# maybeLx/MVSFormerPlusPlus

Hardware: AMD Instinct MI355X
Metric: ref-views/sec at 1152x1536 N=5 D=192 4-stage; achieved HBM GB/s vs peak (higher is better)
Workload: dtype fp16 operands/storage, fp32 accumulate (every stage; 1-2 fp16 MFMA terms)

## Files before the change

### include/mvs_hip.h

```cpp
#ifndef MVS_HIP_H
#define MVS_HIP_H

#include <stddef.h>
#include <stdint.h>

#ifdef __cplusplus
extern "C" {
#endif

#define MVS_ABI_VERSION 11

enum { MVS_OK = 0, MVS_ERR_ARG = 1, MVS_ERR_UNSUPPORTED = 2, MVS_ERR_LAUNCH = 3, MVS_ERR_WORKSPACE = 4 };
enum { MVS_DTYPE_F32 = 0, MVS_DTYPE_BF16 = 1, MVS_DTYPE_F16 = 2 };
enum { MVS_LAYOUT_PLANAR = 0, MVS_LAYOUT_OCTET_TILED = 1 };
enum { MVS_HEAD_CE_EVAL = 0, MVS_HEAD_CE_TRAIN = 1, MVS_HEAD_REG = 2 };
enum { MVS_REG_COSTREGNET = 0, MVS_REG_COSTREGNET3D = 1 };
enum { MVS_PREC_FP32 = 0, MVS_PREC_BF16X3 = 1, MVS_PREC_BF16P = 2, MVS_PREC_BF16X3_SPLIT = 3, MVS_PREC_F16X2 = 4, MVS_PREC_ATTN16 = 5, MVS_PREC_F16 = 6, MVS_PREC_F16MIX = 7 };
enum { MVS_VOLUME_F32 = 0, MVS_VOLUME_SPLIT = 1, MVS_VOLUME_F16 = 2 };
enum { MVS_GATHER_F32 = 0, MVS_GATHER_F16 = 1 };
enum { MVS_CORR_F16 = 0, MVS_CORR_F32 = 1 };
enum { MVS_TR_EPI_BIAS = 0, MVS_TR_EPI_GELU = 1, MVS_TR_EPI_RES_LN = 2 };

int mvs_abi_version(void);

unsigned long long mvs_f16_saturation_count(int reset);
const char* mvs_last_error(void);

int mvs_compose_homography(const float* proj, int B, int V, float* homography , void* stream);
int mvs_cascade_prologue_fwd(const float* const* proj_host_ptrs, int n_stages, int B, int V, float* homography,
                             const float* depth_values, int N, int inverse, float* hyp, int D, int H, int W, void* stream);
int mvs_homography_from_proj(const float* src_proj , const float* ref_proj , int B,
                             float* homography , void* stream);

int mvs_homo_warp_fwd(const void* src_fea, int dtype, const float* homography , const float* depth,
                      int depth_is_volume, float* warped, uint8_t* proj_mask, int B, int C, int D, int H, int W,
                      void* stream);

int mvs_warp_corr_entropy_fwd(const void* features, int dtype, int layout, const float* homography ,
                              const float* hyp, float* entropy, int B, int V, int C, int G, int D, int H, int W,
                              int view_begin, int view_end, int gather_format, void* stream);

int mvs_gather_keeps_correlations(int layout, int C, int G, int D, int H, int W);
int mvs_warp_corr_entropy_keep_fwd(const void* features, int dtype, int layout, const float* homography ,
                                   const float* hyp, float* entropy, void* corr, int corr_format, int B, int V, int C, int G, int D,
                                   int H, int W, void* stream);
int mvs_corr_aggregate_fwd(const void* corr, int corr_format, const float* vis , void* volume_cl, int volume_format,
                           int B, int V, int D, int H, int W, void* stream);

int mvs_feature_conv_is_built(int Cin, int Cout);
int mvs_conv2d3x3_tiles_fwd(const void* x, int in_dtype, const void* w_packed, const float* bias, int act, void* tiled, int out_dtype,
                            int N, int Cin, int Cout, int H, int W, long long in_batch_stride, long long out_batch_stride,
                            void* stream);

int mvs_pack_features(const void* features, int dtype, void* tiled, int out_dtype, int N, int C, int H, int W, void* stream);

size_t mvs_vis_workspace_bytes(int N, int H, int W, int precision);
int mvs_vis_weight_fwd(const float* entropy, const float* w1, const float* b1, const void* w2, const float* b2,
                       const void* w3, const float* b3, const float* w4, const float* b4, float* vis,
                       void* workspace, size_t workspace_bytes, int N, int H, int W, int precision, void* stream);

int mvs_vis_conv1_fwd(const float* entropy, const float* w1, const float* b1, float* out_cl16, int N, int H, int W, void* stream);
int mvs_vis_out_fwd(const float* x_cl8, const float* w4, const float* b4, float* vis, int N, int H, int W, void* stream);

int mvs_warp_corr_aggregate_fwd(const void* features, int dtype, int layout, const float* homography, const float* hyp,
                                const float* vis, float* volume_cl, float* vis_sum, int normalise, int volume_format, int B,
                                int V, int C, int G, int D, int H, int W, int view_begin, int view_end, void* stream);
int mvs_slab_pack(const float* volume_cl, const float* vis_sum, float* const* send_host_ptrs, const int* row_begin, const int* row_end,
                  int n_ranks, int B, int D, int H, int W, int G, void* stream);
int mvs_slab_reduce(const float* volume_cl, const float* vis_sum, float* const* recv_host_ptrs, int n_ranks, int my_rank, float* slab_out,
                    int row_begin, int row_end, int B, int D, int H, int W, int G, void* stream);
int mvs_volume_normalise(float* volume_cl, const float* vis_sum, int B, int D, int H, int W, int G, int volume_format, void* stream);
int mvs_gather_is_lds_staged(int layout, int C, int G, int D, int H, int W);
int mvs_volume_to_f16(const float* volume_cl, const float* vis_sum, void* out_f16, int B, int D, int H, int W, int G, void* stream);

int mvs_warp_corr_aggregate_bwd(const void* features, int dtype, const float* homography, const float* hyp, const float* vis,
                                const float* vis_sum, const float* volume_cl, const float* grad_volume_cl,
                                float* grad_features, float* grad_vis, int B, int V, int C, int G, int D, int H, int W,
                                void* stream);

int mvs_conv3d_bn_relu_fwd(const float* x_cl, const void* w_packed, const float* bias, float* y_cl, int B, int Cin,
                           int Cout, int D, int H, int W, int kd, int sd, int sh, int sw, int relu, int precision,
                           void* stream);

int mvs_conv3d_logits_fwd(const float* x_cl, const void* w_packed, const float* bias, float* logits, int B, int D, int H,
                          int W, int precision, void* stream);

int mvs_deconv3d_linear_fwd(const float* x_cl, const void* w_packed, const float* bias, float* y_cl, int B, int Cin, int Cout,
                            int D, int H, int W, int sd, int precision, void* stream);
int mvs_bn_stats(const float* x_cl, double* sums, long long N, int C, int groups, void* stream);
int mvs_bn_finalize(const double* sums, double count, float eps, float* mean, float* var, float* invstd, float* running_mean,
                    float* running_var, float momentum, int C, int groups, void* stream);
int mvs_bn_running_update(const float* mean, const float* var, double count, float momentum, float* running_mean,
                          float* running_var, int C, int groups, void* stream);
int mvs_bn_relu_apply(const float* z_cl, const float* mean, const float* invstd, const float* gamma, const float* beta,
                      const float* skip_cl, float* y_cl, long long N, int C, int relu, int groups, void* stream);
int mvs_bn_relu_bwd(const float* dy_cl, const float* z_cl, const float* mean, const float* invstd, const float* gamma,
                    const float* beta, double* sums, double count, float* dz_cl, long long N, int C, int relu,
                    int use_batch_stats, int phase, int groups, void* stream);
int mvs_train_block_fwd(const float* a_in_cl, const float* w, int transposed, int Cin, int Cout, int kd, int sd, int sh, int sw,
                        int B, int D, int H, int W, const float* gamma, const float* beta, float eps, float* running_mean,
                        float* running_var, float momentum, const float* skip_cl, const float* zero_bias, void* wpack_ws,
                        double* sums_ws, float* z_cl, float* mean, float* var, float* invstd, float* y_cl, int groups,
                        void* stream);
int mvs_train_block_bwd(const float* dy_cl, const float* a_in_cl, const float* z_cl, const float* mean, const float* var,
                        const float* invstd, const float* w, int transposed, int Cin, int Cout, int kd, int sd, int sh, int sw,
                        int B, int D, int H, int W, const float* gamma, const float* beta, float* running_mean,
                        float* running_var, float momentum, const float* zero_bias, void* wpack_ws, double* sums_ws,
                        float* dz_cl, float* dw, float* dgamma, float* dbeta, float* da_cl, int groups, void* stream);

long long mvs_pack_conv_weights_elems(int cout, int cin, int ntap, int ch);
int mvs_pack_conv_weights(const float* w, void* packed_bf16, int cout, int cin, int ntap, int ch, int tflip, void* stream);
long long mvs_pack_deconv_weights_elems(int cin, int cout, int sd);
int mvs_pack_deconv_weights(const float* w, void* packed_bf16, int cin, int cout, int sd, void* stream);
int mvs_conv3d_wgrad(const float* a_cl, const float* g_cl, float* dw, int B, int CA, int CB, int D, int H, int W, int kd,
                     int sd, int sh, int sw, void* stream);

int mvs_deconv3d_bn_relu_add_fwd(const float* x_cl, const void* w_packed, const float* bias, const float* skip_cl,
                                 float* y_cl, int B, int Cin, int Cout, int D, int H, int W, int sd, int precision,
                                 void* stream);

int mvs_conv3d_generic_fwd(const float* x_cl, const float* w_tck, const float* bias, const float* skip_cl, float* y_cl, int B,
                           int Cin, int Cout, int D, int H, int W, int OD, int OH, int OW, int kd, int kh, int kw, int sd, int sh,
                           int sw, int pd, int ph, int pw, int transposed, int relu, void* stream);
int mvs_conv3d_is_tuned(int Cin, int Cout, int kd, int sd, int sh, int sw);
int mvs_deconv3d_is_tuned(int Cin, int Cout, int sd);

int mvs_deconv3d_prob_fwd(const float* x_cl, const void* w_packed, const float* bias, const float* skip_cl, const float* prob_w,
                          const float* prob_b, float* logits, int B, int Cin, int D, int H, int W, int sd, int precision,
                          void* stream);

size_t mvs_regnet_workspace_bytes(int kind, int B, int D, int H, int W);
int mvs_regnet_fwd(int kind, const float* volume_cl, const void* const* w_packed, const float* const* bias,
                   float* feat_cl, void* workspace, size_t workspace_bytes, int B, int D, int H, int W, int precision,
                   void* stream);
int mvs_regnet_logits_fwd(int kind, const float* volume_cl, const void* const* w_packed, const float* const* bias,
                          const float* prob_w, const float* prob_b, float* logits, void* workspace, size_t workspace_bytes,
                          int B, int D, int H, int W, int precision, void* stream);

int mvs_prob_regress_fwd(const float* feat_cl, const float* prob_w, const float* prob_b, int prob_ksize,
                         const float* hyp, float tmp, int mode, int conf_n, float* depth, float* conf,
                         float* prob_volume, float* prob_volume_pre, int B, int D, int H, int W, void* stream);
int mvs_softmax_regress_fwd(const float* logits, const float* hyp, float tmp, int mode, int conf_n, float* depth,
                            float* conf, float* prob_volume, int B, int D, int H, int W, void* stream);
int mvs_softmax_regress_schedule_fwd(const float* logits, const float* hyp, float tmp, int mode, int conf_n, float* depth, float* conf,
                                     float* prob_volume, float ratio, float* next_hyp, int next_D, int B, int D, int H, int W,
                                     void* stream);
int mvs_softmax_regress_confavg_fwd(const float* logits, const float* hyp, float tmp, int mode, int conf_n, float* depth,
                                    float* conf, float* prob_volume, const float* const* prev_conf_host_ptrs,
                                    const int* prev_shifts_host, int n_prev, float* conf_avg, int B, int D, int H, int W,
                                    void* stream);

int mvs_depth_regression_fwd(const float* p, const float* depth_values, float* out, int B, int D, int H, int W, void* stream);
int mvs_conf_regression_fwd(const float* p, int n, float* out, int B, int D, int H, int W, void* stream);

int mvs_init_range_fwd(const float* depth_values , int N, int inverse, float* hyp , int B,
// ... 103 lines not shown
```

### mvsformerplusplus_amd/_lib.py

```python
from __future__ import annotations

import ctypes as C
import os
import threading
from typing import Optional

import torch

_HERE = os.path.dirname(os.path.abspath(__file__))
LIB_PATH = os.environ.get("MVS_HIP_LIB") or os.path.join(_HERE, "csrc", "libmvs_hip.so")

OK = 0
ABI_VERSION = 11
TR_EPI_BIAS, TR_EPI_GELU, TR_EPI_RES_LN = 0, 1, 2
DTYPE_CODE = {torch.float32: 0, torch.bfloat16: 1, torch.float16: 2}
HEAD_CE_EVAL, HEAD_CE_TRAIN, HEAD_REG = 0, 1, 2
LAYOUT_PLANAR, LAYOUT_OCTET_TILED = 0, 1
REG_COSTREGNET, REG_COSTREGNET3D = 0, 1
PREC_FP32, PREC_BF16X3, PREC_BF16P, PREC_BF16X3_SPLIT, PREC_F16X2, PREC_ATTN16, PREC_F16, PREC_F16MIX = 0, 1, 2, 3, 4, 5, 6, 7
PRECISIONS = {"fp32": PREC_FP32, "bf16x3": PREC_BF16X3, "f16x2": PREC_F16X2, "f16": PREC_F16, "f16mix": PREC_F16MIX}
F16_FORMATS = ("f16x2", "f16", "f16mix")
F16_CODES = (PREC_F16X2, PREC_F16, PREC_F16MIX)
VOLUME_F32, VOLUME_SPLIT, VOLUME_F16 = 0, 1, 2
CORR_F16, CORR_F32 = 0, 1

_vp, _i, _f, _sz = C.c_void_p, C.c_int, C.c_float, C.c_size_t

SIGNATURES = {
    "mvs_abi_version": (_i, []),
    "mvs_f16_saturation_count": (C.c_ulonglong, [_i]),
    "mvs_last_error": (C.c_char_p, []),
    "mvs_compose_homography": (_i, [_vp, _i, _i, _vp, _vp]),
    "mvs_cascade_prologue_fwd": (_i, [_vp, _i, _i, _i, _vp, _vp, _i, _i, _vp, _i, _i, _i, _vp]),
    "mvs_homography_from_proj": (_i, [_vp, _vp, _i, _vp, _vp]),
    "mvs_homo_warp_fwd": (_i, [_vp, _i, _vp, _vp, _i, _vp, _vp, _i, _i, _i, _i, _i, _vp]),
    "mvs_warp_corr_entropy_fwd": (_i, [_vp, _i, _i, _vp, _vp, _vp] + [_i] * 10 + [_vp]),
    "mvs_pack_features": (_i, [_vp, _i, _vp, _i, _i, _i, _i, _i, _vp]),
    "mvs_feature_conv_is_built": (_i, [_i, _i]),
    "mvs_conv2d3x3_tiles_fwd": (_i, [_vp, _i, _vp, _vp, _i, _vp, _i, _i, _i, _i, _i, _i, C.c_longlong, C.c_longlong, _vp]),
    "mvs_vis_workspace_bytes": (_sz, [_i, _i, _i, _i]),
    "mvs_vis_weight_fwd": (_i, [_vp] * 10 + [_vp, _sz, _i, _i, _i, _i, _vp]),
    "mvs_vis_conv1_fwd": (_i, [_vp, _vp, _vp, _vp, _i, _i, _i, _vp]),
    "mvs_vis_out_fwd": (_i, [_vp, _vp, _vp, _vp, _i, _i, _i, _vp]),
    "mvs_warp_corr_aggregate_fwd": (_i, [_vp, _i, _i, _vp, _vp, _vp, _vp, _vp, _i, _i] + [_i] * 9 + [_vp]),
    "mvs_volume_normalise": (_i, [_vp, _vp, _i, _i, _i, _i, _i, _i, _vp]),
    "mvs_volume_to_f16": (_i, [_vp, _vp, _vp, _i, _i, _i, _i, _i, _vp]),
    "mvs_gather_is_lds_staged": (_i, [_i, _i, _i, _i, _i, _i]),
    "mvs_gather_keeps_correlations": (_i, [_i, _i, _i, _i, _i, _i]),
    "mvs_warp_corr_entropy_keep_fwd": (_i, [_vp, _i, _i, _vp, _vp, _vp, _vp] + [_i] * 8 + [_vp]),
    "mvs_corr_aggregate_fwd": (_i, [_vp, _i, _vp, _vp] + [_i] * 6 + [_vp]),
    "mvs_slab_pack": (_i, [_vp, _vp, _vp, _vp, _vp, _i, _i, _i, _i, _i, _i, _vp]),
    "mvs_slab_reduce": (_i, [_vp, _vp, _vp, _i, _i, _vp, _i, _i, _i, _i, _i, _i, _i, _vp]),
    "mvs_conv3d_bn_relu_fwd": (_i, [_vp, _vp, _vp, _vp] + [_i] * 12 + [_vp]),
    "mvs_deconv3d_bn_relu_add_fwd": (_i, [_vp, _vp, _vp, _vp, _vp] + [_i] * 8 + [_vp]),
    "mvs_conv3d_generic_fwd": (_i, [_vp] * 5 + [_i] * 20 + [_vp]),
    "mvs_conv3d_is_tuned": (_i, [_i] * 6),
    "mvs_deconv3d_is_tuned": (_i, [_i] * 3),
    "mvs_deconv3d_prob_fwd": (_i, [_vp] * 7 + [_i] * 7 + [_vp]),
    "mvs_conv3d_logits_fwd": (_i, [_vp] * 4 + [_i] * 5 + [_vp]),
    "mvs_deconv3d_linear_fwd": (_i, [_vp] * 4 + [_i] * 8 + [_vp]),
    "mvs_bn_stats": (_i, [_vp, _vp, C.c_longlong, _i, _i, _vp]),
    "mvs_bn_finalize": (_i, [_vp, C.c_double, C.c_float, _vp, _vp, _vp, _vp, _vp, C.c_float, _i, _i, _vp]),
    "mvs_bn_running_update": (_i, [_vp, _vp, C.c_double, C.c_float, _vp, _vp, _i, _i, _vp]),
    "mvs_bn_relu_apply": (_i, [_vp] * 7 + [C.c_longlong, _i, _i, _i, _vp]),
    "mvs_bn_relu_bwd": (_i, [_vp] * 7 + [C.c_double, _vp, C.c_longlong, _i, _i, _i, _i, _i, _vp]),
    "mvs_train_block_fwd": (_i, [_vp, _vp] + [_i] * 11 + [_vp, _vp, C.c_float, _vp, _vp, C.c_float] + [_vp] * 9 + [_i, _vp]),
    "mvs_train_block_bwd": (_i, [_vp] * 7 + [_i] * 11 + [_vp, _vp, _vp, _vp, C.c_float] + [_vp] * 8 + [_i, _vp]),
    "mvs_pack_conv_weights_elems": (C.c_longlong, [_i] * 4),
    "mvs_pack_conv_weights": (_i, [_vp, _vp] + [_i] * 5 + [_vp]),
    "mvs_pack_deconv_weights_elems": (C.c_longlong, [_i] * 3),
    "mvs_pack_deconv_weights": (_i, [_vp, _vp] + [_i] * 3 + [_vp]),
    "mvs_conv3d_wgrad": (_i, [_vp] * 3 + [_i] * 10 + [_vp]),
    "mvs_warp_corr_aggregate_bwd": (_i, [_vp, _i] + [_vp] * 8 + [_i] * 7 + [_vp]),
    "mvs_regnet_workspace_bytes": (_sz, [_i, _i, _i, _i, _i]),
    "mvs_regnet_fwd": (_i, [_i, _vp, _vp, _vp, _vp, _vp, _sz, _i, _i, _i, _i, _i, _vp]),
    "mvs_regnet_logits_fwd": (_i, [_i, _vp, _vp, _vp, _vp, _vp, _vp, _vp, _sz, _i, _i, _i, _i, _i, _vp]),
    "mvs_prob_regress_fwd": (_i, [_vp, _vp, _vp, _i, _vp, _f, _i, _i, _vp, _vp, _vp, _vp, _i, _i, _i, _i, _vp]),
    "mvs_softmax_regress_fwd": (_i, [_vp, _vp, _f, _i, _i, _vp, _vp, _vp, _i, _i, _i, _i, _vp]),
    "mvs_softmax_regress_schedule_fwd": (_i, [_vp, _vp, _f, _i, _i, _vp, _vp, _vp, _f, _vp, _i, _i, _i, _i, _i, _vp]),
    "mvs_softmax_regress_confavg_fwd": (_i, [_vp, _vp, _f, _i, _i, _vp, _vp, _vp, _vp, _vp, _i, _vp, _i, _i, _i, _i, _vp]),
    "mvs_depth_regression_fwd": (_i, [_vp, _vp, _vp, _i, _i, _i, _i, _vp]),
    "mvs_conf_regression_fwd": (_i, [_vp, _i, _vp, _i, _i, _i, _i, _vp]),
    "mvs_init_range_fwd": (_i, [_vp, _i, _i, _vp, _i, _i, _i, _i, _vp]),
    "mvs_init_range_pixel_fwd": (_i, [_vp, _i, _i, _vp, _i, _i, _i, _i, _vp]),
    "mvs_schedule_inverse_range_fwd": (_i, [_vp, _vp, _i, _f, _i, _vp, _i, _i, _i, _i, _vp]),
    "mvs_schedule_range_fwd": (_i, [_vp, _vp, _i, _vp, _i, _i, _i, _i, _vp]),
    "mvs_confidence_average": (_i, [_vp, _vp, _i, _vp, _i, _i, _i, _vp]),
    "mvs_position3d_workspace_bytes": (_sz, []),
    "mvs_position3d_fwd": (_i, [_vp, _vp, _vp, _i, _vp, _i, _vp, _sz, _vp, _i, _i, _i, _i, _vp]),
    "mvs_position3d_raw_fwd": (_i, [_vp, _vp, _vp, _i, _i, _i, _i, _vp]),
    "mvs_position_encoding3d_fwd": (_i, [_vp, _vp, _vp, _i, _i, _f, C.c_longlong, _vp]),
    "mvs_tr_embed_fwd": (_i, [_vp] * 9 + [_i] * 8 + [_vp]),
    "mvs_tr_linear_fwd": (_i, [_vp, _vp, _vp, _i, _vp, _vp, _vp, _vp, _f, _vp, _i, _i, _i, _i, _i, _vp]),
    "mvs_tr_attention_operand_bytes": (_sz, [_i, _i, _i]),
    "mvs_tr_qkv_fwd": (_i, [_vp, _vp, _vp, _vp, _vp, _f, _i, _i, _i, _i, _i, _vp]),
    "mvs_tr_attention_fwd": (_i, [_vp, _vp, _vp, _vp, _i, _i, _i, _i, _vp]),
    "mvs_tr_attention_bwd": (_i, [_vp, _vp, _vp, _vp, _vp, _vp, _i, _i, _i, _f, _vp]),
    "mvs_tr_up_prob_fwd": (_i, [_vp] * 8 + [_i] * 8 + [_vp]),
    "mvs_fusion_campack_floats": (_sz, []),
    "mvs_fusion_prepare_cams": (_i, [_vp, _i, _vp, _vp]),
    "mvs_fusion_filter_fwd": (_i, [_i] + [_vp] * 8 + [_f] * 4 + [_vp] * 7 + [_i] * 4 + [_vp]),
    "mvs_fusion_ave_fwd": (_i, [_vp, _vp, _vp, _vp, _i, _i, _i, _i, _vp]),
    "mvs_pointcloud_workspace_bytes": (_sz, [_i, _i]),
    "mvs_pointcloud_append": (_i, [_vp, _vp, _vp, _i, _i, _vp, _sz, _vp, _vp, _i, _vp, C.c_longlong, _vp]),
    "mvs_gipuma_view_floats": (_sz, []),
    "mvs_gipuma_pair_floats": (_sz, []),
    "mvs_gipuma_prepare_cams": (_i, [_vp, _i, _vp, _vp]),
    "mvs_gipuma_prepare_view": (_i, [_vp, _vp, _vp, _i, _i, _vp, _vp, _vp]),
    "mvs_gipuma_fuse_view": (_i, [_vp] * 5 + [_i] * 4 + [C.c_double, C.c_double, _f, C.c_double] + [_vp] * 5),
    "mvs_colmap_workspace_bytes": (_sz, [_i]),
    "mvs_colmap_depths": (_i, [_vp, _vp, C.c_longlong, _vp, _vp, _vp, _vp]),
    "mvs_colmap_scores": (_i, [_vp, _vp, _vp, _i, _vp, _vp, _i, _vp, _vp, C.c_double, C.c_double, C.c_double, C.c_longlong]
                          + [_vp] * 3 + [_sz, _vp, _vp]),
    "mvs_fpn_conv_is_built": (_i, [_i] * 4),
    "mvs_fpn_merge_is_built": (_i, [_i, _i]),
    "mvs_fpn_conv_fwd": (_i, [_vp, _vp, _vp, _i, _vp] + [_i] * 7 + [_vp]),
    "mvs_fpn_merge_fwd": (_i, [_vp] * 5 + [_i] * 4 + [_vp]),
    "mvs_fpn_merge_conv_fwd": (_i, [_vp] * 6 + [_i, _vp] + [_i] * 5 + [_vp]),
    "mvs_fmt_weights_bytes": (_sz, []),
    "mvs_fmt_vectors_bytes": (_sz, []),
    "mvs_fmt_kv_operand_bytes": (_sz, []),
    "mvs_fmt_kv_workspace_bytes": (_sz, [_i, _i]),
    "mvs_fmt_kv_fwd": (_i, [_vp] * 5 + [_sz, _vp, _i, _i, _vp]),
    "mvs_fmt_block_fwd": (_i, [_vp] * 6 + [_i, _i, _i, _vp]),
    "mvs_fmt_path_fwd": (_i, [_vp] * 5 + [_i] * 6 + [_vp]),
    "mvs_fmt_merge_fwd": (_i, [_vp] * 4 + [_i] * 6 + [_vp]),
    "mvs_fmt_smooth_fwd": (_i, [_vp] * 3 + [_i] * 4 + [_vp]),
    "mvs_ncdhw_to_cl": (_i, [_vp, _vp, _i, _i, _i, _i, _i, _vp]),
    "mvs_cl_to_ncdhw": (_i, [_vp, _vp, _i, _i, _i, _i, _i, _vp]),
}

# ... 88 lines not shown
```

### mvsformerplusplus_amd/cost_volume.py

```python
from __future__ import annotations

from typing import Dict, Optional

import torch
import torch.nn as nn

from . import _lib, ops, packing
from .module import (DEFAULT_PRECISION, DEFAULT_STAGE_POLICY, resolve_stage_precision, F16_FORMATS, MFMA_FORMATS, ConvBnReLU, CostRegNet, CostRegNet3D, PureTransformerCostReg, _bn_dict, _no_grad_path,
                     _PackedCache, precision_code)


def shard_views(n_src: int, world: int, rank: int):
    base, extra = divmod(n_src, world)
    begin = 1 + rank * base + min(rank, extra)
    return begin, begin + base + (1 if rank < extra else 0)


STAGE_DEFAULT_PRECISION = DEFAULT_STAGE_POLICY


_F16_CALLS = {}
_F16_CHECK_DUE = set()
KEEP_CORRELATIONS_MAX_BYTES = 1 << 30
KEEP_MIN_DEPTH = 5
# ... 83 lines not shown

        def build(dev):
            out = []
            for i, ch in ((0, None), (1, 16), (2, 16)):
                layer = self.vis[i]
                w, b = packing.fold_bn(layer.conv.weight.detach().cpu().float(), _bn_dict(layer.bn), 0)
                if i == 0:
                    out += [w[:, 0].permute(1, 2, 0).reshape(9, 16).contiguous().to(dev), b.contiguous().to(dev)]
                else:
                    out += [pack(w.unsqueeze(2), 16).to(dev), packing.pad_bias(b).to(dev)]
            last = self.vis[3]
            out += [last.weight.detach().float().reshape(8).contiguous().to(dev), last.bias.detach().float().reshape(1).contiguous().to(dev)]
            return out
        return self._vis_cache.get(self.vis, build, prec)

    def _vis_precision(self) -> str:
        return self.conv_precision

    def _keeps_correlations(self, feats, G, hyp) -> bool:
        if not self.keep_correlations:
            return False
        exact = self.gather_precision != "f16"
        B, V, _, H, W = feats.shape
        D = hyp.shape[1]
        dmin = self.keep_min_depth if self.keep_min_depth is not None else (KEEP_EXACT_MIN_DEPTH if exact else KEEP_MIN_DEPTH)
        if D < dmin or (exact and D <= 4):
            return False
        if (V - 1) * B * D * H * W * (32 if exact else 16) > KEEP_CORRELATIONS_MAX_BYTES:
            return False
        return ops.gather_keeps_correlations(feats, G, hyp)

    def _f16_activations(self) -> bool:
        return self.conv_precision in F16_FORMATS and not isinstance(self.cost_reg, PureTransformerCostReg) and not self._generic_regulariser()

    def _generic_regulariser(self) -> bool:
        return bool(getattr(self.cost_reg, "is_generic", False))

    def _wants_autograd(self, features) -> bool:
        return self.training or (torch.is_grad_enabled() and torch.is_tensor(features) and features.requires_grad)

    def forward(self, features, proj_matrices, depth_values, tmp, position3d=None, _fused: Optional[dict] = None) -> Dict[str, torch.Tensor]:
        if self._wants_autograd(features):
            from .training import stage_forward_train
            assert features.shape[1] == proj_matrices.shape[1], "Different number of images and projection matrices"
            return stage_forward_train(self, features, proj_matrices, depth_values, tmp, position3d)
        B, V, C, H, W = features.shape
        assert V == proj_matrices.shape[1], "Different number of images and projection matrices"
        G = self.in_channels
        if G > C:
            raise AssertionError("G must <= C!")
        if C % G != 0:
            raise AssertionError("base_ch=%d must divide the %d feature channels (the reference's .view(B, G, C // G, ...), cost_volume.py:80)" % (G, C))
        feats, code = ops._feat(features)
        hyp = ops._f32c(depth_values)
        if hyp.dim() == 2:
            hyp = hyp[:, :, None, None].expand(B, hyp.shape[1], H, W).contiguous()
        elif hyp.dim() != 4:
            raise ValueError("depth_values must be [B,D] or [B,D,H,W], got shape %s" % (tuple(depth_values.shape),))
        hom = _fused.get("homography") if _fused else None
        if hom is None:
            hom = ops.compose_homography(proj_matrices)
        conf_prev = _fused.get("conf_prev") if _fused and self.view_group is None else None
        nxt = _fused.get("next") if _fused and self.view_group is None and conf_prev is None and hyp.shape[1] >= 3 else None
        vis_params = self._vis_params(feats.device)
        prec = precision_code(self._vis_precision())
        if self.view_group is not None:
            import torch.distributed as dist
            world = dist.get_world_size(self.view_group)
            slab = self._slab_plan(H, world) if self.shard_mode in ("auto", "slab") else None
            if slab is not None and not isinstance(self.cost_reg, PureTransformerCostReg):
                return self._forward_slab(feats, code, hom, hyp, depth_values, G, vis_params, float(tmp), slab)
            volume = self._sharded_volume(feats, code, hom, hyp, G, vis_params)
            split = self._split_activations()
        else:
            split = self._split_activations()
            f16 = self._f16_activations()
            w16 = self.gather_precision == "f16"
            if self._keeps_correlations(feats, G, hyp):
                entropy, corr = ops.warp_corr_entropy_keep(feats, code, hom, hyp, G, exact=not w16)
                vis = ops.vis_weight(entropy, vis_params, prec)
                volume = ops.corr_aggregate(corr, vis, split=split, f16=f16)
                del corr
            else:
                entropy = ops.warp_corr_entropy(feats, code, hom, hyp, G, f16_window=w16)
                vis = ops.vis_weight(entropy, vis_params, prec)
                if f16 and not ops.gather_is_lds_staged(feats, G, hyp):
                    volume = ops.volume_to_f16(ops.warp_corr_aggregate(feats, code, hom, hyp, vis, G, normalise=True)[0])
                else:
                    volume, _ = ops.warp_corr_aggregate(feats, code, hom, hyp, vis, G, normalise=True, split=split, f16=f16)
        out = self._regularise_and_regress(volume, hyp, depth_values, float(tmp), position3d, split=split, conf_prev=conf_prev, nxt=nxt)
        if conf_prev is not None:
            _fused["conf_avg"] = out.pop("_conf_avg")
        if "_next_hyp" in out:
            _fused["next_hyp"] = out.pop("_next_hyp")
        if self._f16_activations():
            self._count_f16_call(feats.device, hyp)
        return out

    @staticmethod
    def _count_f16_call(device, hyp=None):
        key = device.index if device.type == "cuda" else -1
        n = _F16_CALLS[key] = _F16_CALLS.get(key, 0) + 1
        due = bool(F16_SATURATION_CHECK_EVERY) and (n == 8 or n % F16_SATURATION_CHECK_EVERY == 0 or key in _F16_CHECK_DUE)
        if not due:
            return
        if device.type == "cuda" and torch.cuda.is_current_stream_capturing():
            _F16_CHECK_DUE.add(key)
            return
        _F16_CHECK_DUE.discard(key)
        check_f16_saturation(device)
        if hyp is not None:
            check_hypothesis_conditioning(hyp)

    def _split_activations(self) -> bool:
        return self.conv_precision == "bf16x3" and not isinstance(self.cost_reg, PureTransformerCostReg) and not self._generic_regulariser()

    def _head_mode(self, D):
        conf_n = 0
        if self.depth_type == "ce":
            mode = _lib.HEAD_CE_TRAIN if self.training else _lib.HEAD_CE_EVAL
        else:
            mode = _lib.HEAD_REG
            conf_n = 4 if D >= 32 else (3 if D == 16 else (2 if D == 8 else 0))
        return mode, conf_n

    def _regularise_and_regress(self, volume, hyp, depth_values, tmp, position3d=None, split=False, conf_prev=None, nxt=None) -> Dict[str, torch.Tensor]:
        D = hyp.shape[1]
        pcode = _lib.PREC_BF16X3_SPLIT if split else precision_code(self.conv_precision)
        mfma = self.conv_precision in MFMA_FORMATS
        mode, conf_n = self._head_mode(D)
        conf_avg = None

        def head(logits):
            if nxt is not None:
                return ops.softmax_regress_schedule(logits, hyp, tmp, mode, conf_n, self.return_prob_volumes, int(nxt[0]), float(nxt[1]))
            return ops.softmax_regress(logits, hyp, tmp, mode, conf_n, self.return_prob_volumes, conf_prev=conf_prev)

        if isinstance(self.cost_reg, PureTransformerCostReg):
            prob_volume_pre = self.cost_reg.logits_cl(volume, position3d)
            depth, conf, prob_volume, *rest = head(prob_volume_pre)
        elif self._generic_regulariser():
            prob_volume_pre = self.cost_reg.logits_cl_generic(volume)
            depth, conf, prob_volume, *rest = head(prob_volume_pre)
        else:
            ws, bs, prob_w, prob_b = self.cost_reg.packed_all(volume.device, self.conv_precision)
            if self.cost_reg.prob_ksize == 1 and mfma and self.fuse_prob_head:
                prob_volume_pre = ops.regnet_logits(self.cost_reg.kind, volume, ws, bs, prob_w, prob_b, pcode)
                depth, conf, prob_volume, *rest = head(prob_volume_pre)
            elif self.cost_reg.prob_ksize == 3 and mfma:
                feat_cl = ops.regnet(self.cost_reg.kind, volume, ws, bs, pcode)
                prob_volume_pre = ops.conv3d_logits(feat_cl, prob_w, prob_b, pcode)
                depth, conf, prob_volume, *rest = head(prob_volume_pre)
            else:
                feat_cl = ops.regnet(self.cost_reg.kind, volume, ws, bs, pcode)
                if split:
                    feat_cl = ops.from_split(feat_cl)
                elif feat_cl.dtype == torch.float16:
                    feat_cl = feat_cl.float()
                depth, conf, prob_volume, prob_volume_pre = ops.prob_regress(
                    feat_cl, prob_w, prob_b, self.cost_reg.prob_ksize, hyp, tmp, mode, conf_n, self.return_prob_volumes)
                rest = []
                if conf_prev is not None:
                    rest = [ops.confidence_average(list(conf_prev) + [conf], conf.shape[-2], conf.shape[-1])]
        out = {"depth": depth, "prob_volume": prob_volume, "photometric_confidence": conf,
               "depth_values": depth_values, "prob_volume_pre": prob_volume_pre}
        if conf_prev is not None:
            out["_conf_avg"] = rest[0]
        elif nxt is not None and rest:
            out["_next_hyp"] = rest[0]
        return out

    MAX_CACHED_SHAPES = 2
# ... 131 lines not shown
```

### mvsformerplusplus_amd/csrc/gather_lds.h

```cpp
#pragma once
#include "gather_common.h"

namespace mvs {

#ifndef MVS_GL_CAP
#define MVS_GL_CAP 1024
#endif
constexpr int GL_CAP = MVS_GL_CAP;
constexpr int GL_XALIGN = 8;
constexpr int GL_DCH = 4;
constexpr int GL_TH = 4;

#ifndef MVS_OPAQUE_SREG
#define MVS_OPAQUE_SREG "s"
#endif
__device__ __forceinline__ float gl_round_f16(float v) { return (float)(_Float16)fminf(fmaxf(v, -65504.0f), 65504.0f); }

#ifndef MVS_GL_DIRECT16
#define MVS_GL_DIRECT16 1
#endif
template <typename T, bool TILED, bool W16, int NOCT, bool KEEPPASS>
constexpr bool gl_direct_v = (MVS_GL_DIRECT16 != 0) && W16 && TILED && std::is_same<T, _Float16>::value && NOCT == 1;

#ifndef MVS_GL_OPT
#define MVS_GL_OPT 1
#endif
#ifndef MVS_GL_SB
#define MVS_GL_SB 2
#endif
#ifndef MVS_GL_ABL
#define MVS_GL_ABL 0
#endif

#define GL_BLEND8(wv, t00, t01, t10, t11, tp)                                                          \
    _Pragma("unroll") for (int j = 0; j < 4; ++j) {                                                    \
        wv[2 * j] = MVS_FMA_MIX_LO(t00[j], tp.w00, 0.0f);                                              \
        wv[2 * j + 1] = MVS_FMA_MIX_HI(t00[j], tp.w00, 0.0f);                                          \
    }                                                                                                  \
    _Pragma("unroll") for (int j = 0; j < 4; ++j) {                                                    \
        wv[2 * j] = MVS_FMA_MIX_LO(t01[j], tp.w01, wv[2 * j]);                                         \
        wv[2 * j + 1] = MVS_FMA_MIX_HI(t01[j], tp.w01, wv[2 * j + 1]);                                 \
    }                                                                                                  \
    _Pragma("unroll") for (int j = 0; j < 4; ++j) {                                                    \
        wv[2 * j] = MVS_FMA_MIX_LO(t10[j], tp.w10, wv[2 * j]);                                         \
        wv[2 * j + 1] = MVS_FMA_MIX_HI(t10[j], tp.w10, wv[2 * j + 1]);                                 \
    }                                                                                                  \
    _Pragma("unroll") for (int j = 0; j < 4; ++j) {                                                    \
        wv[2 * j] = MVS_FMA_MIX_LO(t11[j], tp.w11, wv[2 * j]);                                         \
        wv[2 * j + 1] = MVS_FMA_MIX_HI(t11[j], tp.w11, wv[2 * j + 1]);                                 \
    }

template <typename T, int NOCT, bool KEEP_GROUPS, bool TILED, bool W16, bool DIRECT = false>
__device__ __forceinline__ void gl_unit(const T* __restrict__ src, const T* __restrict__ ref, const Homography& hm, float fx, float fy,
                                        const float* depth, bool active, int H, int W, unsigned HW, unsigned pc, f32x4* win,
                                        unsigned* red, int unit, float wscale, const float* rf_in, float* out) {
    typedef typename PairOf<T>::type P2;
    constexpr int GPO = 8 / NOCT;
    constexpr int CPG = NOCT;
    const int tid = (int)threadIdx.x, lane = tid & 63, wave = tid >> 6;
    const float qx = hm.r[0] * fx + hm.r[1] * fy + hm.r[2];
    const float qy = hm.r[3] * fx + hm.r[4] * fy + hm.r[5];
    const float qz = hm.r[6] * fx + hm.r[7] * fy + hm.r[8];
    GTap tp[GL_DCH];
    u16x2 mn = {0xffff, 0xffff}, mx = {0, 0};
    const float cx = 0.5f * (float)(W - 1), cy = 0.5f * (float)(H - 1);
#if MVS_GL_OPT
#pragma unroll
    for (int dd = 0; dd < GL_DCH; ++dd) {
#if MVS_GL_ABL == 6
        tp[dd].pk = ((unsigned)(int)fy << 16) | (unsigned)(int)fx; tp[dd].w00 = depth[dd]; tp[dd].w01 = qx; tp[dd].w10 = 0.25f; tp[dd].w11 = 0.25f;
        if ((int)fx > W - 2 || (int)fy > H - 2) tp[dd].pk = 0;
#else
        tp[dd] = make_gtap(hm, qx, qy, qz, depth[dd], H, W, cx, cy);
#endif
        const u16x2 pkv = gl_as_vec(tp[dd].pk);
        mn = __builtin_elementwise_min(mn, pkv);
        mx = __builtin_elementwise_max(mx, (u16x2)(pkv + (u16x2){1, 1}));
    }
    if (!active) { mn = (u16x2){0xffff, 0xffff}; mx = (u16x2){0, 0}; }
#else
#pragma unroll
    for (int dd = 0; dd < GL_DCH; ++dd) {
        tp[dd] = make_gtap(hm, qx, qy, qz, depth[dd], H, W, cx, cy);
        if (active && tp[dd].pk != GL_NONE) {
            mn = __builtin_elementwise_min(mn, gl_as_vec(tp[dd].pk));
            mx = __builtin_elementwise_max(mx, gl_as_vec(tp[dd].pk));
        }
    }
#endif
    if constexpr (DIRECT) {
        static_assert(W16 && TILED && std::is_same<T, _Float16>::value, "the direct form reads fp16 octet tiles");
        typedef unsigned u32x4 __attribute__((ext_vector_type(4)));
        unsigned tofs[GL_DCH];
#pragma unroll
        for (int dd = 0; dd < GL_DCH; ++dd) {
            const unsigned pk = tp[dd].pk;
            tofs[dd] = pk == GL_NONE ? 0u : ((pk >> 16) * (unsigned)W + (pk & 0xffffu)) * 16u;
        }
        const int rowb = W * 16;
        if (!active) return;
#pragma unroll
        for (int o = 0; o < NOCT; ++o) {
            unsigned oofs = gl_octet_offset(o, HW);
            asm volatile("" : "+" MVS_OPAQUE_SREG(oofs));
            const __amdgpu_buffer_rsrc_t rs = __builtin_amdgcn_make_buffer_rsrc(const_cast<T*>(src + oofs), 0, (int)(HW * 16u), 0x00020000);
            float rf[8];
            if (NOCT > 1) {
                gl_load8<TILED, T>(ref + oofs, HW, pc, rf);
            } else {
#pragma unroll
                for (int c = 0; c < 8; ++c) rf[c] = rf_in[c];
            }
            u32x4 t[GL_DCH][4];
#pragma unroll
            for (int dd = 0; dd < GL_DCH; ++dd) {
#if MVS_GL_DIRECT16 == 3
                (void)rs; (void)rowb;
#pragma unroll
                for (int k = 0; k < 4; ++k) t[dd][k] = u32x4{tofs[dd], tofs[dd] + (unsigned)k, tofs[dd] ^ 0x3c003c00u, 0x3c003c00u};
#else
                t[dd][0] = __builtin_amdgcn_raw_buffer_load_b128(rs, (int)tofs[dd], 0, 0);
                t[dd][1] = __builtin_amdgcn_raw_buffer_load_b128(rs, (int)(tofs[dd] + 16u), 0, 0);
                t[dd][2] = __builtin_amdgcn_raw_buffer_load_b128(rs, (int)tofs[dd], rowb, 0);
                t[dd][3] = __builtin_amdgcn_raw_buffer_load_b128(rs, (int)(tofs[dd] + 16u), rowb, 0);
#endif
            }
#pragma unroll
            for (int c = 0; c < 8; ++c) rf[c] *= wscale;
#pragma unroll
            for (int dd = 0; dd < GL_DCH; ++dd) {
                float wv[8];
#if MVS_GL_DIRECT16 == 2
#pragma unroll
                for (int j = 0; j < 4; ++j) {
                    const unsigned x = t[dd][0][j] ^ t[dd][1][j] ^ t[dd][2][j] ^ t[dd][3][j];
                    wv[2 * j] = __builtin_bit_cast(float, x & 0x3fffffffu);
                    wv[2 * j + 1] = tp[dd].w00;
                }
#elif MVS_GL_OPT
                GL_BLEND8(wv, t[dd][0], t[dd][1], t[dd][2], t[dd][3], tp[dd])
#else
#pragma unroll
                for (int j = 0; j < 4; ++j) {
                    float a = MVS_FMA_MIX_LO(t[dd][0][j], tp[dd].w00, 0.0f);
                    a = MVS_FMA_MIX_LO(t[dd][1][j], tp[dd].w01, a);
                    a = MVS_FMA_MIX_LO(t[dd][2][j], tp[dd].w10, a);
                    wv[2 * j] = MVS_FMA_MIX_LO(t[dd][3][j], tp[dd].w11, a);
                    float b = MVS_FMA_MIX_HI(t[dd][0][j], tp[dd].w00, 0.0f);
                    b = MVS_FMA_MIX_HI(t[dd][1][j], tp[dd].w01, b);
                    b = MVS_FMA_MIX_HI(t[dd][2][j], tp[dd].w10, b);
                    wv[2 * j + 1] = MVS_FMA_MIX_HI(t[dd][3][j], tp[dd].w11, b);
                }
#endif
                if (KEEP_GROUPS) {
#pragma unroll
                    for (int j = 0; j < GPO; ++j) {
                        float s = out[(o * GPO + j) * GL_DCH + dd];
#pragma unroll
                        for (int c = 0; c < CPG; ++c) s += rf[j * CPG + c] * wv[j * CPG + c];
                        out[(o * GPO + j) * GL_DCH + dd] = s;
                    }
                } else {
                    float s = out[dd];
#pragma unroll
                    for (int c = 0; c < 8; ++c) s += rf[c] * wv[c];
                    out[dd] = s;
                }
            }
        }
        return;
    }
#if MVS_GL_ABL == 5
    {
        __syncthreads();
        const unsigned p0 = (unsigned)__builtin_amdgcn_readfirstlane((int)tp[0].pk);
        const unsigned bx = (p0 & 0xffffu) > 8u ? (p0 & 0xffffu) - 8u : 0u, by = (p0 >> 16) > 2u ? (p0 >> 16) - 2u : 0u;
        mn = gl_as_vec((by << 16) | bx);
        mx = gl_as_vec(((by + 9u) << 16) | (bx + 81u));
#pragma unroll
        for (int dd = 0; dd < GL_DCH; ++dd) tp[dd].pk = ((by + 1u + (unsigned)(lane & 3)) << 16) | (bx + 1u + (unsigned)(lane & 63));
    }
#else
    mn = gl_wave_reduce<false>(mn);
    mx = gl_wave_reduce<true>(mx);
    unsigned* rd = red + (unit & 1) * 8;
    if (lane == 63) { rd[wave] = gl_as_u32(mn); rd[4 + wave] = gl_as_u32(mx); }
    __syncthreads();
    mn = __builtin_elementwise_min(__builtin_elementwise_min(gl_as_vec(rd[0]), gl_as_vec(rd[1])),
                                   __builtin_elementwise_min(gl_as_vec(rd[2]), gl_as_vec(rd[3])));
    mx = __builtin_elementwise_max(__builtin_elementwise_max(gl_as_vec(rd[4]), gl_as_vec(rd[5])),
                                   __builtin_elementwise_max(gl_as_vec(rd[6]), gl_as_vec(rd[7])));
#endif
#if MVS_GL_OPT
    const int xmin = mn[0], ymin = mn[1], xmax = (int)mx[0] - 1, ymax = (int)mx[1] - 1;
#else
    const int xmin = mn[0], ymin = mn[1], xmax = mx[0], ymax = mx[1];
#endif
    if (xmax < xmin) return;
    const int wx0 = xmin & ~(GL_XALIGN - 1);
    const int ww = (xmax + 2 - wx0 + GL_XALIGN - 1) & ~(GL_XALIGN - 1);
    const int wh = ymax + 2 - ymin;
    const int n = ww * wh;
    typedef _Float16 h8 __attribute__((ext_vector_type(8)));
    h8* win16 = reinterpret_cast<h8*>(win);
    if (n <= (W16 ? 2 * GL_CAP : GL_CAP)) {
        unsigned pos[GL_DCH];
#pragma unroll
        for (int dd = 0; dd < GL_DCH; ++dd) {
            const unsigned pk = tp[dd].pk;
#if MVS_GL_OPT
            const unsigned raw = ((pk >> 16) - (unsigned)ymin) * (unsigned)ww + ((pk & 0xffffu) - (unsigned)wx0);
            pos[dd] = raw < (unsigned)(n - ww - 2) ? raw : (unsigned)(n - ww - 2);
#else
            pos[dd] = pk == GL_NONE ? 0u : ((pk >> 16) - (unsigned)ymin) * (unsigned)ww + ((pk & 0xffffu) - (unsigned)wx0);
#endif
        }
        const float inv_ww = __builtin_amdgcn_rcpf((float)ww) * 1.000001f;
        const unsigned gbase = (unsigned)ymin * (unsigned)W + (unsigned)wx0;
#pragma unroll
        for (int o = 0; o < NOCT; ++o) {
            if (o > 0) __syncthreads();
            unsigned oofs = gl_octet_offset(o, HW);
            asm volatile("" : "+" MVS_OPAQUE_SREG(oofs));
            const T* so = src + oofs;
            float rf[8];
            if (NOCT > 1) {
                gl_load8<TILED, T>(ref + oofs, HW, pc, rf);
            } else {
#pragma unroll
                for (int c = 0; c < 8; ++c) rf[c] = rf_in[c];
            }
#if MVS_GL_OPT
            const __amdgpu_buffer_rsrc_t srs = __builtin_amdgcn_make_buffer_rsrc(const_cast<T*>(so), 0, (int)(8u * HW * (unsigned)sizeof(T)), 0x00020000);
            const unsigned planeb = HW * (unsigned)sizeof(T);
#endif
            int istart = tid;
#if MVS_GL_OPT && MVS_GL_ABL == 0
            if constexpr (!TILED) {
                constexpr int SBR = NOCT == 1 ? MVS_GL_SB : 1;
#pragma unroll 1
                for (int i0 = tid; i0 < n; i0 += 256 * SBR) {
                    float v[SBR][8];
#pragma unroll
                    for (int k = 0; k < SBR; ++k) {
                        const int i = i0 + 256 * k;
                        if (i < n) {
                            const int row = (int)(((float)i + 0.5f) * inv_ww);
                            const unsigned g = gbase + (unsigned)row * (unsigned)(W - ww) + (unsigned)i;
#pragma unroll
                            for (int c = 0; c < 8; ++c) {
                                if constexpr (sizeof(T) == 4)
                                    v[k][c] = __builtin_bit_cast(float, __builtin_amdgcn_raw_buffer_load_b32(srs, (int)(g * 4u), (int)((unsigned)c * planeb), 0));
                                else
                                    v[k][c] = to_f32(__builtin_bit_cast(T, (unsigned short)__builtin_amdgcn_raw_buffer_load_b16(srs, (int)(g * 2u), (int)((unsigned)c * planeb), 0)));
                            }
                        }
                    }
#pragma unroll
                    for (int k = 0; k < SBR; ++k) {
                        const int i = i0 + 256 * k;
                        if (i < n) {
                            if (W16) {
                                h8 hv;
#pragma unroll
                                for (int c = 0; c < 8; ++c) hv[c] = (_Float16)__builtin_amdgcn_fmed3f(v[k][c], -65504.0f, 65504.0f);
                                win16[i] = hv;
                            } else {
                                win[i] = f32x4{v[k][0], v[k][1], v[k][2], v[k][3]};
                                win[GL_CAP + i] = f32x4{v[k][4], v[k][5], v[k][6], v[k][7]};
                            }
                        }
                    }
                }
                istart = n;
// ... 30 lines not shown
                }
#endif
                if constexpr (W16 && TILED && std::is_same<T, _Float16>::value) {
                    win16[i] = *(reinterpret_cast<const h8*>(so) + g);
                    continue;
                }
                float v[8];
                gl_load8<TILED, T>(so, HW, g, v);
                if (W16) {
                    h8 hv;
#pragma unroll
                    for (int c = 0; c < 8; ++c) hv[c] = (_Float16)fminf(fmaxf(v[c], -65504.0f), 65504.0f);
                    win16[i] = hv;
                } else {
                    win[i] = f32x4{v[0], v[1], v[2], v[3]};
                    win[GL_CAP + i] = f32x4{v[4], v[5], v[6], v[7]};
                }
            }
            __syncthreads();
            if (active) {
#pragma unroll
                for (int c = 0; c < 8; ++c) rf[c] *= wscale;
#pragma unroll
                for (int dd = 0; dd < GL_DCH; ++dd) {
                    if (dd == 2) __builtin_amdgcn_sched_barrier(0);
                    float wv[8];
                    if (W16) {
                        typedef unsigned u32x4 __attribute__((ext_vector_type(4)));
                        const u32x4* w0 = reinterpret_cast<const u32x4*>(win16) + pos[dd];
#if MVS_GL_ABL == 3
                        const u32x4 t00 = {pos[dd], 0x3c003c00u, 0x3c003c00u, pos[dd]}, t01 = t00, t10 = {0x3c003c00u, pos[dd], pos[dd], 0x3c003c00u}, t11 = t10;
#else
                        const u32x4 t00 = w0[0], t01 = w0[1], t10 = w0[ww], t11 = w0[ww + 1];
#endif
#if MVS_GL_ABL == 4
#pragma unroll
                        for (int j = 0; j < 4; ++j) { wv[2 * j] = __builtin_bit_cast(float, (t00[j] ^ t01[j] ^ t10[j] ^ t11[j]) & 0x3fffffffu); wv[2 * j + 1] = tp[dd].w00; }
#elif MVS_GL_OPT
                        GL_BLEND8(wv, t00, t01, t10, t11, tp[dd])
#else
#pragma unroll
                        for (int j = 0; j < 4; ++j) {
                            float a = MVS_FMA_MIX_LO(t00[j], tp[dd].w00, 0.0f);
                            a = MVS_FMA_MIX_LO(t01[j], tp[dd].w01, a);
                            a = MVS_FMA_MIX_LO(t10[j], tp[dd].w10, a);
                            wv[2 * j] = MVS_FMA_MIX_LO(t11[j], tp[dd].w11, a);
                            float b = MVS_FMA_MIX_HI(t00[j], tp[dd].w00, 0.0f);
                            b = MVS_FMA_MIX_HI(t01[j], tp[dd].w01, b);
                            b = MVS_FMA_MIX_HI(t10[j], tp[dd].w10, b);
                            wv[2 * j + 1] = MVS_FMA_MIX_HI(t11[j], tp[dd].w11, b);
                        }
#endif
                    } else {
                        const f32x4* w0 = win + pos[dd];
                        const f32x4 a0 = w0[0], a1 = w0[1], b0 = w0[ww], b1 = w0[ww + 1];
                        const f32x4 c0 = w0[GL_CAP], c1 = w0[GL_CAP + 1], d0 = w0[GL_CAP + ww], d1 = w0[GL_CAP + ww + 1];
                        f32x4 lo = a0 * tp[dd].w00;
                        lo += a1 * tp[dd].w01;
                        lo += b0 * tp[dd].w10;
                        lo += b1 * tp[dd].w11;
                        f32x4 hi = c0 * tp[dd].w00;
                        hi += c1 * tp[dd].w01;
                        hi += d0 * tp[dd].w10;
                        hi += d1 * tp[dd].w11;
                        wv[0] = lo[0]; wv[1] = lo[1]; wv[2] = lo[2]; wv[3] = lo[3]; wv[4] = hi[0]; wv[5] = hi[1]; wv[6] = hi[2]; wv[7] = hi[3];
                    }
                    if (KEEP_GROUPS) {
#pragma unroll
                        for (int j = 0; j < GPO; ++j) {
                            float s = out[(o * GPO + j) * GL_DCH + dd];
#pragma unroll
                            for (int c = 0; c < CPG; ++c) s += rf[j * CPG + c] * wv[j * CPG + c];
                            out[(o * GPO + j) * GL_DCH + dd] = s;
                        }
                    } else {
                        float s = out[dd];
#pragma unroll
                        for (int c = 0; c < 8; ++c) s += rf[c] * wv[c];
                        out[dd] = s;
                    }
                }
            }
        }
    } else if (active) {
        unsigned top[GL_DCH];
#pragma unroll
        for (int dd = 0; dd < GL_DCH; ++dd) top[dd] = tp[dd].pk == GL_NONE ? 0u : (tp[dd].pk >> 16) * (unsigned)W + (tp[dd].pk & 0xffffu);
#pragma unroll 1
        for (int c = 0; c < 8 * NOCT; ++c) {
            const unsigned cbase = TILED ? (unsigned)(c >> 3) * 8u * HW + (unsigned)(c & 7) : (unsigned)c * HW;
            const unsigned pstep = TILED ? 8u : 1u;
            const float rfc = to_f32(ref[cbase + pc * pstep]) * wscale;
            const T* sp = src + cbase;
            const int g = c / CPG;
#pragma unroll
            for (int dd = 0; dd < GL_DCH; ++dd) {
                float t0, t1, b0, b1;
                if (TILED) {
                    __builtin_amdgcn_sched_barrier(0);
                    t0 = to_f32(sp[top[dd] * 8u]); t1 = to_f32(sp[(top[dd] + 1u) * 8u]);
                    b0 = to_f32(sp[(top[dd] + (unsigned)W) * 8u]); b1 = to_f32(sp[(top[dd] + (unsigned)W + 1u) * 8u]);
                } else {
                    const P2 t = *reinterpret_cast<const P2*>(sp + top[dd]);
                    const P2 b = *reinterpret_cast<const P2*>(sp + top[dd] + (unsigned)W);
                    t0 = to_f32(t.x); t1 = to_f32(t.y); b0 = to_f32(b.x); b1 = to_f32(b.y);
                }
                if (W16) {
                    t0 = gl_round_f16(t0); t1 = gl_round_f16(t1); b0 = gl_round_f16(b0); b1 = gl_round_f16(b1);
                }
                float wv = tp[dd].w00 * t0;
                wv += tp[dd].w01 * t1;
                wv += tp[dd].w10 * b0;
                wv += tp[dd].w11 * b1;
                if (KEEP_GROUPS) {
#pragma unroll
                    for (int gg = 0; gg < 8; ++gg) out[gg * GL_DCH + dd] += (g == gg) ? rfc * wv : 0.0f;
                } else {
                    out[dd] += rfc * wv;
                }
            }
        }
    }
}

constexpr size_t GL_WIN_BYTES = (size_t)2 * GL_CAP * 16;
constexpr size_t GL_RED_BYTES = 64;

template <int NS>
struct GlTile {
    static constexpr int TP = 256 / NS, TW = TP / GL_TH;
    int slot, pi, x, y;
    bool valid;
    unsigned pc;
    float fx, fy;
    __device__ __forceinline__ GlTile(int blk, int ntx, int H, int W) {
        const int tid = (int)threadIdx.x;
        const int ty = blk / ntx, tx = blk - ty * ntx;
        slot = tid / TP;
        pi = tid % TP;
        x = tx * TW + pi % TW;
        y = ty * GL_TH + pi / TW;
        valid = x < W && y < H;
        pc = valid ? (unsigned)y * (unsigned)W + (unsigned)x : (unsigned)H * (unsigned)W - 1u;
        fx = (float)(valid ? x : W - 1);
        fy = (float)(valid ? y : H - 1);
    }
};

template <int DT, int NOCT, int NS, bool TILED, bool KEEP, bool W16>
__global__ __launch_bounds__(256) void gl_entropy_kernel(const void* __restrict__ feat_, const float* __restrict__ hom,
                                                         const float* __restrict__ hyp, float* __restrict__ entropy,
                                                         void* __restrict__ corr, int V, int D, int H,
                                                         int W, int view_begin, int view_end, int vpb, int ntx, int nblk) {
    typedef typename FeatT<DT>::type T;
    constexpr bool DIRECT = gl_direct_v<T, TILED, W16, NOCT, KEEP>;
    HIP_DYNAMIC_SHARED(float, smem)
    f32x4* win = reinterpret_cast<f32x4*>(smem);
    unsigned* red = reinterpret_cast<unsigned*>(reinterpret_cast<char*>(smem) + GL_WIN_BYTES);
    float* sim = reinterpret_cast<float*>(reinterpret_cast<char*>(smem) + GL_WIN_BYTES + GL_RED_BYTES);
    constexpr int C = 8 * NOCT;
    constexpr int TP = GlTile<NS>::TP;
    const unsigned HW = (unsigned)H * (unsigned)W;
    const int b = (int)blockIdx.z;
    const GlTile<NS> t((int)xcd_remap(blockIdx.x, (unsigned)nblk), ntx, H, W);
    const int nch = (D + GL_DCH - 1) / GL_DCH, niter = (nch + NS - 1) / NS;
    const T* feat = reinterpret_cast<const T*>(feat_) + (size_t)(b * V) * C * HW;
    const T* ref = feat;
    const float* hp = hyp + (size_t)b * D * HW;
    const float inv_cpg = 1.0f / (float)NOCT;
    float rf0[8];
    if (NOCT == 1) gl_load8<TILED, T>(ref, HW, t.pc, rf0);
    else {
#pragma unroll
        for (int c = 0; c < 8; ++c) rf0[c] = 0.0f;
    }
    const int v0 = view_begin + (int)blockIdx.y * vpb, v1 = v0 + vpb < view_end ? v0 + vpb : view_end;
    int unit = 0;
    float sat_amax = 0.0f;
    for (int v = v0; v < v1; ++v) {
        const Homography hm = gl_load_homography(hom + (size_t)(b * (V - 1) + (v - 1)) * 12);
        const T* src = feat + (size_t)v * C * HW;
        float s[GL_DCH];
        for (int it = 0; it < niter; ++it, ++unit) {
            const int chunk = it * NS + t.slot;
            const bool active = t.valid && chunk < nch;
            const int d0 = (chunk < nch ? chunk : nch - 1) * GL_DCH;
            float depth[GL_DCH];
#pragma unroll
            for (int dd = 0; dd < GL_DCH; ++dd) depth[dd] = hp[(unsigned)(d0 + dd < D ? d0 + dd : D - 1) * HW + t.pc];
#pragma unroll
            for (int dd = 0; dd < GL_DCH; ++dd) s[dd] = 0.0f;
            if (KEEP) {
                float acc[8 * GL_DCH];
#pragma unroll
                for (int i = 0; i < 8 * GL_DCH; ++i) acc[i] = 0.0f;
                gl_unit<T, NOCT, true, TILED, W16, DIRECT>(src, ref, hm, t.fx, t.fy, depth, active, H, W, HW, t.pc, win, red, unit, inv_cpg, rf0, acc);
                typedef _Float16 h8 __attribute__((ext_vector_type(8)));
                const size_t cbase = (size_t)(b * (V - 1) + (v - 1)) * D * HW + t.pc;
#pragma unroll
                for (int dd = 0; dd < GL_DCH; ++dd) {
                    float r[8];
#pragma unroll
                    for (int g = 0; g < 8; ++g) { r[g] = acc[g * GL_DCH + dd]; s[dd] += r[g]; }
                    if (active && d0 + dd < D) {
                        const size_t vox = cbase + (size_t)(unsigned)(d0 + dd) * HW;
                        if constexpr (W16) {
                            h8 hv;
#pragma unroll
                            for (int g = 0; g < 8; ++g) hv[g] = (_Float16)fminf(fmaxf(r[g], -65504.0f), 65504.0f);
                            sat::track(sat_amax, r[0], r[1], r[2], r[3]);
                            sat::track(sat_amax, r[4], r[5], r[6], r[7]);
                            reinterpret_cast<h8*>(corr)[vox] = hv;
                        } else {
                            f32x4* cv = reinterpret_cast<f32x4*>(corr) + vox * 2;
                            cv[0] = f32x4{r[0], r[1], r[2], r[3]};
                            cv[1] = f32x4{r[4], r[5], r[6], r[7]};
                        }
                    }
                }
            } else {
                gl_unit<T, NOCT, false, TILED, W16, DIRECT>(src, ref, hm, t.fx, t.fy, depth, active, H, W, HW, t.pc, win, red, unit, inv_cpg, rf0, s);
            }
            if (NS > 1 || niter > 1) {
                if (chunk < nch) {
#pragma unroll
                    for (int dd = 0; dd < GL_DCH; ++dd)
                        if (d0 + dd < D) sim[(d0 + dd) * TP + t.pi] = s[dd];
                }
            }
        }
        float* dst = entropy + (size_t)(b * (V - 1) + (v - 1)) * HW + t.pc;
        if (NS == 1 && niter == 1) {
            const float LOG2E = 1.4426950408889634f, LN2 = 0.6931471805599453f;
            float m = s[0];
#pragma unroll
            for (int dd = 1; dd < GL_DCH; ++dd) m = dd < D ? fmaxf(m, s[dd]) : m;
            float e[GL_DCH], den = 0.0f;
#pragma unroll
            for (int dd = 0; dd < GL_DCH; ++dd) { e[dd] = dd < D ? __builtin_amdgcn_exp2f((s[dd] - m) * LOG2E) : 0.0f; den += e[dd]; }
            const float rden = 1.0f / den;
            float ent = 0.0f;
#pragma unroll
            for (int dd = 0; dd < GL_DCH; ++dd) {
                const float pr = e[dd] * rden;
                if (dd < D) ent -= pr * (__builtin_amdgcn_logf(pr + 1e-7f) * LN2);
            }
            if (t.valid) *dst = ent;
        } else {
            __syncthreads();
            if (t.slot == 0 && t.valid) gl_softmax_entropy_store(sim + t.pi, TP, D, dst);
            if constexpr (DIRECT) __syncthreads();
        }
    }
    if (KEEP && W16) sat::commit(sat_amax);
}

template <int DT, int NOCT, int NS, bool TILED, bool W16>
__global__ __launch_bounds__(256) void gl_aggregate_kernel(const void* __restrict__ feat_, const float* __restrict__ hom,
                                                           const float* __restrict__ hyp, const float* __restrict__ vis,
                                                           float* __restrict__ vol, float* __restrict__ vis_sum, int normalise, int V,
                                                           int D, int H, int W, int view_begin, int view_end, int ntx, int nblk) {
    typedef typename FeatT<DT>::type T;
    HIP_DYNAMIC_SHARED(float, smem)
    f32x4* win = reinterpret_cast<f32x4*>(smem);
    unsigned* red = reinterpret_cast<unsigned*>(reinterpret_cast<char*>(smem) + GL_WIN_BYTES);
    constexpr int C = 8 * NOCT;
    const unsigned HW = (unsigned)H * (unsigned)W;
    const int b = (int)blockIdx.z, it = (int)blockIdx.y;
    const GlTile<NS> t((int)xcd_remap(blockIdx.x, (unsigned)nblk), ntx, H, W);
    const int nch = (D + GL_DCH - 1) / GL_DCH;
    const T* feat = reinterpret_cast<const T*>(feat_) + (size_t)(b * V) * C * HW;
    const T* ref = feat;
    const float* hp = hyp + (size_t)b * D * HW;
    const float* vp = vis + (size_t)(b * (V - 1)) * HW + t.pc;
    float vsum = 0.0f;
    for (int v = view_begin; v < view_end; ++v) vsum += vp[(unsigned)(v - 1) * HW];
    if (vis_sum != nullptr && it == 0 && t.slot == 0 && t.valid) vis_sum[(size_t)b * HW + t.pc] = vsum;
    const float rdenom = (normalise & 1) ? 1.0f / (vsum + 1e-6f) : 1.0f;
    const bool split_out = (normalise & 2) != 0;
    const bool f16_out = (normalise & 4) != 0;
    float sat_amax = 0.0f;
    const float inv_cpg = 1.0f / (float)NOCT;
    float rf0[8];
    if (NOCT == 1) gl_load8<TILED, T>(ref, HW, t.pc, rf0);
    else {
#pragma unroll
        for (int c = 0; c < 8; ++c) rf0[c] = 0.0f;
    }
    const int chunk = it * NS + t.slot;
    const bool active = t.valid && chunk < nch;
    const int d0 = (chunk < nch ? chunk : nch - 1) * GL_DCH;
    float depth[GL_DCH];
#pragma unroll
    for (int dd = 0; dd < GL_DCH; ++dd) depth[dd] = hp[(unsigned)(d0 + dd < D ? d0 + dd : D - 1) * HW + t.pc];
    float acc[8 * GL_DCH];
#pragma unroll
    for (int i = 0; i < 8 * GL_DCH; ++i) acc[i] = 0.0f;
    int unit = 0;
    for (int v = view_begin; v < view_end; ++v, ++unit) {
        const Homography hm = gl_load_homography(hom + (size_t)(b * (V - 1) + (v - 1)) * 12);
        const float w = vp[(unsigned)(v - 1) * HW];
        gl_unit<T, NOCT, true, TILED, W16, gl_direct_v<T, TILED, W16, NOCT, false>>(feat + (size_t)v * C * HW, ref, hm, t.fx, t.fy, depth, active, H, W, HW, t.pc, win, red, unit, inv_cpg * w, rf0, acc);
    }
    if (active) {
        float* vb = vol + (size_t)b * D * HW * 8;
#pragma unroll
        for (int dd = 0; dd < GL_DCH; ++dd) {
            if (d0 + dd >= D) continue;
            float r[8];
#pragma unroll
            for (int g = 0; g < 8; ++g) r[g] = acc[g * GL_DCH + dd] * rdenom;
            if (f16_out) {
                typedef _Float16 h8 __attribute__((ext_vector_type(8)));
                h8 hv;
#pragma unroll
                for (int g = 0; g < 8; ++g) hv[g] = (_Float16)fminf(fmaxf(r[g], -65504.0f), 65504.0f);
                sat::track(sat_amax, r[0], r[1], r[2], r[3]);
                sat::track(sat_amax, r[4], r[5], r[6], r[7]);
                *reinterpret_cast<h8*>(reinterpret_cast<_Float16*>(vol) + ((size_t)b * D * HW + (size_t)(unsigned)(d0 + dd) * HW + t.pc) * 8) = hv;
                continue;
            }
            f32x4* o = reinterpret_cast<f32x4*>(vb + ((size_t)(unsigned)(d0 + dd) * HW + t.pc) * 8);
            if (split_out) {
                unsigned hw[4], lw[4];
#pragma unroll
                for (int j = 0; j < 4; ++j) {
                    const uint16_t h0 = from_f32<uint16_t>(r[2 * j]), h1 = from_f32<uint16_t>(r[2 * j + 1]);
                    const uint16_t l0 = from_f32<uint16_t>(r[2 * j] - to_f32(h0)), l1 = from_f32<uint16_t>(r[2 * j + 1] - to_f32(h1));
                    hw[j] = (unsigned)h0 | ((unsigned)h1 << 16);
                    lw[j] = (unsigned)l0 | ((unsigned)l1 << 16);
                }
                o[0] = f32x4{__builtin_bit_cast(float, hw[0]), __builtin_bit_cast(float, hw[1]), __builtin_bit_cast(float, hw[2]), __builtin_bit_cast(float, hw[3])};
                o[1] = f32x4{__builtin_bit_cast(float, lw[0]), __builtin_bit_cast(float, lw[1]), __builtin_bit_cast(float, lw[2]), __builtin_bit_cast(float, lw[3])};
                continue;
            }
            o[0] = f32x4{r[0], r[1], r[2], r[3]};
            o[1] = f32x4{r[4], r[5], r[6], r[7]};
        }
    }
    if (f16_out) sat::commit(sat_amax);
}

static int gl_slots(int D) {
    const int nch = (D + GL_DCH - 1) / GL_DCH;
    return nch >= 8 ? 8 : (nch >= 4 ? 4 : (nch >= 2 ? 2 : 1));
}

bool gl_window_f16_enabled();
bool gl_supported(int C, int G, int D, int H, int W);

template <int DT, int NOCT, int NS, bool TILED, bool KEEP = false, bool W16 = false>
static int gl_launch_entropy_t(const void* feat, const float* hom, const float* hyp, float* ent, int B, int V, int D, int H, int W, int vb,
                               int ve, hipStream_t st, void* corr = nullptr) {
    constexpr int TP = 256 / NS, TW = TP / GL_TH;
    const int ntx = (int)ceil_div(W, TW), nty = (int)ceil_div(H, GL_TH);
    const int nblk = ntx * nty;
    const int vpb = (long long)nblk * B >= 4096 ? ve - vb : 1;
    const size_t lds = GL_WIN_BYTES + GL_RED_BYTES + (size_t)D * TP * sizeof(float);
    if (lds > 48 * 1024)
        hipFuncSetAttribute(reinterpret_cast<const void*>(&gl_entropy_kernel<DT, NOCT, NS, TILED, KEEP, W16>), hipFuncAttributeMaxDynamicSharedMemorySize, (int)lds);
    hipLaunchKernelGGL((gl_entropy_kernel<DT, NOCT, NS, TILED, KEEP, W16>), dim3(nblk, ceil_div(ve - vb, vpb), B), dim3(256), lds, st, feat, hom, hyp, ent,
                       corr, V, D, H, W, vb, ve, vpb, ntx, nblk);
    return check_launch("gl_entropy_kernel");
}

template <int DT, int NOCT, int NS, bool TILED, bool W16 = false>
static int gl_launch_aggregate_t(const void* feat, const float* hom, const float* hyp, const float* vis, float* vol, float* vis_sum,
                                 int normalise, int B, int V, int D, int H, int W, int vb, int ve, hipStream_t st) {
    constexpr int TP = 256 / NS, TW = TP / GL_TH;
    const int ntx = (int)ceil_div(W, TW), nty = (int)ceil_div(H, GL_TH);
    const int nblk = ntx * nty;
    const int nch = (D + GL_DCH - 1) / GL_DCH, niter = (nch + NS - 1) / NS;
    const size_t lds = GL_WIN_BYTES + GL_RED_BYTES;
    hipLaunchKernelGGL((gl_aggregate_kernel<DT, NOCT, NS, TILED, W16>), dim3(nblk, niter, B), dim3(256), lds, st, feat, hom, hyp, vis, vol, vis_sum,
                       normalise, V, D, H, W, vb, ve, ntx, nblk);
    return check_launch("gl_aggregate_kernel");
}

#define GL_DISPATCH_NS(FN, DTV, NOCTV, ...)                                                    \
    switch (gl_slots(D) * 2 + (layout == MVS_LAYOUT_OCTET_TILED ? 1 : 0)) {                    \
        case 2: return FN<DTV, NOCTV, 1, false>(__VA_ARGS__);                                  \
        case 3: return FN<DTV, NOCTV, 1, true>(__VA_ARGS__);                                   \
        case 4: return FN<DTV, NOCTV, 2, false>(__VA_ARGS__);                                  \
        case 5: return FN<DTV, NOCTV, 2, true>(__VA_ARGS__);                                   \
        case 8: return FN<DTV, NOCTV, 4, false>(__VA_ARGS__);                                  \
        case 9: return FN<DTV, NOCTV, 4, true>(__VA_ARGS__);                                   \
        case 16: return FN<DTV, NOCTV, 8, false>(__VA_ARGS__);                                 \
        default: return FN<DTV, NOCTV, 8, true>(__VA_ARGS__);                                  \
    }
#define GL_DISPATCH_C(FN, DTV, ...)                                                            \
    switch (C) {                                                                               \
        case 8: GL_DISPATCH_NS(FN, DTV, 1, __VA_ARGS__)                                        \
        case 16: GL_DISPATCH_NS(FN, DTV, 2, __VA_ARGS__)                                       \
        case 32: GL_DISPATCH_NS(FN, DTV, 4, __VA_ARGS__)                                       \
        default: GL_DISPATCH_NS(FN, DTV, 8, __VA_ARGS__)                                       \
    }
#define GL_DISPATCH(FN, ...)                                                                   \
    do {                                                                                       \
        switch (dtype) {                                                                       \
            case MVS_DTYPE_F32: GL_DISPATCH_C(FN, MVS_DTYPE_F32, __VA_ARGS__)                  \
            case MVS_DTYPE_BF16: GL_DISPATCH_C(FN, MVS_DTYPE_BF16, __VA_ARGS__)                \
            default: GL_DISPATCH_C(FN, MVS_DTYPE_F16, __VA_ARGS__)                             \
        }                                                                                      \
    } while (0)


}
```

### mvsformerplusplus_amd/csrc/gather_lds_aggregate_kernels.hip

```cpp
#include "gather_lds.h"

namespace mvs {

int gl_launch_aggregate_w16(const void* feat, int dtype, int layout, const float* hom, const float* hyp, const float* vis, float* vol, float* vis_sum,
                            int normalise, int B, int V, int C, int D, int H, int W, int vb, int ve, hipStream_t st);

int gl_launch_aggregate(const void* feat, int dtype, int layout, const float* hom, const float* hyp, const float* vis, float* vol, float* vis_sum,
                        int normalise, int B, int V, int C, int D, int H, int W, int vb, int ve, hipStream_t st) {
    if ((normalise & 4) && gl_window_f16_enabled())
        return gl_launch_aggregate_w16(feat, dtype, layout, hom, hyp, vis, vol, vis_sum, normalise, B, V, C, D, H, W, vb, ve, st);
    GL_DISPATCH(gl_launch_aggregate_t, feat, hom, hyp, vis, vol, vis_sum, normalise, B, V, D, H, W, vb, ve, st);
}

}

namespace mvs { MVS_DEFINE_SAT_READER(sat_read_gather_agg) }
```

### mvsformerplusplus_amd/csrc/gather_lds_aggregate_w16_kernels.hip

```cpp
#include "gather_lds.h"

namespace mvs {

template <int DT, int NOCT, int NS, bool TILED>
static int gl_launch_aggregate_w16_t(const void* feat, const float* hom, const float* hyp, const float* vis, float* vol, float* vis_sum,
                                     int normalise, int B, int V, int D, int H, int W, int vb, int ve, hipStream_t st) {
    return gl_launch_aggregate_t<DT, NOCT, NS, TILED, true>(feat, hom, hyp, vis, vol, vis_sum, normalise, B, V, D, H, W, vb, ve, st);
}

int gl_launch_aggregate_w16(const void* feat, int dtype, int layout, const float* hom, const float* hyp, const float* vis, float* vol, float* vis_sum,
                            int normalise, int B, int V, int C, int D, int H, int W, int vb, int ve, hipStream_t st) {
    GL_DISPATCH(gl_launch_aggregate_w16_t, feat, hom, hyp, vis, vol, vis_sum, normalise, B, V, D, H, W, vb, ve, st);
}

}

namespace mvs { MVS_DEFINE_SAT_READER(sat_read_gather_agg16) }
```

### mvsformerplusplus_amd/csrc/gather_lds_entropy_w16_kernels.hip

```cpp
#include "gather_lds.h"

namespace mvs {

template <int DT, int NOCT, int NS, bool TILED>
static int gl_launch_entropy_w16_t(const void* feat, const float* hom, const float* hyp, float* ent, int B, int V, int D, int H, int W, int vb,
                                   int ve, hipStream_t st) {
    return gl_launch_entropy_t<DT, NOCT, NS, TILED, false, true>(feat, hom, hyp, ent, B, V, D, H, W, vb, ve, st);
}

int gl_launch_entropy_w16(const void* feat, int dtype, int layout, const float* hom, const float* hyp, float* ent, int B, int V, int C, int D, int H, int W,
                          int vb, int ve, hipStream_t st) {
    GL_DISPATCH(gl_launch_entropy_w16_t, feat, hom, hyp, ent, B, V, D, H, W, vb, ve, st);
}

}
```

### mvsformerplusplus_amd/csrc/gather_lds_kernels.hip

```cpp
#include "gather_lds.h"

namespace mvs {

bool gl_window_f16_enabled() {
    static const int on = [] { const char* e = getenv("MVS_GATHER_WINDOW"); return (e && e[0] == 'f' && e[1] == '3') ? 0 : 1; }();
    return on != 0;
}

bool gl_supported(int C, int G, int D, int H, int W) {
    if (G != 8 || !(C == 8 || C == 16 || C == 32 || C == 64)) return false;
    if (W % GL_XALIGN != 0 || W < GL_XALIGN || H < 2 || W > 65535 || H > 65535) return false;
    if ((long long)D * H * W > 0x7fffffffLL) return false;
    if ((long long)H * W >= (1LL << 28)) return false;
    return (size_t)D * (256 / gl_slots(D)) * sizeof(float) <= 64 * 1024;
}

bool gl_keep_supported(int C, int G, int D, int H, int W) { return gl_supported(C, G, D, H, W); }
bool gl_keep32_supported(int C, int G, int D, int H, int W) { return gl_supported(C, G, D, H, W) && D > GL_DCH; }


int gl_launch_entropy_w16(const void* feat, int dtype, int layout, const float* hom, const float* hyp, float* ent, int B, int V, int C, int D, int H, int W,
                          int vb, int ve, hipStream_t st);

int gl_launch_entropy(const void* feat, int dtype, int layout, const float* hom, const float* hyp, float* ent, int B, int V, int C, int D, int H, int W,
                      int vb, int ve, int w16, hipStream_t st) {
    if (w16 && gl_window_f16_enabled()) return gl_launch_entropy_w16(feat, dtype, layout, hom, hyp, ent, B, V, C, D, H, W, vb, ve, st);
    GL_DISPATCH(gl_launch_entropy_t, feat, hom, hyp, ent, B, V, D, H, W, vb, ve, st);
}

template <typename TI, typename TO>
__global__ __launch_bounds__(256) void pack_features_kernel(const TI* __restrict__ in, TO* __restrict__ out, int C, unsigned HW) {
    const unsigned p = blockIdx.x * 256u + threadIdx.x;
    if (p >= HW) return;
    const size_t n = blockIdx.z, o = blockIdx.y;
    const TI* src = in + (n * C + o * 8) * HW + p;
    TO* dst = out + ((n * (C / 8) + o) * HW + p) * 8;
    typedef TO to8 __attribute__((ext_vector_type(8)));
    to8 v;
#pragma unroll
    for (int c = 0; c < 8; ++c) {
        float f = to_f32(src[(size_t)c * HW]);
        if (std::is_same<TO, _Float16>::value && !std::is_same<TI, _Float16>::value) f = fminf(fmaxf(f, -65504.0f), 65504.0f);
        if (sizeof(TI) == 2 && sizeof(TO) == 2) v[c] = *reinterpret_cast<const TO*>(&src[(size_t)c * HW]);
        else v[c] = from_f32<TO>(f);
    }
    *reinterpret_cast<to8*>(dst) = v;
}

template <typename TI, typename TO>
static int pack_features_t(const void* in, void* out, int N, int C, int H, int W, hipStream_t st) {
    const unsigned HW = (unsigned)H * (unsigned)W;
    hipLaunchKernelGGL((pack_features_kernel<TI, TO>), dim3(ceil_div(HW, 256), C / 8, N), dim3(256), 0, st, static_cast<const TI*>(in),
                       static_cast<TO*>(out), C, HW);
    return check_launch("pack_features_kernel");
}

int pack_features_dispatch(const void* in, int in_dtype, void* out, int out_dtype, int N, int C, int H, int W, hipStream_t st) {
    if (out_dtype == MVS_DTYPE_F32) {
        switch (in_dtype) {
            case MVS_DTYPE_F32: return pack_features_t<float, float>(in, out, N, C, H, W, st);
            case MVS_DTYPE_BF16: return pack_features_t<uint16_t, float>(in, out, N, C, H, W, st);
            default: return pack_features_t<_Float16, float>(in, out, N, C, H, W, st);
        }
    }
    if (out_dtype == MVS_DTYPE_BF16) {
        switch (in_dtype) {
            case MVS_DTYPE_F32: return pack_features_t<float, uint16_t>(in, out, N, C, H, W, st);
            case MVS_DTYPE_BF16: return pack_features_t<uint16_t, uint16_t>(in, out, N, C, H, W, st);
            default: set_error("mvs_pack_features: fp16 -> bf16 is not a hand-off the reference produces"); return MVS_ERR_UNSUPPORTED;
        }
    }
    switch (in_dtype) {
        case MVS_DTYPE_F32: return pack_features_t<float, _Float16>(in, out, N, C, H, W, st);
        case MVS_DTYPE_F16: return pack_features_t<_Float16, _Float16>(in, out, N, C, H, W, st);
        default: set_error("mvs_pack_features: bf16 -> fp16 is not a hand-off the reference produces"); return MVS_ERR_UNSUPPORTED;
    }
}

}

namespace mvs { MVS_DEFINE_SAT_READER(sat_read_gather) }
```

### mvsformerplusplus_amd/csrc/warp_kernels.hip

```cpp
#include "mvs_common.h"

#include <stdlib.h>

namespace mvs {

__device__ void compose_p(const float* pm , double* P ) {
    const float* E = pm;
    const float* K = pm + 16;
    for (int i = 0; i < 3; ++i)
        for (int j = 0; j < 4; ++j) {
            float s = 0.0f;
            for (int k = 0; k < 3; ++k) s += K[i * 4 + k] * E[k * 4 + j];
            P[i * 4 + j] = (double)s;
        }
    for (int j = 0; j < 4; ++j) P[12 + j] = (double)E[12 + j];
}

__device__ void invert4(const double* A, double* Ai) {
    double m[4][8];
    for (int i = 0; i < 4; ++i)
        for (int j = 0; j < 4; ++j) { m[i][j] = A[i * 4 + j]; m[i][4 + j] = (i == j) ? 1.0 : 0.0; }
    for (int c = 0; c < 4; ++c) {
        int piv = c;
        double best = fabs(m[c][c]);
// ... 423 lines not shown
}

template <int DT>
__global__ __launch_bounds__(256) void homo_warp_kernel(const void* __restrict__ src_, const float* __restrict__ hom,
                                                        const float* __restrict__ depth_, int depth_is_volume,
                                                        float* __restrict__ warped, uint8_t* __restrict__ mask, int C, int D, int H,
                                                        int W) {
    typedef typename FeatT<DT>::type T;
    const int HW = H * W;
    const int lane = threadIdx.x & 63, slot = threadIdx.x >> 6;
    const int p = (int)blockIdx.x * 64 + lane;
    const int b = (int)blockIdx.z;
    if (p >= HW) return;
    const int y = p / W, x = p - y * W;
    const Homography hm = load_homography(hom + (size_t)b * 12);
    const float fx = (float)x, fy = (float)y;
    const float qx = hm.r[0] * fx + hm.r[1] * fy + hm.r[2];
    const float qy = hm.r[3] * fx + hm.r[4] * fy + hm.r[5];
    const float qz = hm.r[6] * fx + hm.r[7] * fy + hm.r[8];
    const float half_w = (float)((double)(W - 1) / 2.0), half_h = (float)((double)(H - 1) / 2.0);
    const T* src = reinterpret_cast<const T*>(src_) + (size_t)b * C * HW;
    for (int d = (int)blockIdx.y * 4 + slot; d < D; d += (int)gridDim.y * 4) {
        const float depth = depth_is_volume ? depth_[((size_t)b * D + d) * HW + p] : depth_[(size_t)b * D + d];
        bool oof;
        const Taps tp = make_taps(hm, qx, qy, qz, depth, H, W, half_w, half_h, &oof);
        if (mask != nullptr) mask[((size_t)b * D + d) * HW + p] = oof ? 1 : 0;
        if (warped != nullptr) {
            for (int c = 0; c < C; ++c) {
                const T* sp = src + (size_t)c * HW;
                float wv = tp.w[0] * to_f32(sp[tp.off[0]]);
                wv += tp.w[1] * to_f32(sp[tp.off[1]]);
                wv += tp.w[2] * to_f32(sp[tp.off[2]]);
                wv += tp.w[3] * to_f32(sp[tp.off[3]]);
                warped[(((size_t)b * C + c) * D + d) * HW + p] = wv;
            }
        }
    }
}

template <int DT, int CT, int GT>
static int launch_entropy(const void* feat, const float* hom, const float* hyp, float* ent, int B, int V, int C, int G,
                          int D, int H, int W, int vb, int ve, hipStream_t st) {
    const int HW = H * W;
    const int ppb = CT > 0 ? chunk_map(D).ppb : 64;
    const int nblk = (int)ceil_div(HW, ppb);
    const size_t lds = (size_t)D * ppb * sizeof(float);
    if (lds > 160 * 1024) { set_error("warp_corr_entropy: D=%d needs %zu B of LDS (> 160 KiB)", D, lds); return MVS_ERR_UNSUPPORTED; }
    if (lds > 48 * 1024)
        hipFuncSetAttribute(reinterpret_cast<const void*>(&warp_corr_entropy_kernel<DT, CT, GT>), hipFuncAttributeMaxDynamicSharedMemorySize, (int)lds);
    hipLaunchKernelGGL((warp_corr_entropy_kernel<DT, CT, GT>), dim3(nblk, ve - vb, B), dim3(256), lds, st, feat, hom, hyp, ent, V, C, G, D,
                       H, W, vb, nblk);
    return check_launch("warp_corr_entropy_kernel");
}

template <int DT, int CT, int GT>
static int launch_aggregate(const void* feat, const float* hom, const float* hyp, const float* vis, float* vol, float* vis_sum,
                            int normalise, int B, int V, int C, int G, int D, int H, int W, int vb, int ve, hipStream_t st) {
    const int nblk = (int)ceil_div((long long)H * W, CT > 0 ? chunk_map(D).ppb : 64);
    hipLaunchKernelGGL((warp_corr_aggregate_kernel<DT, CT, GT>), dim3(nblk, 1, B), dim3(256), 0, st, feat, hom, hyp, vis, vol, vis_sum,
                       normalise, V, C, G, D, H, W, vb, ve, nblk);
    return check_launch("warp_corr_aggregate_kernel");
}

#define MVS_DISPATCH_CG(FN, DT, ...)                                              \
    do {                                                                          \
        if (G == 8 && W >= 2) return FN<DT, 1, 8>(__VA_ARGS__);                   \
        return FN<DT, 0, 0>(__VA_ARGS__);                                         \
    } while (0)

static int check_corr_args(const char* who, const void* feat, const float* hom, const float* hyp, int dtype, int B, int V, int C, int G,
                           int D, int H, int W, int vb, int ve) {
    if (!feat || !hom || !hyp) { set_error("%s: null pointer", who); return MVS_ERR_ARG; }
    if (B < 1 || V < 2 || C < 1 || G < 1 || D < 1 || H < 1 || W < 1) { set_error("%s: bad shape", who); return MVS_ERR_ARG; }
    if (G > C || C % G != 0) { set_error("%s: G must divide C and G <= C (got C=%d G=%d)", who, C, G); return MVS_ERR_ARG; }
    if (G > 64) { set_error("%s: G=%d > 64 unsupported", who, G); return MVS_ERR_UNSUPPORTED; }
    if (vb < 1 || ve > V || vb >= ve) { set_error("%s: bad source-view range [%d,%d) for V=%d", who, vb, ve, V); return MVS_ERR_ARG; }
    if (dtype < 0 || dtype > 2) { set_error("%s: bad dtype %d", who, dtype); return MVS_ERR_ARG; }
    if ((long long)B * V * C * H * W > 0x7fffffffLL * 2 || (long long)C * H * W > 0x7fffffffLL) { set_error("%s: feature tensor too large for 32-bit plane offsets", who); return MVS_ERR_UNSUPPORTED; }
    return MVS_OK;
}

bool gl_supported(int C, int G, int D, int H, int W);
int gl_launch_entropy(const void* feat, int dtype, int layout, const float* hom, const float* hyp, float* ent, int B, int V, int C, int D, int H,
                      int W, int vb, int ve, int w16, hipStream_t st);
int gl_launch_aggregate(const void* feat, int dtype, int layout, const float* hom, const float* hyp, const float* vis, float* vol,
                        float* vis_sum, int normalise, int B, int V, int C, int D, int H, int W, int vb, int ve, hipStream_t st);
bool gl_keep_supported(int C, int G, int D, int H, int W);
bool gl_keep32_supported(int C, int G, int D, int H, int W);
int gl_launch_entropy_keep(const void* feat, int dtype, int layout, const float* hom, const float* hyp, float* ent, void* corr, int corr_format, int B,
                           int V, int C, int D, int H, int W, hipStream_t st);
int launch_corr_aggregate(const void* corr, int corr_format, const float* vis, void* vol, int volume_format, int B, int V, int D, int H, int W,
                          hipStream_t st);
int pack_features_dispatch(const void* in, int in_dtype, void* out, int out_dtype, int N, int C, int H, int W, hipStream_t st);

static int gather_impl(int C, int G, int D, int H, int W) {
    const char* e = getenv("MVS_GATHER_IMPL");
    if (e && e[0] == 'd') return 0;
    return gl_supported(C, G, D, H, W) ? 1 : 0;
}

}

using namespace mvs;

static int volume_to_split(float* volume_cl, const float* vis_sum, int B, int D, int H, int W, int G, hipStream_t st, const char* who);

extern "C" int mvs_compose_homography(const float* proj, int B, int V, float* homography, void* stream) {
    if (!proj || !homography || B < 1 || V < 2) { set_error("mvs_compose_homography: bad arguments"); return MVS_ERR_ARG; }
    const int n = B * (V - 1);
    hipLaunchKernelGGL(compose_homography_kernel, dim3(ceil_div(n, 64)), dim3(64), 0, (hipStream_t)stream, proj, B, V, homography);
    return check_launch("compose_homography_kernel");
}

extern "C" int mvs_cascade_prologue_fwd(const float* const* proj_host_ptrs, int n_stages, int B, int V, float* homography, const float* depth_values,
                                       int N, int inverse, float* hyp, int D, int H, int W, void* stream) {
    if (!proj_host_ptrs || !homography || n_stages < 1 || n_stages > 8 || B < 1 || V < 2) { set_error("mvs_cascade_prologue_fwd: bad arguments (1..8 stages)"); return MVS_ERR_ARG; }
    if (hyp && (!depth_values || N < 1 || D < 2 || H < 1 || W < 1)) { set_error("mvs_cascade_prologue_fwd: bad hypothesis arguments"); return MVS_ERR_ARG; }
    ProloguePtrs pp;
    pp.n = n_stages;
    for (int i = 0; i < 8; ++i) {
        pp.proj[i] = i < n_stages ? proj_host_ptrs[i] : nullptr;
        if (i < n_stages && !pp.proj[i]) { set_error("mvs_cascade_prologue_fwd: null projection tensor of stage %d", i); return MVS_ERR_ARG; }
    }
    int init_blocks = 0;
    dim3 grid(1, 1, 1);
    if (hyp) {
        const int HW = H * W;
        init_blocks = (int)(ceil_div(HW, 1024) > 64 ? 64 : ceil_div(HW, 1024));
        grid = dim3(init_blocks + 1, D, B);
    }
    hipLaunchKernelGGL(cascade_prologue_kernel, grid, dim3(256), 0, (hipStream_t)stream, pp, B, V, homography, depth_values, N, inverse,
                       hyp, D, H * W, init_blocks);
    return check_launch("cascade_prologue_kernel");
}

extern "C" int mvs_homography_from_proj(const float* src_proj, const float* ref_proj, int B, float* homography, void* stream) {
    if (!src_proj || !ref_proj || !homography || B < 1) { set_error("mvs_homography_from_proj: bad arguments"); return MVS_ERR_ARG; }
    hipLaunchKernelGGL(homography_from_proj_kernel, dim3(ceil_div(B, 64)), dim3(64), 0, (hipStream_t)stream, src_proj, ref_proj, B, homography);
    return check_launch("homography_from_proj_kernel");
}

extern "C" int mvs_homo_warp_fwd(const void* src_fea, int dtype, const float* homography, const float* depth, int depth_is_volume,
                                 float* warped, uint8_t* proj_mask, int B, int C, int D, int H, int W, void* stream) {
    if (!src_fea || !homography || !depth || B < 1 || C < 1 || D < 1 || H < 1 || W < 1) { set_error("mvs_homo_warp_fwd: bad arguments"); return MVS_ERR_ARG; }
    const dim3 grid(ceil_div((long long)H * W, 64), ceil_div(D, 4) > 64 ? 64 : ceil_div(D, 4), B);
    hipStream_t st = (hipStream_t)stream;
    switch (dtype) {
        case MVS_DTYPE_F32: hipLaunchKernelGGL((homo_warp_kernel<MVS_DTYPE_F32>), grid, dim3(256), 0, st, src_fea, homography, depth, depth_is_volume, warped, proj_mask, C, D, H, W); break;
        case MVS_DTYPE_BF16: hipLaunchKernelGGL((homo_warp_kernel<MVS_DTYPE_BF16>), grid, dim3(256), 0, st, src_fea, homography, depth, depth_is_volume, warped, proj_mask, C, D, H, W); break;
        case MVS_DTYPE_F16: hipLaunchKernelGGL((homo_warp_kernel<MVS_DTYPE_F16>), grid, dim3(256), 0, st, src_fea, homography, depth, depth_is_volume, warped, proj_mask, C, D, H, W); break;
        default: set_error("mvs_homo_warp_fwd: bad dtype %d", dtype); return MVS_ERR_ARG;
    }
    return check_launch("homo_warp_kernel");
}

extern "C" int mvs_pack_features(const void* features, int dtype, void* tiled, int out_dtype, int N, int C, int H, int W, void* stream) {
    if (!features || !tiled || N < 1 || C < 8 || (C % 8) || H < 1 || W < 1 || dtype < 0 || dtype > 2 || out_dtype < 0 || out_dtype > 2) {
        set_error("mvs_pack_features: bad arguments (C must be a multiple of 8)");
        return MVS_ERR_ARG;
    }
    return pack_features_dispatch(features, dtype, tiled, out_dtype, N, C, H, W, (hipStream_t)stream);
}

static int check_layout(const char* who, int layout, int C, int G, int D, int H, int W) {
    if (layout == MVS_LAYOUT_PLANAR) return MVS_OK;
    if (layout != MVS_LAYOUT_OCTET_TILED) { set_error("%s: unknown feature layout %d", who, layout); return MVS_ERR_ARG; }
    if (!gl_supported(C, G, D, H, W)) {
        set_error("%s: the octet-tiled feature layout needs G == 8, C in {8,16,32,64} and W %% 8 == 0", who);
        return MVS_ERR_UNSUPPORTED;
    }
    return MVS_OK;
}

extern "C" int mvs_warp_corr_entropy_fwd(const void* features, int dtype, int layout, const float* homography, const float* hyp, float* entropy,
                                         int B, int V, int C, int G, int D, int H, int W, int view_begin, int view_end, int gather_format,
                                         void* stream) {
    int rc = check_corr_args("mvs_warp_corr_entropy_fwd", features, homography, hyp, dtype, B, V, C, G, D, H, W, view_begin, view_end);
    if (rc != MVS_OK) return rc;
    if (!entropy) { set_error("mvs_warp_corr_entropy_fwd: null output"); return MVS_ERR_ARG; }
    if (gather_format != MVS_GATHER_F32 && gather_format != MVS_GATHER_F16) { set_error("mvs_warp_corr_entropy_fwd: unknown gather format %d", gather_format); return MVS_ERR_ARG; }
    hipStream_t st = (hipStream_t)stream;
    rc = check_layout("mvs_warp_corr_entropy_fwd", layout, C, G, D, H, W);
    if (rc != MVS_OK) return rc;
    const int impl = gather_impl(C, G, D, H, W);
    if (layout == MVS_LAYOUT_OCTET_TILED || impl == 1)
        return gl_launch_entropy(features, dtype, layout, homography, hyp, entropy, B, V, C, D, H, W, view_begin, view_end, gather_format == MVS_GATHER_F16, st);
    switch (dtype) {
        case MVS_DTYPE_F32: MVS_DISPATCH_CG(launch_entropy, MVS_DTYPE_F32, features, homography, hyp, entropy, B, V, C, G, D, H, W, view_begin, view_end, st);
        case MVS_DTYPE_BF16: MVS_DISPATCH_CG(launch_entropy, MVS_DTYPE_BF16, features, homography, hyp, entropy, B, V, C, G, D, H, W, view_begin, view_end, st);
        default: MVS_DISPATCH_CG(launch_entropy, MVS_DTYPE_F16, features, homography, hyp, entropy, B, V, C, G, D, H, W, view_begin, view_end, st);
    }
}

extern "C" int mvs_gather_keeps_correlations(int layout, int C, int G, int D, int H, int W) {
    if (layout != MVS_LAYOUT_OCTET_TILED && gather_impl(C, G, D, H, W) != 1) return 0;
    return gl_keep_supported(C, G, D, H, W) ? 1 : 0;
}

extern "C" int mvs_warp_corr_entropy_keep_fwd(const void* features, int dtype, int layout, const float* homography, const float* hyp, float* entropy,
                                              void* corr, int corr_format, int B, int V, int C, int G, int D, int H, int W, void* stream) {
    int rc = check_corr_args("mvs_warp_corr_entropy_keep_fwd", features, homography, hyp, dtype, B, V, C, G, D, H, W, 1, V);
    if (rc != MVS_OK) return rc;
    if (!entropy || !corr) { set_error("mvs_warp_corr_entropy_keep_fwd: null output"); return MVS_ERR_ARG; }
    if (corr_format != MVS_CORR_F16 && corr_format != MVS_CORR_F32) { set_error("mvs_warp_corr_entropy_keep_fwd: unknown correlation format %d", corr_format); return MVS_ERR_ARG; }
    rc = check_layout("mvs_warp_corr_entropy_keep_fwd", layout, C, G, D, H, W);
    if (rc != MVS_OK) return rc;
    if (!gl_keep_supported(C, G, D, H, W) || (corr_format == MVS_CORR_F32 && !gl_keep32_supported(C, G, D, H, W))) {
        set_error("mvs_warp_corr_entropy_keep_fwd: built for the LDS-staged gather (G == 8, C in {8,16,32,64}, W %% 8 == 0; MVS_CORR_F32: D > 4 as well); "
                  "mvs_gather_keeps_correlations() says which shapes qualify");
        return MVS_ERR_UNSUPPORTED;
    }
    return gl_launch_entropy_keep(features, dtype, layout, homography, hyp, entropy, corr, corr_format, B, V, C, D, H, W, (hipStream_t)stream);
}

extern "C" int mvs_corr_aggregate_fwd(const void* corr, int corr_format, const float* vis, void* volume_cl, int volume_format, int B, int V, int D,
                                      int H, int W, void* stream) {
    if (!corr || !vis || !volume_cl) { set_error("mvs_corr_aggregate_fwd: null pointer"); return MVS_ERR_ARG; }
    if (corr_format != MVS_CORR_F16 && corr_format != MVS_CORR_F32) { set_error("mvs_corr_aggregate_fwd: unknown correlation format %d", corr_format); return MVS_ERR_ARG; }
    if (B < 1 || V < 2 || D < 1 || H < 1 || W < 1 || (long long)D * H * W > 0x7fffffffLL) { set_error("mvs_corr_aggregate_fwd: bad shape"); return MVS_ERR_ARG; }
    if (volume_format != MVS_VOLUME_F32 && volume_format != MVS_VOLUME_SPLIT && volume_format != MVS_VOLUME_F16) { set_error("mvs_corr_aggregate_fwd: unknown volume format %d", volume_format); return MVS_ERR_ARG; }
    return launch_corr_aggregate(corr, corr_format, vis, volume_cl, volume_format, B, V, D, H, W, (hipStream_t)stream);
}

extern "C" int mvs_warp_corr_aggregate_fwd(const void* features, int dtype, int layout, const float* homography, const float* hyp, const float* vis,
                                           float* volume_cl, float* vis_sum, int normalise, int volume_format, int B, int V, int C, int G,
                                           int D, int H, int W, int view_begin, int view_end, void* stream) {
    int rc = check_corr_args("mvs_warp_corr_aggregate_fwd", features, homography, hyp, dtype, B, V, C, G, D, H, W, view_begin, view_end);
    if (rc != MVS_OK) return rc;
    if (!vis || !volume_cl) { set_error("mvs_warp_corr_aggregate_fwd: null pointer"); return MVS_ERR_ARG; }
    if (!normalise && !vis_sum) { set_error("mvs_warp_corr_aggregate_fwd: partial mode needs vis_sum"); return MVS_ERR_ARG; }
    if (volume_format != MVS_VOLUME_F32 && volume_format != MVS_VOLUME_SPLIT && volume_format != MVS_VOLUME_F16) { set_error("mvs_warp_corr_aggregate_fwd: unknown volume format %d", volume_format); return MVS_ERR_ARG; }
    if (volume_format != MVS_VOLUME_F32 && (!normalise || G != 8)) {
        set_error("mvs_warp_corr_aggregate_fwd: the split / fp16 volume formats hold the NORMALISED volume of 8 groups (partial sums stay fp32)");
        return MVS_ERR_UNSUPPORTED;
    }
    hipStream_t st = (hipStream_t)stream;
    rc = check_layout("mvs_warp_corr_aggregate_fwd", layout, C, G, D, H, W);
    if (rc != MVS_OK) return rc;
    const int impl = gather_impl(C, G, D, H, W);
    if (layout == MVS_LAYOUT_OCTET_TILED || impl == 1)
        return gl_launch_aggregate(features, dtype, layout, homography, hyp, vis, volume_cl, vis_sum, normalise | (volume_format << 1), B, V, C, D, H, W, view_begin, view_end, st);
    if (volume_format == MVS_VOLUME_F16) {
        set_error("mvs_warp_corr_aggregate_fwd: the fp16 volume is written by the LDS-staged gather only (C in {8,16,32,64}, W %% 8 == 0); "
                  "for other shapes aggregate in MVS_VOLUME_F32 and convert with mvs_volume_to_f16");
        return MVS_ERR_UNSUPPORTED;
    }
    if (volume_format == MVS_VOLUME_SPLIT) {
        rc = mvs_warp_corr_aggregate_fwd(features, dtype, layout, homography, hyp, vis, volume_cl, vis_sum, normalise, MVS_VOLUME_F32, B, V, C, G, D, H, W,
                                         view_begin, view_end, stream);
        return rc != MVS_OK ? rc : volume_to_split(volume_cl, nullptr, B, D, H, W, G, st, "mvs_warp_corr_aggregate_fwd");
    }
    switch (dtype) {
        case MVS_DTYPE_F32: MVS_DISPATCH_CG(launch_aggregate, MVS_DTYPE_F32, features, homography, hyp, vis, volume_cl, vis_sum, normalise, B, V, C, G, D, H, W, view_begin, view_end, st);
        case MVS_DTYPE_BF16: MVS_DISPATCH_CG(launch_aggregate, MVS_DTYPE_BF16, features, homography, hyp, vis, volume_cl, vis_sum, normalise, B, V, C, G, D, H, W, view_begin, view_end, st);
        default: MVS_DISPATCH_CG(launch_aggregate, MVS_DTYPE_F16, features, homography, hyp, vis, volume_cl, vis_sum, normalise, B, V, C, G, D, H, W, view_begin, view_end, st);
    }
}

static int volume_to_split(float* volume_cl, const float* vis_sum, int B, int D, int H, int W, int G, hipStream_t st, const char* who) {
    if (G != 8) { set_error("%s: the split volume format needs 8 groups", who); return MVS_ERR_UNSUPPORTED; }
    const size_t nvox = (size_t)B * D * H * W;
    const unsigned grid = (unsigned)((nvox + 255) / 256 > 16384 ? 16384 : (nvox + 255) / 256);
    hipLaunchKernelGGL(volume_to_split_kernel, dim3(grid), dim3(256), 0, st, volume_cl, vis_sum, D, H * W, nvox);
    return check_launch("volume_to_split_kernel");
}

static bool slab_args(const char* who, const float* volume_cl, const float* vis_sum, float* const* bufs, const int* r0, const int* r1, int n, int B, int D,
                      int H, int W, int G, SlabMsgs* m) {
    if (!volume_cl || !vis_sum || !bufs || !r0 || !r1 || n < 1 || n > kMaxShardRanks || B < 1 || D < 1 || H < 1 || W < 1 || G < 1) {
        set_error("%s: bad arguments (1..%d ranks)", who, kMaxShardRanks);
        return false;
    }
    m->n = n;
    for (int j = 0; j < kMaxShardRanks; ++j) {
        m->ptr[j] = j < n ? bufs[j] : nullptr;
        m->r0[j] = j < n ? r0[j] : 0;
        m->r1[j] = j < n ? r1[j] : 0;
        if (j < n && bufs[j] != nullptr && (r0[j] < 0 || r1[j] > H || r1[j] < r0[j])) { set_error("%s: rows [%d, %d) outside the volume", who, r0[j], r1[j]); return false; }
    }
    return true;
}

extern "C" int mvs_slab_pack(const float* volume_cl, const float* vis_sum, float* const* send_host_ptrs, const int* row_begin, const int* row_end,
                             int n_ranks, int B, int D, int H, int W, int G, void* stream) {
    SlabMsgs m;
    if (!slab_args("mvs_slab_pack", volume_cl, vis_sum, send_host_ptrs, row_begin, row_end, n_ranks, B, D, H, W, G, &m)) return MVS_ERR_ARG;
    hipLaunchKernelGGL(slab_pack_kernel, dim3(1024, n_ranks), dim3(256), 0, (hipStream_t)stream, volume_cl, vis_sum, m, B, D, H, W, G);
    return check_launch("slab_pack_kernel");
}

extern "C" int mvs_slab_reduce(const float* volume_cl, const float* vis_sum, float* const* recv_host_ptrs, int n_ranks, int my_rank, float* slab_out,
                               int row_begin, int row_end, int B, int D, int H, int W, int G, void* stream) {
    int r0[kMaxShardRanks], r1[kMaxShardRanks];
    for (int j = 0; j < kMaxShardRanks; ++j) { r0[j] = row_begin; r1[j] = row_end; }
    SlabMsgs m;
    if (!slab_out || my_rank < 0 || my_rank >= n_ranks || row_begin < 0 || row_end > H || row_end <= row_begin ||
        !slab_args("mvs_slab_reduce", volume_cl, vis_sum, recv_host_ptrs, r0, r1, n_ranks, B, D, H, W, G, &m)) {
        if (!slab_out || my_rank < 0 || my_rank >= n_ranks || row_begin < 0 || row_end > H || row_end <= row_begin) set_error("mvs_slab_reduce: bad arguments");
        return MVS_ERR_ARG;
    }
    hipLaunchKernelGGL(slab_reduce_kernel, dim3(2048), dim3(256), 0, (hipStream_t)stream, volume_cl, vis_sum, m, my_rank, slab_out, row_begin, row_end, B, D, H,
                       W, G);
    return check_launch("slab_reduce_kernel");
}

extern "C" int mvs_gather_is_lds_staged(int layout, int C, int G, int D, int H, int W) {
    return (layout == MVS_LAYOUT_OCTET_TILED || gather_impl(C, G, D, H, W) == 1) ? 1 : 0;
}

extern "C" int mvs_volume_to_f16(const float* volume_cl, const float* vis_sum, void* out_f16, int B, int D, int H, int W, int G, void* stream) {
    if (!volume_cl || !out_f16 || B < 1 || D < 1 || H < 1 || W < 1) { set_error("mvs_volume_to_f16: bad arguments"); return MVS_ERR_ARG; }
    if (G != 8) { set_error("mvs_volume_to_f16: the fp16 volume format needs 8 groups"); return MVS_ERR_UNSUPPORTED; }
    const size_t nvox = (size_t)B * D * H * W;
    const unsigned grid = (unsigned)((nvox + 255) / 256 > 16384 ? 16384 : (nvox + 255) / 256);
    hipLaunchKernelGGL(volume_to_f16_kernel, dim3(grid), dim3(256), 0, (hipStream_t)stream, volume_cl, vis_sum, static_cast<_Float16*>(out_f16), D, H * W, nvox);
    return check_launch("volume_to_f16_kernel");
}

extern "C" int mvs_volume_normalise(float* volume_cl, const float* vis_sum, int B, int D, int H, int W, int G, int volume_format, void* stream) {
    if (!volume_cl || !vis_sum || B < 1 || D < 1 || H < 1 || W < 1 || G < 1) { set_error("mvs_volume_normalise: bad arguments"); return MVS_ERR_ARG; }
    if (volume_format == MVS_VOLUME_SPLIT) return volume_to_split(volume_cl, vis_sum, B, D, H, W, G, (hipStream_t)stream, "mvs_volume_normalise");
    if (volume_format != MVS_VOLUME_F32) { set_error("mvs_volume_normalise: unknown volume format %d", volume_format); return MVS_ERR_ARG; }
    const size_t total = (size_t)B * D * H * W * G;
    const unsigned grid = (unsigned)((total + 255) / 256 > 8192 ? 8192 : (total + 255) / 256);
// ... 6 lines not shown
```

### mvsformerplusplus_amd/ops.py

```python
from __future__ import annotations

import ctypes as C
import os
from typing import List, Optional, Sequence, Tuple

import torch

from . import _lib
from ._lib import check, lib, ptr, stream_of


def _f32c(t: torch.Tensor) -> torch.Tensor:
    return t.contiguous() if t.dtype == torch.float32 else t.float().contiguous()


class PackedFeatures:

    def __init__(self, data: torch.Tensor):
        assert data.dim() == 6 and data.shape[-1] == 8 and data.is_contiguous(), "PackedFeatures wants a dense [B,V,C/8,H,W,8] tensor"
        self.data = data

    @property
    def shape(self):
        B, V, O, H, W, _ = self.data.shape
# ... 169 lines not shown


def fmt_merge(prev: torch.Tensor, lateral: torch.Tensor, w_reduce: torch.Tensor) -> torch.Tensor:
    prev, lateral, w_reduce, N, C, h, w, H, W = _fmt_level(prev, lateral, w_reduce)
    out = torch.empty_like(lateral)
    check(lib().mvs_fmt_merge_fwd(ptr(prev), ptr(lateral), ptr(w_reduce), ptr(out), N, C, h, w, H, W, stream_of(lateral)), "mvs_fmt_merge_fwd")
    return out


def fmt_smooth(x: torch.Tensor, w_packed: torch.Tensor) -> torch.Tensor:
    x = _planar32(x)
    N, C, H, W = x.shape
    _fmt_smooth_weights(w_packed, C)
    out = torch.empty_like(x)
    check(lib().mvs_fmt_smooth_fwd(ptr(x), ptr(w_packed), ptr(out), N, C, H, W, stream_of(x)), "mvs_fmt_smooth_fwd")
    return out


def _feat(t) -> Tuple[torch.Tensor, int]:
    if isinstance(t, PackedFeatures):
        return t, _lib.DTYPE_CODE[t.dtype]
    if t.dtype not in _lib.DTYPE_CODE:
        t = t.float()
    return t.contiguous(), _lib.DTYPE_CODE[t.dtype]


def _feat_ptr(features):
    if isinstance(features, PackedFeatures):
        return features.data, _lib.LAYOUT_OCTET_TILED
    return features, _lib.LAYOUT_PLANAR


def compose_homography(proj_matrices: torch.Tensor) -> torch.Tensor:
    p = _f32c(proj_matrices)
    B, V = p.shape[:2]
    assert p.shape[2:] == (2, 4, 4), "proj_matrices must be [B,V,2,4,4]"
    out = torch.empty(B, V - 1, 12, dtype=torch.float32, device=p.device)
    check(lib().mvs_compose_homography(ptr(p), B, V, ptr(out), stream_of(p)), "mvs_compose_homography")
    return out


def cascade_prologue(proj_matrices: Sequence[torch.Tensor], depth_values: Optional[torch.Tensor] = None, ndepths: int = 0, H: int = 0, W: int = 0,
                     inverse: bool = True):
    ps = [_f32c(p) for p in proj_matrices]
    B, V = ps[0].shape[:2]
    for p in ps:
        assert p.shape == (B, V, 2, 4, 4), "proj_matrices must be [B,V,2,4,4] with the same B, V on every stage"
    hom = torch.empty(len(ps), B, V - 1, 12, dtype=torch.float32, device=ps[0].device)
    hyp, dv, N = None, None, 0
    if depth_values is not None:
        dv = _f32c(depth_values)
        assert dv.dim() == 2 and dv.shape[0] == B, "depth_values must be [B,N] (per-pixel ranges go through init_range)"
        N = dv.shape[1]
        hyp = torch.empty(B, ndepths, H, W, dtype=torch.float32, device=dv.device)
    pa = _ptr_array(ps)
    check(lib().mvs_cascade_prologue_fwd(C.cast(pa, C.c_void_p), len(ps), B, V, ptr(hom), ptr(dv), N, 1 if inverse else 0, ptr(hyp), ndepths, H, W,
                                         stream_of(ps[0])), "mvs_cascade_prologue_fwd")
    return list(hom.unbind(0)), hyp


def homography_from_proj(src_proj: torch.Tensor, ref_proj: torch.Tensor) -> torch.Tensor:
    s, r = _f32c(src_proj), _f32c(ref_proj)
    B = s.shape[0]
    out = torch.empty(B, 12, dtype=torch.float32, device=s.device)
    check(lib().mvs_homography_from_proj(ptr(s), ptr(r), B, ptr(out), stream_of(s)), "mvs_homography_from_proj")
    return out


def homo_warp(src_fea: torch.Tensor, homography: torch.Tensor, depth_values: torch.Tensor,
              want_warped: bool = True, want_mask: bool = True):
    f, code = _feat(src_fea)
    B, Cc, H, W = f.shape
    dv = _f32c(depth_values)
    D = dv.shape[1]
    is_vol = 1 if dv.dim() == 4 else 0
    warped = torch.empty(B, Cc, D, H, W, dtype=torch.float32, device=f.device) if want_warped else None
    mask = torch.empty(B, D, H, W, dtype=torch.uint8, device=f.device) if want_mask else None
    check(lib().mvs_homo_warp_fwd(ptr(f), code, ptr(homography.contiguous()), ptr(dv), is_vol, ptr(warped), ptr(mask),
                                  B, Cc, D, H, W, stream_of(f)), "mvs_homo_warp_fwd")
    return warped, (mask.bool() if mask is not None else None)


def warp_corr_entropy(features: torch.Tensor, code: int, homography: torch.Tensor, hyp: torch.Tensor, G: int,
                      view_begin: int = 1, view_end: Optional[int] = None, out: Optional[torch.Tensor] = None, f16_window: bool = False) -> torch.Tensor:
    B, V, Cc, H, W = features.shape
    D = hyp.shape[1]
    view_end = V if view_end is None else view_end
    if out is not None:
        ent = out
    elif view_begin == 1 and view_end == V:
        ent = torch.empty(B, V - 1, H, W, dtype=torch.float32, device=features.device)
    else:
        ent = torch.zeros(B, V - 1, H, W, dtype=torch.float32, device=features.device)
    ft, layout = _feat_ptr(features)
    check(lib().mvs_warp_corr_entropy_fwd(ptr(ft), code, layout, ptr(homography), ptr(hyp), ptr(ent), B, V, Cc, G, D, H, W,
                                          view_begin, view_end, 1 if f16_window else 0, stream_of(ft)), "mvs_warp_corr_entropy_fwd")
    return ent


def vis_weight(entropy: torch.Tensor, params: Sequence[torch.Tensor], precision: int = 0) -> torch.Tensor:
    e = _f32c(entropy)
    H, W = e.shape[-2:]
    N = e.numel() // (H * W)
    vis = torch.empty_like(e)
    nbytes = lib().mvs_vis_workspace_bytes(N, H, W, precision)
    ws = torch.empty(max(nbytes // 4, 4), dtype=torch.float32, device=e.device)
    check(lib().mvs_vis_weight_fwd(ptr(e), *[ptr(p) for p in params], ptr(vis), ptr(ws), nbytes, N, H, W, precision, stream_of(e)),
          "mvs_vis_weight_fwd")
    return vis


def vis_conv1(entropy: torch.Tensor, w1: torch.Tensor, b1: torch.Tensor) -> torch.Tensor:
    e = _f32c(entropy)
    H, W = e.shape[-2:]
    N = e.numel() // (H * W)
    out = torch.empty(N, H, W, 16, dtype=torch.float32, device=e.device)
    check(lib().mvs_vis_conv1_fwd(ptr(e), ptr(w1), ptr(b1), ptr(out), N, H, W, stream_of(e)), "mvs_vis_conv1_fwd")
    return out


def vis_out(x_cl8: torch.Tensor, w4: torch.Tensor, b4: torch.Tensor, shape) -> torch.Tensor:
    N, H, W, _ = x_cl8.shape
    vis = torch.empty(shape, dtype=torch.float32, device=x_cl8.device)
    check(lib().mvs_vis_out_fwd(ptr(x_cl8), ptr(w4), ptr(b4), ptr(vis), N, H, W, stream_of(x_cl8)), "mvs_vis_out_fwd")
    return vis


def warp_corr_aggregate(features: torch.Tensor, code: int, homography: torch.Tensor, hyp: torch.Tensor, vis: torch.Tensor,
                        G: int, normalise: bool = True, view_begin: int = 1, view_end: Optional[int] = None, out=None, split: bool = False,
                        f16: bool = False):
    B, V, Cc, H, W = features.shape
    D = hyp.shape[1]
    view_end = V if view_end is None else view_end
    if out is not None:
        vol, vsum = out
    else:
        vol = torch.empty(B, D, H, W, G, dtype=torch.float16 if f16 else torch.float32, device=features.device)
        vsum = None if normalise else torch.empty(B, H, W, dtype=torch.float32, device=features.device)
    ft, layout = _feat_ptr(features)
    check(lib().mvs_warp_corr_aggregate_fwd(ptr(ft), code, layout, ptr(homography), ptr(hyp), ptr(vis), ptr(vol), ptr(vsum),
                                            1 if normalise else 0, _lib.VOLUME_F16 if f16 else (_lib.VOLUME_SPLIT if split else _lib.VOLUME_F32), B, V, Cc, G, D, H, W,
                                            view_begin, view_end, stream_of(ft)), "mvs_warp_corr_aggregate_fwd")
    return vol, vsum


def warp_corr_aggregate_bwd(features: torch.Tensor, code: int, homography: torch.Tensor, hyp: torch.Tensor, vis: torch.Tensor,
                            vis_sum: torch.Tensor, volume_cl: torch.Tensor, grad_volume_cl: torch.Tensor, G: int):
    B, V, Cc, H, W = features.shape
    D = hyp.shape[1]
    gfeat = torch.empty(B, V, Cc, H, W, dtype=torch.float32, device=features.device)
    gvis = torch.empty(B, V - 1, H, W, dtype=torch.float32, device=features.device)
    check(lib().mvs_warp_corr_aggregate_bwd(ptr(features), code, ptr(homography), ptr(hyp), ptr(vis), ptr(vis_sum), ptr(volume_cl),
                                            ptr(grad_volume_cl), ptr(gfeat), ptr(gvis), B, V, Cc, G, D, H, W, stream_of(features)),
          "mvs_warp_corr_aggregate_bwd")
    return gfeat, gvis


def volume_normalise_(vol_cl: torch.Tensor, vis_sum: torch.Tensor, split: bool = False) -> torch.Tensor:
    B, D, H, W, G = vol_cl.shape
    check(lib().mvs_volume_normalise(ptr(vol_cl), ptr(vis_sum), B, D, H, W, G, _lib.VOLUME_SPLIT if split else _lib.VOLUME_F32,
                                     stream_of(vol_cl)), "mvs_volume_normalise")
    return vol_cl


def gather_is_lds_staged(features, G: int, hyp: torch.Tensor) -> bool:
    B, V, Cc, H, W = features.shape
    _, layout = _feat_ptr(features)
    return bool(lib().mvs_gather_is_lds_staged(layout, Cc, G, hyp.shape[1], H, W))


def gather_keeps_correlations(features, G: int, hyp: torch.Tensor) -> bool:
    B, V, Cc, H, W = features.shape
    _, layout = _feat_ptr(features)
    return bool(lib().mvs_gather_keeps_correlations(layout, Cc, G, hyp.shape[1], H, W))


def warp_corr_entropy_keep(features, code: int, homography: torch.Tensor, hyp: torch.Tensor, G: int, exact: bool = False) -> Tuple[torch.Tensor, torch.Tensor]:
    B, V, Cc, H, W = features.shape
    D = hyp.shape[1]
    ft, layout = _feat_ptr(features)
    ent = torch.empty(B, V - 1, H, W, dtype=torch.float32, device=ft.device)
    corr = torch.empty(B, V - 1, D, H, W, 8, dtype=torch.float32 if exact else torch.float16, device=ft.device)
    check(lib().mvs_warp_corr_entropy_keep_fwd(ptr(ft), code, layout, ptr(homography), ptr(hyp), ptr(ent), ptr(corr),
                                               _lib.CORR_F32 if exact else _lib.CORR_F16, B, V, Cc, G, D, H, W, stream_of(ft)),
          "mvs_warp_corr_entropy_keep_fwd")
    return ent, corr


def corr_aggregate(corr: torch.Tensor, vis: torch.Tensor, split: bool = False, f16: bool = True) -> torch.Tensor:
    assert corr.dtype in (torch.float16, torch.float32) and corr.is_contiguous() and corr.dim() == 6 and corr.shape[-1] == 8
    B, NV, D, H, W, _ = corr.shape
    v = _f32c(vis)
    assert v.shape == (B, NV, H, W)
    f16 = f16 and not split
    vol = torch.empty(B, D, H, W, 8, dtype=torch.float16 if f16 else torch.float32, device=corr.device)
    fmt = _lib.VOLUME_F16 if f16 else (_lib.VOLUME_SPLIT if split else _lib.VOLUME_F32)
    cfmt = _lib.CORR_F32 if corr.dtype == torch.float32 else _lib.CORR_F16
    check(lib().mvs_corr_aggregate_fwd(ptr(corr), cfmt, ptr(v), ptr(vol), fmt, B, NV + 1, D, H, W, stream_of(corr)), "mvs_corr_aggregate_fwd")
    return vol


def f16_saturation_count(reset: bool = False, device=None) -> int:
    if device is not None and torch.device(device).type == "cuda":
        with torch.cuda.device(device):
            return int(lib().mvs_f16_saturation_count(1 if reset else 0))
    return int(lib().mvs_f16_saturation_count(1 if reset else 0))


def volume_to_f16(vol_cl: torch.Tensor, vis_sum: Optional[torch.Tensor] = None) -> torch.Tensor:
    B, D, H, W, G = vol_cl.shape
    out = torch.empty(B, D, H, W, G, dtype=torch.float16, device=vol_cl.device)
    check(lib().mvs_volume_to_f16(ptr(vol_cl), ptr(vis_sum), ptr(out), B, D, H, W, G, stream_of(vol_cl)), "mvs_volume_to_f16")
    return out


def slab_pack(vol_cl: torch.Tensor, vis_sum: torch.Tensor, send_bufs, rows) -> None:
    import ctypes as C
    B, D, H, W, G = vol_cl.shape
    n = len(send_bufs)
    fn = lib().mvs_slab_pack
    ptrs = (C.c_void_p * n)(*[None if b is None else ptr(b) for b in send_bufs])
    r0 = (C.c_int * n)(*[int(r[0]) for r in rows])
# ... 657 lines not shown
```

### mvsformerplusplus_amd/profiling.py

```python
from __future__ import annotations

from collections import OrderedDict
from typing import Dict, List, Sequence, Tuple

import torch

from . import _lib, ops
from .cascade import CascadeDepthHead

PEAK_HBM_GBS = 8000.0
PEAK_F32_MFMA_TFLOPS = 157.3
PEAK_F16_MFMA_TFLOPS = 2500.0


def match_kernel(label: str, table: dict):
    import re
    keys = [k for k in table if not k.startswith("_")]
    if label in table:
        return label
    base = label.split(" ")[0].split("+")[0]
    cands = []
    m = re.match(r"conv3d_mfma<(\d+),(\d+),k(\d),s(\d)(\d)(\d)>", base)
    if m:
        cin, cout, kd, sd, sh, sw = m.groups()
# ... 143 lines not shown
    P = net._cache.get(net, net._build, "bf16x3")
    prec = _lib.PREC_BF16X3
    B, D, H, W, _ = vol.shape
    rate = net.rate
    n = (D // rate[0]) * (H // rate[1]) * (W // rate[2])
    kp = 8 * rate[0] * rate[1] * rate[2]
    T = B * n
    x = _timed(launches, "tr_gemm<embed>", stage, 2.0 * T * kp * 64, 4.0 * (vol.numel() + (3 * B * D * H * W if pos is not None else 0) + T * 64),
               lambda: ops.tr_embed(vol, pos, P["pe_w"], P["pe_div"], P["down_w"], P["down_b"], *P["down_ln"], rate, prec))
    scale = (64 // net.num_heads) ** -0.5
    if net.softmax_scale == "entropy_invariance":
        scale *= math.log(n, net.train_avg_length)
    for L in P["layers"]:
        a = _timed(launches, "[bundle] tr_gemm<qkv>+tr_attention", stage, 2.0 * T * 64 * 192 + 4.0 * B * n * n * 64,
                   4.0 * T * (64 + 64) + 2.0 * T * 192 * 2, lambda: ops.tr_attention(x, L["qkv"], net.num_heads, scale, prec, net.attention_code()))
        x = _timed(launches, "tr_gemm<res_ln,64>", stage, 2.0 * T * 64 * 64, 4.0 * T * 64 * 3,
                   lambda: ops.tr_linear(a, L["proj"], L["proj_b"], _lib.TR_EPI_RES_LN, 64, prec, residual=x, gamma=L["g1"],
                                         ln_w=L["n1"][0], ln_b=L["n1"][1], ln_eps=L["n1"][2]))
        hdn = _timed(launches, "tr_gemm<gelu>", stage, 2.0 * T * 64 * 256, 4.0 * T * (64 + 256),
                     lambda: ops.tr_linear(x, L["l1"], L["l1_b"], _lib.TR_EPI_GELU, 256, prec))
        x = _timed(launches, "tr_gemm<res_ln,256>", stage, 2.0 * T * 256 * 64, 4.0 * T * (256 + 128),
                   lambda: ops.tr_linear(hdn, L["l2"], L["l2_b"], _lib.TR_EPI_RES_LN, 64, prec, residual=x, gamma=L["g2"],
                                         ln_w=L["n2"][0], ln_b=L["n2"][1], ln_eps=L["n2"][2]))
    return _timed(launches, "tr_gemm<up>", stage, 2.0 * T * 64 * kp, 4.0 * (T * 64 + B * D * H * W),
                  lambda: ops.tr_up_prob(x, P["up_w"], P["up_b"], *P["up_ln"], P["prob_w"], P["prob_b"], (D, H, W), rate, prec))


@torch.no_grad()
def profile_cascade(head: CascadeDepthHead, features, proj_matrices, depth_values, tmp=(5.0, 5.0, 5.0, 1.0)) -> Tuple[dict, List[Launch]]:
    launches: List[Launch] = []
    n = len(head.ndepths)
    out = None
    confs = []
    final_conf = None
    pe_range = None
    if depth_values.is_cuda:
        torch.cuda._sleep(int(2.0e7))
    H0, W0 = features["stage1"].shape[-2:]
    B0 = depth_values.shape[0]
    homs, hyp0 = _timed(launches, "cascade_prologue", 0, 0, 4.0 * B0 * head.ndepths[0] * H0 * W0,
                        lambda: ops.cascade_prologue([proj_matrices["stage%d" % (i + 1)] for i in range(n)], depth_values, head.ndepths[0], H0, W0,
                                                     inverse=head.inverse_depth))
    for s in range(n):
        key = "stage%d" % (s + 1)
        net = head.fusions[s]
        _CUR_PREC[0] = net.conv_precision
        feats, code = ops._feat(features[key])
        proj = proj_matrices[key]
        B, V, C, H, W = feats.shape
        D = head.ndepths[s]
        HW = H * W
        esz = feats.element_size()
        if s == 0:
            hyp = hyp0
        elif out.get("next_hyp") is not None:
            hyp = out["next_hyp"]
        else:
            pd, ph = out["depth"], out["depth_values"]
            hyp = _timed(launches, "schedule_range", s, 0, 4.0 * (B * D * HW + 3 * B * HW / 4),
                         lambda: ops.schedule_inverse_range(pd, ph, D, head.depth_interals_ratio[s], H, W))
        hom = homs[s]
        last = s == n - 1
        cprev = list(confs) if last else None
        sched = (not last and head.inverse_depth and D >= 3 and tuple(features["stage%d" % (s + 2)].shape[-2:]) == (2 * H, 2 * W))
        Dn = head.ndepths[s + 1] if not last else 0
        rn = head.depth_interals_ratio[s + 1] if not last else 0.0

        def run_head(lg):
            if sched:
                return ops.softmax_regress_schedule(lg, hyp, tmp[s], _lib.HEAD_CE_EVAL, 0, net.return_prob_volumes, Dn, rn)
            return ops.softmax_regress(lg, hyp, tmp[s], _lib.HEAD_CE_EVAL, 0, net.return_prob_volumes, conf_prev=cprev)
        head_label = "prob_regress_sched_kernel" if sched else "softmax_regress_kernel"
        head_bytes = 4.0 * B * ((2 + int(bool(net.return_prob_volumes))) * D * HW + 2 * HW + (HW if last else 0) + (4 * Dn * HW if sched else 0))
        corr_flops = 2.0 * (V - 1) * B * D * HW * C * 5
        tiled = isinstance(feats, ops.PackedFeatures)
        keep = net._keeps_correlations(feats, 8, hyp)
        w16 = net.gather_precision == "f16"
        corr_bytes = B * (V - 1) * D * HW * (16.0 if w16 else 32.0)
        if keep:
            ent, corr = _timed(launches, gather_kernel_name("entropy", code, C, D, W, tiled, True, w16), s, corr_flops,
                               B * (V * C * HW * esz + D * HW * 4 + (V - 1) * HW * 4) + corr_bytes,
                               lambda: ops.warp_corr_entropy_keep(feats, code, hom, hyp, 8, exact=not w16))
        else:
            ent = _timed(launches, gather_kernel_name("entropy", code, C, D, W, tiled, False, w16), s, corr_flops, B * (V * C * HW * esz + D * HW * 4 + (V - 1) * HW * 4),
                         lambda: ops.warp_corr_entropy(feats, code, hom, hyp, 8, f16_window=w16))
        vp = net._vis_params(feats.device)
        prec = _lib.PRECISIONS[net._vis_precision()]
        N = B * (V - 1)
        vis_flops = 2.0 * N * HW * (9 * 16 + 9 * 16 * 16 + 9 * 16 * 8 + 8)
        if net._vis_precision() in ("bf16x3",) + _lib.F16_FORMATS:
            vis = _timed(launches, "vis_cnn_kernel", s, vis_flops, 4.0 * N * HW * 2, lambda: ops.vis_weight(ent, vp, prec))
        else:
            t1 = _timed(launches, "vis_conv1", s, 2.0 * N * HW * 9 * 16, 4.0 * N * HW * 17, lambda: ops.vis_conv1(ent, vp[0], vp[1]))
            t1 = t1.reshape(1, N, H, W, 16)
            t2 = _timed(launches, _conv_name(16, 16, 1, (1, 1, 1)), s, 2.0 * N * HW * 9 * 16 * 16, 4.0 * N * HW * 32,
                        lambda: ops.conv3d_bn_relu(t1, vp[2], vp[3], 16, 1, (1, 1, 1), True, prec))
            t3 = _timed(launches, _conv_name(16, 8, 1, (1, 1, 1)), s, 2.0 * N * HW * 9 * 16 * 8, 4.0 * N * HW * 24,
                        lambda: ops.conv3d_bn_relu(t2, vp[4], vp[5], 8, 1, (1, 1, 1), True, prec))
            vis = _timed(launches, "vis_out", s, 2.0 * N * HW * 8, 4.0 * N * HW * 9,
                         lambda: ops.vis_out(t3.reshape(N, H, W, 8), vp[6], vp[7], ent.shape))
        split = net._split_activations()
        f16 = net._f16_activations()
        agg_name = gather_kernel_name("aggregate", code, C, D, W, tiled, w16=f16 and ops.gather_is_lds_staged(feats, 8, hyp))
        if keep:
            vol = _timed(launches, "corr_aggregate_kernel", s, 2.0 * B * (V - 1) * D * HW * 8, corr_bytes + B * ((V - 1) * HW * 4 + 8 * D * HW * (2 if f16 else 4)),
                         lambda: ops.corr_aggregate(corr, vis, split=split, f16=f16))
            del corr
        elif f16 and not ops.gather_is_lds_staged(feats, 8, hyp):
            v32 = _timed(launches, agg_name, s, corr_flops, B * (V * C * HW * esz + D * HW * 4 + (V - 1) * HW * 4 + 8 * D * HW * 4),
                         lambda: ops.warp_corr_aggregate(feats, code, hom, hyp, vis, 8, normalise=True)[0])
            vol = _timed(launches, "volume_to_f16", s, 0, B * 8 * D * HW * 6.0, lambda: ops.volume_to_f16(v32))
        else:
            vol = _timed(launches, agg_name, s, corr_flops,
                         B * (V * C * HW * esz + D * HW * 4 + (V - 1) * HW * 4 + 8 * D * HW * (2 if f16 else 4)),
                         lambda: ops.warp_corr_aggregate(feats, code, hom, hyp, vis, 8, split=split, f16=f16)[0])
        if getattr(net.cost_reg, "kind", None) == "transformer":
            pos = None
            if head.use_pe3d:
                pr = pe_range
                pos, pe_range = _timed(launches, "[bundle] pos3d", s, 0, 4.0 * 4 * B * D * HW,
                                       lambda: ops.position3d(proj[:, 0, 1, :3, :3], hyp, depth_values, pr))
            logits = _transformer_layers(net.cost_reg, vol, pos, s, launches)
            r3 = _timed(launches, head_label, s, 0, head_bytes, lambda: run_head(logits))
            out = {"depth": r3[0], "photometric_confidence": r3[1], "depth_values": hyp, "next_hyp": r3[3] if sched else None}
            confs.append(r3[1])
            if last:
                final_conf = r3[3]
            continue
        ks = net.cost_reg.prob_ksize
        if ks == 1 and net.conv_precision in _lib.F16_FORMATS + ("bf16x3",) and net.fuse_prob_head:
            logits = _regnet_layers(net.cost_reg, vol, s, launches, net.conv_precision, fused_head=True, split=split)
            r3 = _timed(launches, head_label, s, 0, head_bytes, lambda: run_head(logits))
            out = {"depth": r3[0], "photometric_confidence": r3[1], "depth_values": hyp, "next_hyp": r3[3] if sched else None}
            confs.append(r3[1])
            if last:
                final_conf = r3[3]
            continue
        feat_cl = _regnet_layers(net.cost_reg, vol, s, launches, net.conv_precision, split=split)
        ws, bs, prob_w, prob_b = net.cost_reg.packed_all(feats.device, net.conv_precision)
        if ks == 3 and net.conv_precision in _lib.F16_FORMATS + ("bf16x3",):
            logits = _timed(launches, "conv3d_mfma<8,1,k3,s111> prob head", s, 2.0 * B * D * HW * 8 * 27, B * (float(feat_cl.element_size()) * 8 * D * HW + 4.0 * D * HW),
                            lambda: ops.conv3d_logits(feat_cl, prob_w, prob_b, _lib.PREC_BF16X3_SPLIT if split else _lib.PRECISIONS[net.conv_precision]))
            r3 = _timed(launches, head_label, s, 0, head_bytes, lambda: run_head(logits))
            out = {"depth": r3[0], "photometric_confidence": r3[1], "depth_values": hyp, "next_hyp": r3[3] if sched else None}
            confs.append(r3[1])
            if last:
                final_conf = r3[3]
            continue
        res = _timed(launches, "prob_regress_kernel<%d,%d>" % (D, ks), s, 2.0 * B * D * HW * 8 * (27 if ks == 3 else 1),
                     4.0 * B * (8 * D * HW + D * HW + 2 * D * HW + 2 * HW),
                     lambda: ops.prob_regress(feat_cl, prob_w, prob_b, ks, hyp, tmp[s], _lib.HEAD_CE_EVAL, 0, net.return_prob_volumes))
        out = {"depth": res[0], "photometric_confidence": res[1], "depth_values": hyp}
        confs.append(res[1])
    Hf, Wf = features["stage%d" % n].shape[-2:]
    if final_conf is None:
        final_conf = _timed(launches, "confidence_average", n - 1, 0, 4.0 * Hf * Wf * 2, lambda: ops.confidence_average(confs, Hf, Wf))
    torch.cuda.synchronize()
    for l in launches:
        l.ms = l.start.elapsed_time(l.end)
    return {"refined_depth": out["depth"], "photometric_confidence": final_conf}, launches


def summarize(launches: Sequence[Launch]) -> "OrderedDict[str, dict]":
    agg: "OrderedDict[str, dict]" = OrderedDict()
    for l in launches:
        a = agg.setdefault(l.kernel, {"calls": 0, "ms": 0.0, "flops": 0.0, "bytes": 0.0, "issued_flops": 0.0})
        a["calls"] += 1
        a["ms"] += l.ms
        a["flops"] += l.flops
        a["bytes"] += l.bytes
        a["issued_flops"] += l.flops * (mfma_terms(l.kernel, l.prec) if l.prec else 1)
    for a in agg.values():
        t = max(a["ms"], 1e-9) * 1e-3
        a["avg_ms"] = a["ms"] / a["calls"]
        a["gbs"] = a["bytes"] / t / 1e9
        a["tflops"] = a["flops"] / t / 1e12
    return agg
```

Measured before the change: 677.0.

## Record gather window boxes in entropy pass and reuse them in aggregate pass

The entropy gather kernel now writes each tile's per-view bounding box of sampled pixels to a small buffer. The aggregate gather reads these boxes back instead of recomputing them with a wave reduction and block barrier. A pipelined aggregate path double-buffers the staged LDS window across views using the known boxes. This trades a small extra global buffer and added code complexity for fewer reductions and syncs, plus overlap of window staging with the blend.

```diff
diff --git a/include/mvs_hip.h b/include/mvs_hip.h
--- a/include/mvs_hip.h
+++ b/include/mvs_hip.h
@@ -71,6 +71,15 @@
                     int row_begin, int row_end, int B, int D, int H, int W, int G, void* stream);
 int mvs_volume_normalise(float* volume_cl, const float* vis_sum, int B, int D, int H, int W, int G, int volume_format, void* stream);
 int mvs_gather_is_lds_staged(int layout, int C, int G, int D, int H, int W);
+
+int mvs_gather_boxes_dims(int D, int H, int W, int* iterations, int* tiles);
+int mvs_warp_corr_entropy_boxes_fwd(const void* features, int dtype, int layout, const float* homography , const float* hyp,
+                                    float* entropy, unsigned* boxes, int B, int V, int C, int G, int D, int H, int W, int view_begin,
+                                    int view_end, int gather_format, void* stream);
+int mvs_warp_corr_aggregate_boxes_fwd(const void* features, int dtype, int layout, const float* homography, const float* hyp,
+                                      const float* vis, float* volume_cl, float* vis_sum, int normalise, int volume_format,
+                                      const unsigned* boxes, int B, int V, int C, int G, int D, int H, int W, int view_begin, int view_end,
+                                      void* stream);
 int mvs_volume_to_f16(const float* volume_cl, const float* vis_sum, void* out_f16, int B, int D, int H, int W, int G, void* stream);
 
 int mvs_warp_corr_aggregate_bwd(const void* features, int dtype, const float* homography, const float* hyp, const float* vis,
diff --git a/mvsformerplusplus_amd/_lib.py b/mvsformerplusplus_amd/_lib.py
--- a/mvsformerplusplus_amd/_lib.py
+++ b/mvsformerplusplus_amd/_lib.py
@@ -47,6 +47,9 @@
     "mvs_volume_to_f16": (_i, [_vp, _vp, _vp, _i, _i, _i, _i, _i, _vp]),
     "mvs_gather_is_lds_staged": (_i, [_i, _i, _i, _i, _i, _i]),
     "mvs_gather_keeps_correlations": (_i, [_i, _i, _i, _i, _i, _i]),
+    "mvs_gather_boxes_dims": (_i, [_i, _i, _i, _vp, _vp]),
+    "mvs_warp_corr_entropy_boxes_fwd": (_i, [_vp, _i, _i, _vp, _vp, _vp, _vp] + [_i] * 10 + [_vp]),
+    "mvs_warp_corr_aggregate_boxes_fwd": (_i, [_vp, _i, _i, _vp, _vp, _vp, _vp, _vp, _i, _i, _vp] + [_i] * 9 + [_vp]),
     "mvs_warp_corr_entropy_keep_fwd": (_i, [_vp, _i, _i, _vp, _vp, _vp, _vp] + [_i] * 8 + [_vp]),
     "mvs_corr_aggregate_fwd": (_i, [_vp, _i, _vp, _vp] + [_i] * 6 + [_vp]),
     "mvs_slab_pack": (_i, [_vp, _vp, _vp, _vp, _vp, _i, _i, _i, _i, _i, _i, _vp]),
diff --git a/mvsformerplusplus_amd/cost_volume.py b/mvsformerplusplus_amd/cost_volume.py
--- a/mvsformerplusplus_amd/cost_volume.py
+++ b/mvsformerplusplus_amd/cost_volume.py
@@ -189,12 +189,14 @@
                 volume = ops.corr_aggregate(corr, vis, split=split, f16=f16)
                 del corr
             else:
-                entropy = ops.warp_corr_entropy(feats, code, hom, hyp, G, f16_window=w16)
+                staged = ops.gather_is_lds_staged(feats, G, hyp)
+                boxes = ops.gather_boxes(feats, hyp) if staged else None
+                entropy = ops.warp_corr_entropy(feats, code, hom, hyp, G, f16_window=w16, boxes=boxes)
                 vis = ops.vis_weight(entropy, vis_params, prec)
-                if f16 and not ops.gather_is_lds_staged(feats, G, hyp):
+                if f16 and not staged:
                     volume = ops.volume_to_f16(ops.warp_corr_aggregate(feats, code, hom, hyp, vis, G, normalise=True)[0])
                 else:
-                    volume, _ = ops.warp_corr_aggregate(feats, code, hom, hyp, vis, G, normalise=True, split=split, f16=f16)
+                    volume, _ = ops.warp_corr_aggregate(feats, code, hom, hyp, vis, G, normalise=True, split=split, f16=f16, boxes=boxes)
         out = self._regularise_and_regress(volume, hyp, depth_values, float(tmp), position3d, split=split, conf_prev=conf_prev, nxt=nxt)
         if conf_prev is not None:
             _fused["conf_avg"] = out.pop("_conf_avg")
diff --git a/mvsformerplusplus_amd/csrc/gather_lds.h b/mvsformerplusplus_amd/csrc/gather_lds.h
--- a/mvsformerplusplus_amd/csrc/gather_lds.h
+++ b/mvsformerplusplus_amd/csrc/gather_lds.h
@@ -50,10 +50,167 @@
         wv[2 * j + 1] = MVS_FMA_MIX_HI(t11[j], tp.w11, wv[2 * j + 1]);                                 \
     }
 
-template <typename T, int NOCT, bool KEEP_GROUPS, bool TILED, bool W16, bool DIRECT = false>
+template <typename T, int R>
+__device__ __forceinline__ void gl_stage_load(__amdgpu_buffer_rsrc_t srs, unsigned planeb, unsigned gbase, int W, int ww, float inv_ww, int n, int i0,
+                                              float (&v)[R][8]) {
+#pragma unroll
+    for (int k = 0; k < R; ++k) {
+        const int i = i0 + 256 * k;
+        if (i < n) {
+#if MVS_GL_ABL == 1
+#pragma unroll
+            for (int c = 0; c < 8; ++c) v[k][c] = (float)(i & 7);
+#else
+            const int row = (int)(((float)i + 0.5f) * inv_ww);
+            const unsigned g = gbase + (unsigned)row * (unsigned)(W - ww) + (unsigned)i;
+#pragma unroll
+            for (int c = 0; c < 8; ++c) {
+                if constexpr (sizeof(T) == 4)
+                    v[k][c] = __builtin_bit_cast(float, __builtin_amdgcn_raw_buffer_load_b32(srs, (int)(g * 4u), (int)((unsigned)c * planeb), 0));
+                else
+                    v[k][c] = to_f32(__builtin_bit_cast(T, (unsigned short)__builtin_amdgcn_raw_buffer_load_b16(srs, (int)(g * 2u), (int)((unsigned)c * planeb), 0)));
+            }
+#endif
+        }
+    }
+}
+template <bool W16, int R>
+__device__ __forceinline__ void gl_stage_store(f32x4* w, int n, int i0, const float (&v)[R][8]) {
+    typedef _Float16 h8 __attribute__((ext_vector_type(8)));
+#pragma unroll
+    for (int k = 0; k < R; ++k) {
+        const int i = i0 + 256 * k;
+        if (i < n) {
+            if (W16) {
+                h8 hv;
+#pragma unroll
+                for (int c = 0; c < 8; ++c) hv[c] = (_Float16)__builtin_amdgcn_fmed3f(v[k][c], -65504.0f, 65504.0f);
+                reinterpret_cast<h8*>(w)[i] = hv;
+            } else {
+                w[i] = f32x4{v[k][0], v[k][1], v[k][2], v[k][3]};
+                w[GL_CAP + i] = f32x4{v[k][4], v[k][5], v[k][6], v[k][7]};
+            }
+        }
+    }
+}
+
+template <int NOCT, bool KEEP_GROUPS, bool W16>
+__device__ __forceinline__ void gl_gather_octet(const f32x4* w, const unsigned* pos, int ww, const GTap* tp, float* rf, float wscale, int o, float* out) {
+    constexpr int GPO = 8 / NOCT;
+    constexpr int CPG = NOCT;
+#pragma unroll
+    for (int c = 0; c < 8; ++c) rf[c] *= wscale;
+#pragma unroll
+    for (int dd = 0; dd < GL_DCH; ++dd) {
+        if (dd == 2) __builtin_amdgcn_sched_barrier(0);
+        float wv[8];
+        if (W16) {
+            typedef unsigned u32x4 __attribute__((ext_vector_type(4)));
+            const u32x4* w0 = reinterpret_cast<const u32x4*>(w) + pos[dd];
+#if MVS_GL_ABL == 3
+            const u32x4 t00 = {pos[dd], 0x3c003c00u, 0x3c003c00u, pos[dd]}, t01 = t00, t10 = {0x3c003c00u, pos[dd], pos[dd], 0x3c003c00u}, t11 = t10;
+#else
+            const u32x4 t00 = w0[0], t01 = w0[1], t10 = w0[ww], t11 = w0[ww + 1];
+#endif
+#if MVS_GL_ABL == 4
+#pragma unroll
+            for (int j = 0; j < 4; ++j) { wv[2 * j] = __builtin_bit_cast(float, (t00[j] ^ t01[j] ^ t10[j] ^ t11[j]) & 0x3fffffffu); wv[2 * j + 1] = tp[dd].w00; }
+#elif MVS_GL_OPT
+            GL_BLEND8(wv, t00, t01, t10, t11, tp[dd])
+#else
+#pragma unroll
+            for (int j = 0; j < 4; ++j) {
+                float a = MVS_FMA_MIX_LO(t00[j], tp[dd].w00, 0.0f);
+                a = MVS_FMA_MIX_LO(t01[j], tp[dd].w01, a);
+                a = MVS_FMA_MIX_LO(t10[j], tp[dd].w10, a);
+                wv[2 * j] = MVS_FMA_MIX_LO(t11[j], tp[dd].w11, a);
+                float b = MVS_FMA_MIX_HI(t00[j], tp[dd].w00, 0.0f);
+                b = MVS_FMA_MIX_HI(t01[j], tp[dd].w01, b);
+                b = MVS_FMA_MIX_HI(t10[j], tp[dd].w10, b);
+                wv[2 * j + 1] = MVS_FMA_MIX_HI(t11[j], tp[dd].w11, b);
+            }
+#endif
+        } else {
+            const f32x4* w0 = w + pos[dd];
+            const f32x4 a0 = w0[0], a1 = w0[1], b0 = w0[ww], b1 = w0[ww + 1];
+            const f32x4 c0 = w0[GL_CAP], c1 = w0[GL_CAP + 1], d0 = w0[GL_CAP + ww], d1 = w0[GL_CAP + ww + 1];
+            f32x4 lo = a0 * tp[dd].w00;
+            lo += a1 * tp[dd].w01;
+            lo += b0 * tp[dd].w10;
+            lo += b1 * tp[dd].w11;
+            f32x4 hi = c0 * tp[dd].w00;
+            hi += c1 * tp[dd].w01;
+            hi += d0 * tp[dd].w10;
+            hi += d1 * tp[dd].w11;
+            wv[0] = lo[0]; wv[1] = lo[1]; wv[2] = lo[2]; wv[3] = lo[3]; wv[4] = hi[0]; wv[5] = hi[1]; wv[6] = hi[2]; wv[7] = hi[3];
+        }
+        if (KEEP_GROUPS) {
+#pragma unroll
+            for (int j = 0; j < GPO; ++j) {
+                float s = out[(o * GPO + j) * GL_DCH + dd];
+#pragma unroll
+                for (int c = 0; c < CPG; ++c) s += rf[j * CPG + c] * wv[j * CPG + c];
+                out[(o * GPO + j) * GL_DCH + dd] = s;
+            }
+        } else {
+            float s = out[dd];
+#pragma unroll
+            for (int c = 0; c < 8; ++c) s += rf[c] * wv[c];
+            out[dd] = s;
+        }
+    }
+}
+
+template <typename T, int NOCT, bool KEEP_GROUPS, bool TILED, bool W16>
+__device__ __forceinline__ void gl_unit_global(const T* __restrict__ src, const T* __restrict__ ref, const GTap* tp, int W, unsigned HW, unsigned pc,
+                                               float wscale, float* out) {
+    typedef typename PairOf<T>::type P2;
+    constexpr int CPG = NOCT;
+    unsigned top[GL_DCH];
+#pragma unroll
+    for (int dd = 0; dd < GL_DCH; ++dd) top[dd] = tp[dd].pk == GL_NONE ? 0u : (tp[dd].pk >> 16) * (unsigned)W + (tp[dd].pk & 0xffffu);
+#pragma unroll 1
+    for (int c = 0; c < 8 * NOCT; ++c) {
+        const unsigned cbase = TILED ? (unsigned)(c >> 3) * 8u * HW + (unsigned)(c & 7) : (unsigned)c * HW;
+        const unsigned pstep = TILED ? 8u : 1u;
+        const float rfc = to_f32(ref[cbase + pc * pstep]) * wscale;
+        const T* sp = src + cbase;
+        const int g = c / CPG;
+#pragma unroll
+        for (int dd = 0; dd < GL_DCH; ++dd) {
+            float t0, t1, b0, b1;
+            if (TILED) {
+                __builtin_amdgcn_sched_barrier(0);
+                t0 = to_f32(sp[top[dd] * 8u]); t1 = to_f32(sp[(top[dd] + 1u) * 8u]);
+                b0 = to_f32(sp[(top[dd] + (unsigned)W) * 8u]); b1 = to_f32(sp[(top[dd] + (unsigned)W + 1u) * 8u]);
+            } else {
+                const P2 t = *reinterpret_cast<const P2*>(sp + top[dd]);
+                const P2 b = *reinterpret_cast<const P2*>(sp + top[dd] + (unsigned)W);
+                t0 = to_f32(t.x); t1 = to_f32(t.y); b0 = to_f32(b.x); b1 = to_f32(b.y);
+            }
+            if (W16) {
+                t0 = gl_round_f16(t0); t1 = gl_round_f16(t1); b0 = gl_round_f16(b0); b1 = gl_round_f16(b1);
+            }
+            float wv = tp[dd].w00 * t0;
+            wv += tp[dd].w01 * t1;
+            wv += tp[dd].w10 * b0;
+            wv += tp[dd].w11 * b1;
+            if (KEEP_GROUPS) {
+#pragma unroll
+                for (int gg = 0; gg < 8; ++gg) out[gg * GL_DCH + dd] += (g == gg) ? rfc * wv : 0.0f;
+            } else {
+                out[dd] += rfc * wv;
+            }
+        }
+    }
+}
+
+template <typename T, int NOCT, bool KEEP_GROUPS, bool TILED, bool W16, bool DIRECT = false, bool BOXES = false>
 __device__ __forceinline__ void gl_unit(const T* __restrict__ src, const T* __restrict__ ref, const Homography& hm, float fx, float fy,
                                         const float* depth, bool active, int H, int W, unsigned HW, unsigned pc, f32x4* win,
-                                        unsigned* red, int unit, float wscale, const float* rf_in, float* out) {
+                                        unsigned* red, int unit, float wscale, const float* rf_in, float* out,
+                                        const unsigned* box_in = nullptr, unsigned* box_out = nullptr) {
+    static_assert(!(BOXES && DIRECT), "the direct form has no window");
     typedef typename PairOf<T>::type P2;
     constexpr int GPO = 8 / NOCT;
     constexpr int CPG = NOCT;
@@ -73,9 +230,11 @@
 #else
         tp[dd] = make_gtap(hm, qx, qy, qz, depth[dd], H, W, cx, cy);
 #endif
-        const u16x2 pkv = gl_as_vec(tp[dd].pk);
-        mn = __builtin_elementwise_min(mn, pkv);
-        mx = __builtin_elementwise_max(mx, (u16x2)(pkv + (u16x2){1, 1}));
+        if constexpr (!BOXES) {
+            const u16x2 pkv = gl_as_vec(tp[dd].pk);
+            mn = __builtin_elementwise_min(mn, pkv);
+            mx = __builtin_elementwise_max(mx, (u16x2)(pkv + (u16x2){1, 1}));
+        }
     }
     if (!active) { mn = (u16x2){0xffff, 0xffff}; mx = (u16x2){0, 0}; }
 #else
@@ -170,6 +329,10 @@
         }
         return;
     }
+    if constexpr (BOXES) {
+        mn = gl_as_vec(box_in[0]);
+        mx = gl_as_vec(box_in[1]);
+    } else
 #if MVS_GL_ABL == 5
     {
         __syncthreads();
@@ -181,15 +344,18 @@
         for (int dd = 0; dd < GL_DCH; ++dd) tp[dd].pk = ((by + 1u + (unsigned)(lane & 3)) << 16) | (bx + 1u + (unsigned)(lane & 63));
     }
 #else
-    mn = gl_wave_reduce<false>(mn);
-    mx = gl_wave_reduce<true>(mx);
-    unsigned* rd = red + (unit & 1) * 8;
-    if (lane == 63) { rd[wave] = gl_as_u32(mn); rd[4 + wave] = gl_as_u32(mx); }
-    __syncthreads();
-    mn = __builtin_elementwise_min(__builtin_elementwise_min(gl_as_vec(rd[0]), gl_as_vec(rd[1])),
-                                   __builtin_elementwise_min(gl_as_vec(rd[2]), gl_as_vec(rd[3])));
-    mx = __builtin_elementwise_max(__builtin_elementwise_max(gl_as_vec(rd[4]), gl_as_vec(rd[5])),
-                                   __builtin_elementwise_max(gl_as_vec(rd[6]), gl_as_vec(rd[7])));
+    {
+        mn = gl_wave_reduce<false>(mn);
+        mx = gl_wave_reduce<true>(mx);
+        unsigned* rd = red + (unit & 1) * 8;
+        if (lane == 63) { rd[wave] = gl_as_u32(mn); rd[4 + wave] = gl_as_u32(mx); }
+        __syncthreads();
+        mn = __builtin_elementwise_min(__builtin_elementwise_min(gl_as_vec(rd[0]), gl_as_vec(rd[1])),
+                                       __builtin_elementwise_min(gl_as_vec(rd[2]), gl_as_vec(rd[3])));
+        mx = __builtin_elementwise_max(__builtin_elementwise_max(gl_as_vec(rd[4]), gl_as_vec(rd[5])),
+                                       __builtin_elementwise_max(gl_as_vec(rd[6]), gl_as_vec(rd[7])));
+        if (box_out != nullptr && tid == 0) { box_out[0] = gl_as_u32(mn); box_out[1] = gl_as_u32(mx); }
+    }
 #endif
 #if MVS_GL_OPT
     const int xmin = mn[0], ymin = mn[1], xmax = (int)mx[0] - 1, ymax = (int)mx[1] - 1;
@@ -386,6 +552,7 @@
                 }
             }
         }
+        if constexpr (BOXES) __syncthreads();
     } else if (active) {
         unsigned top[GL_DCH];
 #pragma unroll
@@ -424,6 +591,115 @@
                 }
             }
         }
+    }
+}
+
+#ifndef MVS_GL_PIPE
+#define MVS_GL_PIPE 1
+#endif
+template <typename T, bool TILED, bool W16, int NOCT>
+constexpr bool gl_pipe_v = (MVS_GL_PIPE != 0) && (MVS_GL_OPT != 0) && (MVS_GL_ABL == 0 || MVS_GL_ABL == 1) && !TILED && NOCT == 1;
+
+struct GlBox {
+    int wx0, ymin, ww, n;
+};
+__device__ __forceinline__ GlBox gl_box_decode(const unsigned* bx) {
+    const u16x2 mn = gl_as_vec(bx[0]), mx = gl_as_vec(bx[1]);
+    const int xmin = mn[0], ymin = mn[1], xmax = (int)mx[0] - 1, ymax = (int)mx[1] - 1;
+    GlBox b;
+    b.wx0 = xmin & ~(GL_XALIGN - 1);
+    b.ymin = ymin;
+    b.ww = (xmax + 2 - b.wx0 + GL_XALIGN - 1) & ~(GL_XALIGN - 1);
+    b.n = xmax < xmin ? 0 : b.ww * (ymax + 2 - ymin);
+    return b;
+}
+
+template <typename T, bool W16>
+__device__ __forceinline__ void gl_stage_window(const T* so, unsigned HW, int W, const GlBox& bx, f32x4* w) {
+    const __amdgpu_buffer_rsrc_t srs = __builtin_amdgcn_make_buffer_rsrc(const_cast<T*>(so), 0, (int)(8u * HW * (unsigned)sizeof(T)), 0x00020000);
+    const unsigned planeb = HW * (unsigned)sizeof(T);
+    const float inv_ww = __builtin_amdgcn_rcpf((float)bx.ww) * 1.000001f;
+    const unsigned gbase = (unsigned)bx.ymin * (unsigned)W + (unsigned)bx.wx0;
+#pragma unroll 1
+    for (int i0 = (int)threadIdx.x; i0 < bx.n; i0 += 256 * MVS_GL_SB) {
+        float v[MVS_GL_SB][8];
+        gl_stage_load<T, MVS_GL_SB>(srs, planeb, gbase, W, bx.ww, inv_ww, bx.n, i0, v);
+        gl_stage_store<W16, MVS_GL_SB>(w, bx.n, i0, v);
+    }
+}
+
+template <typename T, bool W16>
+__device__ __forceinline__ void gl_aggregate_pipe(const T* __restrict__ feat, const float* __restrict__ hom, const float* __restrict__ vp,
+                                                  const unsigned* __restrict__ boxes, size_t bvs, float fx, float fy, const float* depth, bool active,
+                                                  int H, int W, unsigned HW, unsigned pc, f32x4* win, int view_begin, int view_end, int pipe,
+                                                  const float* rf0, float* acc) {
+    constexpr int CAPP = W16 ? 2 * GL_CAP : GL_CAP, HALF = CAPP / 2;
+    constexpr int R = HALF / 256;
+    const int tid = (int)threadIdx.x;
+    const float cx = 0.5f * (float)(W - 1), cy = 0.5f * (float)(H - 1);
+    int half = 0;
+    bool staged = false;
+    GlBox bx = gl_box_decode(boxes + (size_t)(view_begin - 1) * bvs);
+    for (int v = view_begin; v < view_end; ++v) {
+        GlBox nb;
+        nb.wx0 = nb.ymin = nb.ww = nb.n = 0;
+        if (v + 1 < view_end) nb = gl_box_decode(boxes + (size_t)v * bvs);
+        if (bx.n != 0) {
+            const Homography hm = gl_load_homography(hom + (size_t)(v - 1) * 12);
+            const float wscale = vp[(unsigned)(v - 1) * HW];
+            const T* src = feat + (size_t)v * 8 * HW;
+            const float qx = hm.r[0] * fx + hm.r[1] * fy + hm.r[2];
+            const float qy = hm.r[3] * fx + hm.r[4] * fy + hm.r[5];
+            const float qz = hm.r[6] * fx + hm.r[7] * fy + hm.r[8];
+            GTap tp[GL_DCH];
+            if (bx.n > CAPP) {
+#pragma unroll
+                for (int dd = 0; dd < GL_DCH; ++dd) tp[dd] = make_gtap(hm, qx, qy, qz, depth[dd], H, W, cx, cy);
+                if (active) gl_unit_global<T, 1, true, false, W16>(src, feat, tp, W, HW, pc, wscale, acc);
+            } else {
+                const bool fits = bx.n <= HALF;
+                f32x4* wv = win + (fits ? half * HALF : 0);
+                if (!staged) {
+                    gl_stage_window<T, W16>(src, HW, W, bx, wv);
+                    __syncthreads();
+                }
+                const bool pf = pipe != 0 && fits && nb.n != 0 && nb.n <= HALF;
+                f32x4* wn = win + (half ^ 1) * HALF;
+                const __amdgpu_buffer_rsrc_t nrs =
+                    __builtin_amdgcn_make_buffer_rsrc(const_cast<T*>(src + (size_t)8 * HW), 0, (int)(8u * HW * (unsigned)sizeof(T)), 0x00020000);
+                const unsigned planeb = HW * (unsigned)sizeof(T);
+                const float ninv = __builtin_amdgcn_rcpf((float)nb.ww) * 1.000001f;
+                const unsigned ngbase = (unsigned)nb.ymin * (unsigned)W + (unsigned)nb.wx0;
+                float pv[R][8];
+#pragma unroll
+                for (int k = 0; k < R; ++k) {
+#pragma unroll
+                    for (int c = 0; c < 8; ++c) pv[k][c] = 0.0f;
+                }
+                if (pf) gl_stage_load<T, R>(nrs, planeb, ngbase, W, nb.ww, ninv, nb.n, tid, pv);
+                __builtin_amdgcn_sched_barrier(0);
+                unsigned pos[GL_DCH];
+#pragma unroll
+                for (int dd = 0; dd < GL_DCH; ++dd) {
+                    tp[dd] = make_gtap(hm, qx, qy, qz, depth[dd], H, W, cx, cy);
+                    const unsigned pk = tp[dd].pk;
+                    const unsigned raw = ((pk >> 16) - (unsigned)bx.ymin) * (unsigned)bx.ww + ((pk & 0xffffu) - (unsigned)bx.wx0);
+                    pos[dd] = raw < (unsigned)(bx.n - bx.ww - 2) ? raw : (unsigned)(bx.n - bx.ww - 2);
+                }
+                __builtin_amdgcn_sched_barrier(0);
+                if (pf) gl_stage_store<W16, R>(wn, nb.n, tid, pv);
+                if (active) {
+                    float rf[8];
+#pragma unroll
+                    for (int c = 0; c < 8; ++c) rf[c] = rf0[c];
+                    gl_gather_octet<1, true, W16>(wv, pos, bx.ww, tp, rf, wscale, 0, acc);
+                }
+                __syncthreads();
+                staged = pf;
+                if (pf) half ^= 1;
+            }
+        }
+        bx = nb;
     }
 }
 
@@ -455,7 +731,8 @@
 __global__ __launch_bounds__(256) void gl_entropy_kernel(const void* __restrict__ feat_, const float* __restrict__ hom,
                                                          const float* __restrict__ hyp, float* __restrict__ entropy,
                                                          void* __restrict__ corr, int V, int D, int H,
-                                                         int W, int view_begin, int view_end, int vpb, int ntx, int nblk) {
+                                                         int W, int view_begin, int view_end, int vpb, int ntx, int nblk,
+                                                         unsigned* __restrict__ boxes) {
     typedef typename FeatT<DT>::type T;
     constexpr bool DIRECT = gl_direct_v<T, TILED, W16, NOCT, KEEP>;
     HIP_DYNAMIC_SHARED(float, smem)
@@ -466,7 +743,8 @@
     constexpr int TP = GlTile<NS>::TP;
     const unsigned HW = (unsigned)H * (unsigned)W;
     const int b = (int)blockIdx.z;
-    const GlTile<NS> t((int)xcd_remap(blockIdx.x, (unsigned)nblk), ntx, H, W);
+    const unsigned blk = xcd_remap(blockIdx.x, (unsigned)nblk);
+    const GlTile<NS> t((int)blk, ntx, H, W);
     const int nch = (D + GL_DCH - 1) / GL_DCH, niter = (nch + NS - 1) / NS;
     const T* feat = reinterpret_cast<const T*>(feat_) + (size_t)(b * V) * C * HW;
     const T* ref = feat;
@@ -494,11 +772,12 @@
             for (int dd = 0; dd < GL_DCH; ++dd) depth[dd] = hp[(unsigned)(d0 + dd < D ? d0 + dd : D - 1) * HW + t.pc];
 #pragma unroll
             for (int dd = 0; dd < GL_DCH; ++dd) s[dd] = 0.0f;
+            unsigned* bxo = (KEEP || boxes == nullptr) ? nullptr : boxes + ((((size_t)(b * (V - 1) + (v - 1))) * niter + it) * nblk + blk) * 2;
             if (KEEP) {
                 float acc[8 * GL_DCH];
 #pragma unroll
                 for (int i = 0; i < 8 * GL_DCH; ++i) acc[i] = 0.0f;
-                gl_unit<T, NOCT, true, TILED, W16, DIRECT>(src, ref, hm, t.fx, t.fy, depth, active, H, W, HW, t.pc, win, red, unit, inv_cpg, rf0, acc);
+                gl_unit<T, NOCT, true, TILED, W16, DIRECT>(src, ref, hm, t.fx, t.fy, depth, active, H, W, HW, t.pc, win, red, unit, inv_cpg, rf0, acc, nullptr, bxo);
                 typedef _Float16 h8 __attribute__((ext_vector_type(8)));
                 const size_t cbase = (size_t)(b * (V - 1) + (v - 1)) * D * HW + t.pc;
 #pragma unroll
@@ -523,7 +802,7 @@
                     }
                 }
             } else {
-                gl_unit<T, NOCT, false, TILED, W16, DIRECT>(src, ref, hm, t.fx, t.fy, depth, active, H, W, HW, t.pc, win, red, unit, inv_cpg, rf0, s);
+                gl_unit<T, NOCT, false, TILED, W16, DIRECT>(src, ref, hm, t.fx, t.fy, depth, active, H, W, HW, t.pc, win, red, unit, inv_cpg, rf0, s, nullptr, bxo);
             }
             if (NS > 1 || niter > 1) {
                 if (chunk < nch) {
@@ -563,7 +842,8 @@
 __global__ __launch_bounds__(256) void gl_aggregate_kernel(const void* __restrict__ feat_, const float* __restrict__ hom,
                                                            const float* __restrict__ hyp, const float* __restrict__ vis,
                                                            float* __restrict__ vol, float* __restrict__ vis_sum, int normalise, int V,
-                                                           int D, int H, int W, int view_begin, int view_end, int ntx, int nblk) {
+                                                           int D, int H, int W, int view_begin, int view_end, int ntx, int nblk,
+                                                           const unsigned* __restrict__ boxes, int pipe) {
     typedef typename FeatT<DT>::type T;
     HIP_DYNAMIC_SHARED(float, smem)
     f32x4* win = reinterpret_cast<f32x4*>(smem);
@@ -571,7 +851,8 @@
     constexpr int C = 8 * NOCT;
     const unsigned HW = (unsigned)H * (unsigned)W;
     const int b = (int)blockIdx.z, it = (int)blockIdx.y;
-    const GlTile<NS> t((int)xcd_remap(blockIdx.x, (unsigned)nblk), ntx, H, W);
+    const unsigned blk = xcd_remap(blockIdx.x, (unsigned)nblk);
+    const GlTile<NS> t((int)blk, ntx, H, W);
     const int nch = (D + GL_DCH - 1) / GL_DCH;
     const T* feat = reinterpret_cast<const T*>(feat_) + (size_t)(b * V) * C * HW;
     const T* ref = feat;
@@ -600,11 +881,30 @@
     float acc[8 * GL_DCH];
 #pragma unroll
     for (int i = 0; i < 8 * GL_DCH; ++i) acc[i] = 0.0f;
-    int unit = 0;
-    for (int v = view_begin; v < view_end; ++v, ++unit) {
-        const Homography hm = gl_load_homography(hom + (size_t)(b * (V - 1) + (v - 1)) * 12);
-        const float w = vp[(unsigned)(v - 1) * HW];
-        gl_unit<T, NOCT, true, TILED, W16, gl_direct_v<T, TILED, W16, NOCT, false>>(feat + (size_t)v * C * HW, ref, hm, t.fx, t.fy, depth, active, H, W, HW, t.pc, win, red, unit, inv_cpg * w, rf0, acc);
+    constexpr bool DIRECT = gl_direct_v<T, TILED, W16, NOCT, false>;
+    const size_t bvs = (size_t)gridDim.y * (unsigned)nblk * 2;
+    const unsigned* bxp = boxes == nullptr ? nullptr : boxes + ((size_t)(b * (V - 1)) * gridDim.y + (unsigned)it) * (unsigned)nblk * 2 + (size_t)blk * 2;
+    if (!DIRECT && bxp != nullptr) {
+        if constexpr (!DIRECT) {
+            if constexpr (gl_pipe_v<T, TILED, W16, NOCT>) {
+                gl_aggregate_pipe<T, W16>(feat, hom + (size_t)(b * (V - 1)) * 12, vp, bxp, bvs, t.fx, t.fy, depth, active, H, W, HW, t.pc, win, view_begin,
+                                          view_end, pipe, rf0, acc);
+            } else {
+                for (int v = view_begin; v < view_end; ++v) {
+                    const Homography hm = gl_load_homography(hom + (size_t)(b * (V - 1) + (v - 1)) * 12);
+                    const float w = vp[(unsigned)(v - 1) * HW];
+                    gl_unit<T, NOCT, true, TILED, W16, false, true>(feat + (size_t)v * C * HW, ref, hm, t.fx, t.fy, depth, active, H, W, HW, t.pc, win, red, 0,
+                                                                    inv_cpg * w, rf0, acc, bxp + (size_t)(v - 1) * bvs);
+                }
+            }
+        }
+    } else {
+        int unit = 0;
+        for (int v = view_begin; v < view_end; ++v, ++unit) {
+            const Homography hm = gl_load_homography(hom + (size_t)(b * (V - 1) + (v - 1)) * 12);
+            const float w = vp[(unsigned)(v - 1) * HW];
+            gl_unit<T, NOCT, true, TILED, W16, DIRECT>(feat + (size_t)v * C * HW, ref, hm, t.fx, t.fy, depth, active, H, W, HW, t.pc, win, red, unit, inv_cpg * w, rf0, acc);
+        }
     }
     if (active) {
         float* vb = vol + (size_t)b * D * HW * 8;
@@ -655,7 +955,7 @@
 
 template <int DT, int NOCT, int NS, bool TILED, bool KEEP = false, bool W16 = false>
 static int gl_launch_entropy_t(const void* feat, const float* hom, const float* hyp, float* ent, int B, int V, int D, int H, int W, int vb,
-                               int ve, hipStream_t st, void* corr = nullptr) {
+                               int ve, hipStream_t st, void* corr = nullptr, unsigned* boxes = nullptr) {
     constexpr int TP = 256 / NS, TW = TP / GL_TH;
     const int ntx = (int)ceil_div(W, TW), nty = (int)ceil_div(H, GL_TH);
     const int nblk = ntx * nty;
@@ -664,20 +964,21 @@
     if (lds > 48 * 1024)
         hipFuncSetAttribute(reinterpret_cast<const void*>(&gl_entropy_kernel<DT, NOCT, NS, TILED, KEEP, W16>), hipFuncAttributeMaxDynamicSharedMemorySize, (int)lds);
     hipLaunchKernelGGL((gl_entropy_kernel<DT, NOCT, NS, TILED, KEEP, W16>), dim3(nblk, ceil_div(ve - vb, vpb), B), dim3(256), lds, st, feat, hom, hyp, ent,
-                       corr, V, D, H, W, vb, ve, vpb, ntx, nblk);
+                       corr, V, D, H, W, vb, ve, vpb, ntx, nblk, boxes);
     return check_launch("gl_entropy_kernel");
 }
 
 template <int DT, int NOCT, int NS, bool TILED, bool W16 = false>
 static int gl_launch_aggregate_t(const void* feat, const float* hom, const float* hyp, const float* vis, float* vol, float* vis_sum,
-                                 int normalise, int B, int V, int D, int H, int W, int vb, int ve, hipStream_t st) {
+                                 int normalise, int B, int V, int D, int H, int W, int vb, int ve, hipStream_t st, const unsigned* boxes = nullptr,
+                                 int pipe = 0) {
     constexpr int TP = 256 / NS, TW = TP / GL_TH;
     const int ntx = (int)ceil_div(W, TW), nty = (int)ceil_div(H, GL_TH);
     const int nblk = ntx * nty;
     const int nch = (D + GL_DCH - 1) / GL_DCH, niter = (nch + NS - 1) / NS;
     const size_t lds = GL_WIN_BYTES + GL_RED_BYTES;
     hipLaunchKernelGGL((gl_aggregate_kernel<DT, NOCT, NS, TILED, W16>), dim3(nblk, niter, B), dim3(256), lds, st, feat, hom, hyp, vis, vol, vis_sum,
-                       normalise, V, D, H, W, vb, ve, ntx, nblk);
+                       normalise, V, D, H, W, vb, ve, ntx, nblk, boxes, pipe);
     return check_launch("gl_aggregate_kernel");
 }
 
diff --git a/mvsformerplusplus_amd/csrc/gather_lds_aggregate_kernels.hip b/mvsformerplusplus_amd/csrc/gather_lds_aggregate_kernels.hip
--- a/mvsformerplusplus_amd/csrc/gather_lds_aggregate_kernels.hip
+++ b/mvsformerplusplus_amd/csrc/gather_lds_aggregate_kernels.hip
@@ -3,13 +3,28 @@
 namespace mvs {
 
 int gl_launch_aggregate_w16(const void* feat, int dtype, int layout, const float* hom, const float* hyp, const float* vis, float* vol, float* vis_sum,
-                            int normalise, int B, int V, int C, int D, int H, int W, int vb, int ve, hipStream_t st);
+                            int normalise, int B, int V, int C, int D, int H, int W, int vb, int ve, hipStream_t st, const unsigned* boxes,
+                            int pipe);
+
+static int gl_pipe_choice() {
+    const char* sw = getenv("MVS_GATHER_PIPELINE");
+    if (sw && (sw[0] == '0' || sw[0] == '1') && sw[1] == 0) return sw[0] - '0';
+    return 1;
+}
+
+template <int DT, int NOCT, int NS, bool TILED>
+static int gl_launch_aggregate_f32_t(const void* feat, const float* hom, const float* hyp, const float* vis, float* vol, float* vis_sum,
+                                     int normalise, int B, int V, int D, int H, int W, int vb, int ve, hipStream_t st, const unsigned* boxes,
+                                     int pipe) {
+    return gl_launch_aggregate_t<DT, NOCT, NS, TILED, false>(feat, hom, hyp, vis, vol, vis_sum, normalise, B, V, D, H, W, vb, ve, st, boxes, pipe);
+}
 
 int gl_launch_aggregate(const void* feat, int dtype, int layout, const float* hom, const float* hyp, const float* vis, float* vol, float* vis_sum,
-                        int normalise, int B, int V, int C, int D, int H, int W, int vb, int ve, hipStream_t st) {
+                        int normalise, int B, int V, int C, int D, int H, int W, int vb, int ve, hipStream_t st, const unsigned* boxes) {
+    const int pipe = boxes != nullptr ? gl_pipe_choice() : 0;
     if ((normalise & 4) && gl_window_f16_enabled())
-        return gl_launch_aggregate_w16(feat, dtype, layout, hom, hyp, vis, vol, vis_sum, normalise, B, V, C, D, H, W, vb, ve, st);
-    GL_DISPATCH(gl_launch_aggregate_t, feat, hom, hyp, vis, vol, vis_sum, normalise, B, V, D, H, W, vb, ve, st);
+        return gl_launch_aggregate_w16(feat, dtype, layout, hom, hyp, vis, vol, vis_sum, normalise, B, V, C, D, H, W, vb, ve, st, boxes, pipe);
+    GL_DISPATCH(gl_launch_aggregate_f32_t, feat, hom, hyp, vis, vol, vis_sum, normalise, B, V, D, H, W, vb, ve, st, boxes, pipe);
 }
 
 }
diff --git a/mvsformerplusplus_amd/csrc/gather_lds_aggregate_w16_kernels.hip b/mvsformerplusplus_amd/csrc/gather_lds_aggregate_w16_kernels.hip
--- a/mvsformerplusplus_amd/csrc/gather_lds_aggregate_w16_kernels.hip
+++ b/mvsformerplusplus_amd/csrc/gather_lds_aggregate_w16_kernels.hip
@@ -4,13 +4,14 @@
 
 template <int DT, int NOCT, int NS, bool TILED>
 static int gl_launch_aggregate_w16_t(const void* feat, const float* hom, const float* hyp, const float* vis, float* vol, float* vis_sum,
-                                     int normalise, int B, int V, int D, int H, int W, int vb, int ve, hipStream_t st) {
-    return gl_launch_aggregate_t<DT, NOCT, NS, TILED, true>(feat, hom, hyp, vis, vol, vis_sum, normalise, B, V, D, H, W, vb, ve, st);
+                                     int normalise, int B, int V, int D, int H, int W, int vb, int ve, hipStream_t st, const unsigned* boxes,
+                                     int pipe) {
+    return gl_launch_aggregate_t<DT, NOCT, NS, TILED, true>(feat, hom, hyp, vis, vol, vis_sum, normalise, B, V, D, H, W, vb, ve, st, boxes, pipe);
 }
 
 int gl_launch_aggregate_w16(const void* feat, int dtype, int layout, const float* hom, const float* hyp, const float* vis, float* vol, float* vis_sum,
-                            int normalise, int B, int V, int C, int D, int H, int W, int vb, int ve, hipStream_t st) {
-    GL_DISPATCH(gl_launch_aggregate_w16_t, feat, hom, hyp, vis, vol, vis_sum, normalise, B, V, D, H, W, vb, ve, st);
+                            int normalise, int B, int V, int C, int D, int H, int W, int vb, int ve, hipStream_t st, const unsigned* boxes, int pipe) {
+    GL_DISPATCH(gl_launch_aggregate_w16_t, feat, hom, hyp, vis, vol, vis_sum, normalise, B, V, D, H, W, vb, ve, st, boxes, pipe);
 }
 
 }
diff --git a/mvsformerplusplus_amd/csrc/gather_lds_entropy_w16_kernels.hip b/mvsformerplusplus_amd/csrc/gather_lds_entropy_w16_kernels.hip
--- a/mvsformerplusplus_amd/csrc/gather_lds_entropy_w16_kernels.hip
+++ b/mvsformerplusplus_amd/csrc/gather_lds_entropy_w16_kernels.hip
@@ -4,13 +4,13 @@
 
 template <int DT, int NOCT, int NS, bool TILED>
 static int gl_launch_entropy_w16_t(const void* feat, const float* hom, const float* hyp, float* ent, int B, int V, int D, int H, int W, int vb,
-                                   int ve, hipStream_t st) {
-    return gl_launch_entropy_t<DT, NOCT, NS, TILED, false, true>(feat, hom, hyp, ent, B, V, D, H, W, vb, ve, st);
+                                   int ve, hipStream_t st, unsigned* boxes) {
+    return gl_launch_entropy_t<DT, NOCT, NS, TILED, false, true>(feat, hom, hyp, ent, B, V, D, H, W, vb, ve, st, nullptr, boxes);
 }
 
 int gl_launch_entropy_w16(const void* feat, int dtype, int layout, const float* hom, const float* hyp, float* ent, int B, int V, int C, int D, int H, int W,
-                          int vb, int ve, hipStream_t st) {
-    GL_DISPATCH(gl_launch_entropy_w16_t, feat, hom, hyp, ent, B, V, D, H, W, vb, ve, st);
+                          int vb, int ve, hipStream_t st, unsigned* boxes) {
+    GL_DISPATCH(gl_launch_entropy_w16_t, feat, hom, hyp, ent, B, V, D, H, W, vb, ve, st, boxes);
 }
 
 }
diff --git a/mvsformerplusplus_amd/csrc/gather_lds_kernels.hip b/mvsformerplusplus_amd/csrc/gather_lds_kernels.hip
--- a/mvsformerplusplus_amd/csrc/gather_lds_kernels.hip
+++ b/mvsformerplusplus_amd/csrc/gather_lds_kernels.hip
@@ -20,12 +20,24 @@
 
 
 int gl_launch_entropy_w16(const void* feat, int dtype, int layout, const float* hom, const float* hyp, float* ent, int B, int V, int C, int D, int H, int W,
-                          int vb, int ve, hipStream_t st);
+                          int vb, int ve, hipStream_t st, unsigned* boxes);
+
+template <int DT, int NOCT, int NS, bool TILED>
+static int gl_launch_entropy_f32_t(const void* feat, const float* hom, const float* hyp, float* ent, int B, int V, int D, int H, int W, int vb,
+                                   int ve, hipStream_t st, unsigned* boxes) {
+    return gl_launch_entropy_t<DT, NOCT, NS, TILED, false, false>(feat, hom, hyp, ent, B, V, D, H, W, vb, ve, st, nullptr, boxes);
+}
+
+void gl_boxes_dims(int D, int H, int W, int* iters, int* tiles) {
+    const int ns = gl_slots(D), tw = 256 / ns / GL_TH, nch = (D + GL_DCH - 1) / GL_DCH;
+    *iters = (nch + ns - 1) / ns;
+    *tiles = (int)(ceil_div(W, tw) * ceil_div(H, GL_TH));
+}
 
 int gl_launch_entropy(const void* feat, int dtype, int layout, const float* hom, const float* hyp, float* ent, int B, int V, int C, int D, int H, int W,
-                      int vb, int ve, int w16, hipStream_t st) {
-    if (w16 && gl_window_f16_enabled()) return gl_launch_entropy_w16(feat, dtype, layout, hom, hyp, ent, B, V, C, D, H, W, vb, ve, st);
-    GL_DISPATCH(gl_launch_entropy_t, feat, hom, hyp, ent, B, V, D, H, W, vb, ve, st);
+                      int vb, int ve, int w16, hipStream_t st, unsigned* boxes) {
+    if (w16 && gl_window_f16_enabled()) return gl_launch_entropy_w16(feat, dtype, layout, hom, hyp, ent, B, V, C, D, H, W, vb, ve, st, boxes);
+    GL_DISPATCH(gl_launch_entropy_f32_t, feat, hom, hyp, ent, B, V, D, H, W, vb, ve, st, boxes);
 }
 
 template <typename TI, typename TO>
diff --git a/mvsformerplusplus_amd/csrc/warp_kernels.hip b/mvsformerplusplus_amd/csrc/warp_kernels.hip
--- a/mvsformerplusplus_amd/csrc/warp_kernels.hip
+++ b/mvsformerplusplus_amd/csrc/warp_kernels.hip
@@ -529,9 +529,10 @@
 
 bool gl_supported(int C, int G, int D, int H, int W);
 int gl_launch_entropy(const void* feat, int dtype, int layout, const float* hom, const float* hyp, float* ent, int B, int V, int C, int D, int H,
-                      int W, int vb, int ve, int w16, hipStream_t st);
+                      int W, int vb, int ve, int w16, hipStream_t st, unsigned* boxes);
 int gl_launch_aggregate(const void* feat, int dtype, int layout, const float* hom, const float* hyp, const float* vis, float* vol,
-                        float* vis_sum, int normalise, int B, int V, int C, int D, int H, int W, int vb, int ve, hipStream_t st);
+                        float* vis_sum, int normalise, int B, int V, int C, int D, int H, int W, int vb, int ve, hipStream_t st, const unsigned* boxes);
+void gl_boxes_dims(int D, int H, int W, int* iters, int* tiles);
 bool gl_keep_supported(int C, int G, int D, int H, int W);
 bool gl_keep32_supported(int C, int G, int D, int H, int W);
 int gl_launch_entropy_keep(const void* feat, int dtype, int layout, const float* hom, const float* hyp, float* ent, void* corr, int corr_format, int B,
@@ -619,19 +620,54 @@
     return MVS_OK;
 }
 
+static int boxes_supported(const char* who, int layout, int C, int G, int D, int H, int W) {
+    if (layout != MVS_LAYOUT_OCTET_TILED && gather_impl(C, G, D, H, W) != 1) {
+        set_error("%s: window boxes belong to the LDS-staged gather (G == 8, C in {8,16,32,64}, W %% 8 == 0); mvs_gather_is_lds_staged() says which shapes qualify", who);
+        return MVS_ERR_UNSUPPORTED;
+    }
+    return MVS_OK;
+}
+
+extern "C" int mvs_gather_boxes_dims(int D, int H, int W, int* iterations, int* tiles) {
+    if (!iterations || !tiles || D < 1 || H < 1 || W < 1) { set_error("mvs_gather_boxes_dims: bad arguments"); return MVS_ERR_ARG; }
+    gl_boxes_dims(D, H, W, iterations, tiles);
+    return MVS_OK;
+}
+
+static int warp_corr_entropy(const char* who, const void* features, int dtype, int layout, const float* homography, const float* hyp, float* entropy,
+                             unsigned* boxes, int B, int V, int C, int G, int D, int H, int W, int view_begin, int view_end, int gather_format,
+                             void* stream);
+
 extern "C" int mvs_warp_corr_entropy_fwd(const void* features, int dtype, int layout, const float* homography, const float* hyp, float* entropy,
                                          int B, int V, int C, int G, int D, int H, int W, int view_begin, int view_end, int gather_format,
                                          void* stream) {
-    int rc = check_corr_args("mvs_warp_corr_entropy_fwd", features, homography, hyp, dtype, B, V, C, G, D, H, W, view_begin, view_end);
+    return warp_corr_entropy("mvs_warp_corr_entropy_fwd", features, dtype, layout, homography, hyp, entropy, nullptr, B, V, C, G, D, H, W, view_begin,
+                             view_end, gather_format, stream);
+}
+
+extern "C" int mvs_warp_corr_entropy_boxes_fwd(const void* features, int dtype, int layout, const float* homography, const float* hyp, float* entropy,
+                                               unsigned* boxes, int B, int V, int C, int G, int D, int H, int W, int view_begin, int view_end,
+                                               int gather_format, void* stream) {
+    if (!boxes) { set_error("mvs_warp_corr_entropy_boxes_fwd: null boxes"); return MVS_ERR_ARG; }
+    const int rc = boxes_supported("mvs_warp_corr_entropy_boxes_fwd", layout, C, G, D, H, W);
     if (rc != MVS_OK) return rc;
-    if (!entropy) { set_error("mvs_warp_corr_entropy_fwd: null output"); return MVS_ERR_ARG; }
-    if (gather_format != MVS_GATHER_F32 && gather_format != MVS_GATHER_F16) { set_error("mvs_warp_corr_entropy_fwd: unknown gather format %d", gather_format); return MVS_ERR_ARG; }
+    return warp_corr_entropy("mvs_warp_corr_entropy_boxes_fwd", features, dtype, layout, homography, hyp, entropy, boxes, B, V, C, G, D, H, W, view_begin,
+                             view_end, gather_format, stream);
+}
+
+static int warp_corr_entropy(const char* who, const void* features, int dtype, int layout, const float* homography, const float* hyp, float* entropy,
+                             unsigned* boxes, int B, int V, int C, int G, int D, int H, int W, int view_begin, int view_end, int gather_format,
+                             void* stream) {
+    int rc = check_corr_args(who, features, homography, hyp, dtype, B, V, C, G, D, H, W, view_begin, view_end);
+    if (rc != MVS_OK) return rc;
+    if (!entropy) { set_error("%s: null output", who); return MVS_ERR_ARG; }
+    if (gather_format != MVS_GATHER_F32 && gather_format != MVS_GATHER_F16) { set_error("%s: unknown gather format %d", who, gather_format); return MVS_ERR_ARG; }
     hipStream_t st = (hipStream_t)stream;
-    rc = check_layout("mvs_warp_corr_entropy_fwd", layout, C, G, D, H, W);
+    rc = check_layout(who, layout, C, G, D, H, W);
     if (rc != MVS_OK) return rc;
     const int impl = gather_impl(C, G, D, H, W);
     if (layout == MVS_LAYOUT_OCTET_TILED || impl == 1)
-        return gl_launch_entropy(features, dtype, layout, homography, hyp, entropy, B, V, C, D, H, W, view_begin, view_end, gather_format == MVS_GATHER_F16, st);
+        return gl_launch_entropy(features, dtype, layout, homography, hyp, entropy, B, V, C, D, H, W, view_begin, view_end, gather_format == MVS_GATHER_F16, st, boxes);
     switch (dtype) {
         case MVS_DTYPE_F32: MVS_DISPATCH_CG(launch_entropy, MVS_DTYPE_F32, features, homography, hyp, entropy, B, V, C, G, D, H, W, view_begin, view_end, st);
         case MVS_DTYPE_BF16: MVS_DISPATCH_CG(launch_entropy, MVS_DTYPE_BF16, features, homography, hyp, entropy, B, V, C, G, D, H, W, view_begin, view_end, st);
@@ -669,9 +705,30 @@
     return launch_corr_aggregate(corr, corr_format, vis, volume_cl, volume_format, B, V, D, H, W, (hipStream_t)stream);
 }
 
+static int warp_corr_aggregate(const void* features, int dtype, int layout, const float* homography, const float* hyp, const float* vis,
+                               float* volume_cl, float* vis_sum, int normalise, int volume_format, const unsigned* boxes, int B, int V, int C, int G,
+                               int D, int H, int W, int view_begin, int view_end, void* stream);
+
 extern "C" int mvs_warp_corr_aggregate_fwd(const void* features, int dtype, int layout, const float* homography, const float* hyp, const float* vis,
                                            float* volume_cl, float* vis_sum, int normalise, int volume_format, int B, int V, int C, int G,
                                            int D, int H, int W, int view_begin, int view_end, void* stream) {
+    return warp_corr_aggregate(features, dtype, layout, homography, hyp, vis, volume_cl, vis_sum, normalise, volume_format, nullptr, B, V, C, G, D, H, W,
+                               view_begin, view_end, stream);
+}
+
+extern "C" int mvs_warp_corr_aggregate_boxes_fwd(const void* features, int dtype, int layout, const float* homography, const float* hyp, const float* vis,
+                                                 float* volume_cl, float* vis_sum, int normalise, int volume_format, const unsigned* boxes, int B, int V,
+                                                 int C, int G, int D, int H, int W, int view_begin, int view_end, void* stream) {
+    if (!boxes) { set_error("mvs_warp_corr_aggregate_boxes_fwd: null boxes"); return MVS_ERR_ARG; }
+    const int rc = boxes_supported("mvs_warp_corr_aggregate_boxes_fwd", layout, C, G, D, H, W);
+    if (rc != MVS_OK) return rc;
+    return warp_corr_aggregate(features, dtype, layout, homography, hyp, vis, volume_cl, vis_sum, normalise, volume_format, boxes, B, V, C, G, D, H, W,
+                               view_begin, view_end, stream);
+}
+
+static int warp_corr_aggregate(const void* features, int dtype, int layout, const float* homography, const float* hyp, const float* vis,
+                               float* volume_cl, float* vis_sum, int normalise, int volume_format, const unsigned* boxes, int B, int V, int C, int G,
+                               int D, int H, int W, int view_begin, int view_end, void* stream) {
     int rc = check_corr_args("mvs_warp_corr_aggregate_fwd", features, homography, hyp, dtype, B, V, C, G, D, H, W, view_begin, view_end);
     if (rc != MVS_OK) return rc;
     if (!vis || !volume_cl) { set_error("mvs_warp_corr_aggregate_fwd: null pointer"); return MVS_ERR_ARG; }
@@ -686,7 +743,7 @@
     if (rc != MVS_OK) return rc;
     const int impl = gather_impl(C, G, D, H, W);
     if (layout == MVS_LAYOUT_OCTET_TILED || impl == 1)
-        return gl_launch_aggregate(features, dtype, layout, homography, hyp, vis, volume_cl, vis_sum, normalise | (volume_format << 1), B, V, C, D, H, W, view_begin, view_end, st);
+        return gl_launch_aggregate(features, dtype, layout, homography, hyp, vis, volume_cl, vis_sum, normalise | (volume_format << 1), B, V, C, D, H, W, view_begin, view_end, st, boxes);
     if (volume_format == MVS_VOLUME_F16) {
         set_error("mvs_warp_corr_aggregate_fwd: the fp16 volume is written by the LDS-staged gather only (C in {8,16,32,64}, W %% 8 == 0); "
                   "for other shapes aggregate in MVS_VOLUME_F32 and convert with mvs_volume_to_f16");
diff --git a/mvsformerplusplus_amd/ops.py b/mvsformerplusplus_amd/ops.py
--- a/mvsformerplusplus_amd/ops.py
+++ b/mvsformerplusplus_amd/ops.py
@@ -275,7 +275,8 @@
 
 
 def warp_corr_entropy(features: torch.Tensor, code: int, homography: torch.Tensor, hyp: torch.Tensor, G: int,
-                      view_begin: int = 1, view_end: Optional[int] = None, out: Optional[torch.Tensor] = None, f16_window: bool = False) -> torch.Tensor:
+                      view_begin: int = 1, view_end: Optional[int] = None, out: Optional[torch.Tensor] = None, f16_window: bool = False,
+                      boxes: Optional[torch.Tensor] = None) -> torch.Tensor:
     B, V, Cc, H, W = features.shape
     D = hyp.shape[1]
     view_end = V if view_end is None else view_end
@@ -286,9 +287,25 @@
     else:
         ent = torch.zeros(B, V - 1, H, W, dtype=torch.float32, device=features.device)
     ft, layout = _feat_ptr(features)
+    if boxes is not None:
+        assert boxes.dtype == torch.int32 and tuple(boxes.shape) == gather_boxes_shape(B, V, D, H, W), "boxes: gather_boxes(...) of this call's shapes"
+        check(lib().mvs_warp_corr_entropy_boxes_fwd(ptr(ft), code, layout, ptr(homography), ptr(hyp), ptr(ent), ptr(boxes), B, V, Cc, G, D, H, W,
+                                                    view_begin, view_end, 1 if f16_window else 0, stream_of(ft)), "mvs_warp_corr_entropy_boxes_fwd")
+        return ent
     check(lib().mvs_warp_corr_entropy_fwd(ptr(ft), code, layout, ptr(homography), ptr(hyp), ptr(ent), B, V, Cc, G, D, H, W,
                                           view_begin, view_end, 1 if f16_window else 0, stream_of(ft)), "mvs_warp_corr_entropy_fwd")
     return ent
+
+
+def gather_boxes_shape(B: int, V: int, D: int, H: int, W: int) -> Tuple[int, int, int, int, int]:
+    it, tiles = C.c_int(0), C.c_int(0)
+    check(lib().mvs_gather_boxes_dims(D, H, W, C.addressof(it), C.addressof(tiles)), "mvs_gather_boxes_dims")
+    return (B, V - 1, it.value, tiles.value, 2)
+
+
+def gather_boxes(features: torch.Tensor, hyp: torch.Tensor) -> torch.Tensor:
+    B, V, _, H, W = features.shape
+    return torch.empty(gather_boxes_shape(B, V, hyp.shape[1], H, W), dtype=torch.int32, device=features.device)
 
 
 def vis_weight(entropy: torch.Tensor, params: Sequence[torch.Tensor], precision: int = 0) -> torch.Tensor:
@@ -321,7 +338,7 @@
 
 def warp_corr_aggregate(features: torch.Tensor, code: int, homography: torch.Tensor, hyp: torch.Tensor, vis: torch.Tensor,
                         G: int, normalise: bool = True, view_begin: int = 1, view_end: Optional[int] = None, out=None, split: bool = False,
-                        f16: bool = False):
+                        f16: bool = False, boxes: Optional[torch.Tensor] = None):
     B, V, Cc, H, W = features.shape
     D = hyp.shape[1]
     view_end = V if view_end is None else view_end
@@ -331,6 +348,12 @@
         vol = torch.empty(B, D, H, W, G, dtype=torch.float16 if f16 else torch.float32, device=features.device)
         vsum = None if normalise else torch.empty(B, H, W, dtype=torch.float32, device=features.device)
     ft, layout = _feat_ptr(features)
+    if boxes is not None:
+        assert boxes.dtype == torch.int32 and tuple(boxes.shape) == gather_boxes_shape(B, V, D, H, W), "boxes: gather_boxes(...) of this call's shapes"
+        check(lib().mvs_warp_corr_aggregate_boxes_fwd(ptr(ft), code, layout, ptr(homography), ptr(hyp), ptr(vis), ptr(vol), ptr(vsum),
+                                                      1 if normalise else 0, _lib.VOLUME_F16 if f16 else (_lib.VOLUME_SPLIT if split else _lib.VOLUME_F32),
+                                                      ptr(boxes), B, V, Cc, G, D, H, W, view_begin, view_end, stream_of(ft)), "mvs_warp_corr_aggregate_boxes_fwd")
+        return vol, vsum
     check(lib().mvs_warp_corr_aggregate_fwd(ptr(ft), code, layout, ptr(homography), ptr(hyp), ptr(vis), ptr(vol), ptr(vsum),
                                             1 if normalise else 0, _lib.VOLUME_F16 if f16 else (_lib.VOLUME_SPLIT if split else _lib.VOLUME_F32), B, V, Cc, G, D, H, W,
                                             view_begin, view_end, stream_of(ft)), "mvs_warp_corr_aggregate_fwd")
diff --git a/mvsformerplusplus_amd/profiling.py b/mvsformerplusplus_amd/profiling.py
--- a/mvsformerplusplus_amd/profiling.py
+++ b/mvsformerplusplus_amd/profiling.py
@@ -249,8 +249,9 @@
                                B * (V * C * HW * esz + D * HW * 4 + (V - 1) * HW * 4) + corr_bytes,
                                lambda: ops.warp_corr_entropy_keep(feats, code, hom, hyp, 8, exact=not w16))
         else:
+            boxes = ops.gather_boxes(feats, hyp) if ops.gather_is_lds_staged(feats, 8, hyp) else None
             ent = _timed(launches, gather_kernel_name("entropy", code, C, D, W, tiled, False, w16), s, corr_flops, B * (V * C * HW * esz + D * HW * 4 + (V - 1) * HW * 4),
-                         lambda: ops.warp_corr_entropy(feats, code, hom, hyp, 8, f16_window=w16))
+                         lambda: ops.warp_corr_entropy(feats, code, hom, hyp, 8, f16_window=w16, boxes=boxes))
         vp = net._vis_params(feats.device)
         prec = _lib.PRECISIONS[net._vis_precision()]
         N = B * (V - 1)
@@ -280,7 +281,7 @@
         else:
             vol = _timed(launches, agg_name, s, corr_flops,
                          B * (V * C * HW * esz + D * HW * 4 + (V - 1) * HW * 4 + 8 * D * HW * (2 if f16 else 4)),
-                         lambda: ops.warp_corr_aggregate(feats, code, hom, hyp, vis, 8, split=split, f16=f16)[0])
+                         lambda: ops.warp_corr_aggregate(feats, code, hom, hyp, vis, 8, split=split, f16=f16, boxes=boxes)[0])
         if getattr(net.cost_reg, "kind", None) == "transformer":
             pos = None
             if head.use_pe3d:
```

After: 680.4, median of 6. No clear change (+0.5%).
